# weiguangzhao/PBNet

Measured on AMD Instinct MI355X. Metric: scenes/sec fwd+cluster (ScanNet ~150k pts/scene), higher is better.
Workload: dtype bf16

## Files before the change

include/pbnet_hip.h:

```cpp
#ifndef PBNET_HIP_H
#define PBNET_HIP_H

#include <stddef.h>
#include <stdint.h>

#ifdef __cplusplus
extern "C" {
#endif

typedef void* pbn_stream_t;

enum {
    PBN_OK = 0,
    PBN_ERR_ARG = -1,
    PBN_ERR_WORKSPACE = -2,
    PBN_ERR_HIP = -3,
    PBN_ERR_RANGE = -4,
    PBN_ERR_UNSUPPORTED = -5
};

enum { PBN_F32 = 0, PBN_BF16 = 1, PBN_F16 = 2 };

#define PBN_MAX_SCENES 8

const char* pbn_version(void);
int pbn_last_hip_error(void);

size_t pbn_cluster_workspace_bytes(int n_points, int n_segments, int general_sem);

int pbn_binary_cluster(const float* off_xyz, const float* org_xyz, const int32_t* sem, const int32_t* seg_len,
                       int n_points, int n_segments, float radius, int min_pts, float para_f, int nv_flag,
                       int general_sem , int32_t* cluster_id, int32_t* cluster_num, int32_t* den, float* centers,
                       int32_t* clt_sem, int32_t* n_clusters, int32_t* member_start, int32_t* member_idx,
                       void* workspace, size_t workspace_bytes, pbn_stream_t stream);

int pbn_get_iou(const int32_t* proposals_idx, const int32_t* proposals_offset, const int64_t* instance_labels,
                const int32_t* instance_pointnum, float* proposals_iou, int n_instance, int n_proposal,
                pbn_stream_t stream);

int pbn_cal_iou_and_masklabel(const int32_t* proposals_idx, const int32_t* proposals_offset,
                              const int64_t* instance_labels, const int32_t* instance_pointnum,
                              float* proposals_iou, int n_instance, int n_proposal,
                              const float* mask_scores_sigmoid, float* mask_label, int mode, pbn_stream_t stream);


int pbn_hash_capacity(int n);
size_t pbn_coords_workspace_bytes(int n_max);

int pbn_coords_unique(const int32_t* coords, const int32_t* n_dev, int n_max, uint64_t* table_keys, int32_t* table_vals,
                      int capacity, int32_t* unique_index, int32_t* inverse, int32_t* unique_coords, int32_t* n_unique,
                      void* workspace, size_t workspace_bytes, pbn_stream_t stream);

int pbn_coords_stride(const int32_t* fine_coords, const int32_t* n_fine_dev, int n_fine_max, int stride_out,
                      uint64_t* table_keys, int32_t* table_vals, int capacity, int32_t* coarse_coords,
                      int32_t* parent_row, int32_t* child_k, int32_t* nbr_down, int32_t* n_coarse, void* workspace,
                      size_t workspace_bytes, pbn_stream_t stream);

int pbn_kernel_map(const int32_t* out_coords, const int32_t* n_out_dev, int n_out_max, const int32_t* offsets,
                   int n_offsets, const uint64_t* table_keys, const int32_t* table_vals, int capacity, int32_t* nbr,
                   pbn_stream_t stream);

int pbn_kernel_map_cube(const int32_t* out_coords, const int32_t* n_out_dev, int n_out_max, int kernel_size,
                        int tensor_stride, int x_fastest, const uint64_t* table_keys, const int32_t* table_vals,
                        int capacity, int32_t* nbr, pbn_stream_t stream);

int pbn_up_table(const int32_t* parent_row, const int32_t* child_k, const int32_t* n_fine_dev, int n_fine_max,
                 int32_t* nbr_up, pbn_stream_t stream);

int pbn_spconv_forward(const void* in_feat, int ld_in, int n_in, const int32_t* nbr, int n_offsets, const int32_t* row_perm,
                       const int32_t* n_out_dev, int n_out, const void* w_packed, int vecs_per_offset, int n_steps,
                       int cout_padded, const float* scale, const float* shift, const void* residual, int ld_res,
                       int relu, void* out_feat, int ld_out, int dtype, int rows_per_wave, void* workspace,
                       size_t workspace_bytes, pbn_stream_t stream);

int pbn_spconv_forward_dual(const void* in_feat, int ld_in, int n_in, const int32_t* nbr, int n_offsets,
                            const int32_t* n_out_dev, int n_out, const void* w_packed, int vecs_per_offset, int n_steps,
                            int cout_padded, const float* scale, const float* shift, const void* residual, int ld_res,
                            int relu, void* out_feat, int ld_out, int dtype, int rows_per_wave, void* workspace,
                            size_t workspace_bytes, const void* in2_feat, int ld_in2, int n_in2, int vecs_second,
                            pbn_stream_t stream);

int pbn_spconv_family(int n_out, int n_offsets, int vecs_per_offset, int n_steps, int cout_padded, int dtype, int has_map);

int pbn_gather_rows(const void* in, int ld_in_bytes, const int64_t* idx, int n, int row_bytes, void* out,
                    int ld_out_bytes, pbn_stream_t stream);

size_t pbn_segment_pool_workspace_bytes(int n_seg, int channels);
int pbn_segment_pool(const void* feats, int ld, int channels, int dtype, const int32_t* seg_start, int n_seg,
                     float* out_max, float* out_avg, void* workspace, size_t workspace_bytes, pbn_stream_t stream);

int pbn_local_scene_rows(const int32_t* ent_row_start, const int32_t* ent_member_start, const int32_t* ent_scene,
                         const float* ent_weight, int n_ent, int n_rows, const int32_t* member_idx,
                         const int64_t* ins_ind, const float* xyz, float inv_voxel, const void* point_feat, int ld_feat,
                         int channels, const void* sem_score, int ld_sem, const int64_t* sem_pred, int dtype,
                         int64_t* point_idx, int64_t* row_scene, int32_t* coords, void* feat_out, int ld_out,
                         pbn_stream_t stream);
int pbn_gather_pad_rows(const void* in, int ld_in_bytes, int row_bytes, const int64_t* idx, int n, void* out,
                        int ld_out_bytes, pbn_stream_t stream);

int pbn_pack_weight(const float* src, int n_offsets, int dim_a, int dim_b, int flip, int transpose, int dtype,
                    int vecs_per_offset, int n_steps, int cout_padded, void* out, pbn_stream_t stream);

typedef struct pbn_pack_job {
    const float* src;
    void* out;
    int32_t n_offsets, dim_a, dim_b, flip, transpose, cin, cout, cin_p, cout_p, n_steps;
    int32_t reserved[2];
} pbn_pack_job;
int pbn_pack_weights_batch(const pbn_pack_job* jobs, int n_jobs, int max_vectors, int dtype, pbn_stream_t stream);

int pbn_gather_rulebook_rows(const void* in, int ld_in_bytes, int row_bytes, const int32_t* nbr, int n_offsets, int k0,
                             int kc, int n, void* out, pbn_stream_t stream);

size_t pbn_bn_workspace_bytes(int channels);
int pbn_bn_train_forward(const void* x, int ld_x, int n, int channels, int dtype, const float* weight, const float* bias,
                         float eps, float momentum, float* running_mean, float* running_var, void* y, int ld_y,
                         float* save_mean, float* save_invstd, void* workspace, size_t workspace_bytes, pbn_stream_t stream);
int pbn_bn_train_backward(const void* x, int ld_x, const void* dy, int ld_dy, int n, int channels, int dtype,
                          const float* weight, const float* save_mean, const float* save_invstd, void* dx, int ld_dx,
                          float* dweight, float* dbias, void* workspace, size_t workspace_bytes, pbn_stream_t stream);

int pbn_bn_act_train_forward(const void* x, int ld_x, int n, int channels, int dtype, const float* weight, const float* bias,
                             float eps, float momentum, float* running_mean, float* running_var, const void* residual,
                             int ld_res, int relu, void* y, int ld_y, float* save_mean, float* save_invstd, void* workspace,
                             size_t workspace_bytes, pbn_stream_t stream);
int pbn_bn_act_train_backward(const void* x, int ld_x, const void* dy, int ld_dy, const void* y, int ld_y, int n, int channels,
                              int dtype, const float* weight, const float* save_mean, const float* save_invstd, void* dx,
                              int ld_dx, void* dres, int ld_dres, float* dweight, float* dbias, void* workspace,
                              size_t workspace_bytes, pbn_stream_t stream);

int pbn_rulebook_pair_blocks(int n);
int pbn_rulebook_pair_counts(const int32_t* nbr, int n, int n_offsets, int32_t* table, int32_t* totals, pbn_stream_t stream);
int pbn_rulebook_pair_fill(const int32_t* nbr, int n, int n_offsets, const int32_t* table, const int32_t* seg_start, int seg,
                           int n_segments, int32_t* in_idx, int32_t* out_idx, int64_t* seg_offset, pbn_stream_t stream);

int pbn_rulebook_pair_fill_dev(const int32_t* nbr, int n, int n_offsets, const int32_t* table, const int32_t* totals,
                               int segment, int32_t* seg_begin, int32_t* in_idx, int32_t* out_idx, int64_t* seg_offset,
                               pbn_stream_t stream);

typedef struct {
    const int32_t* nbr;
    int32_t n, n_offsets;
    int32_t* table;
    int32_t* totals;
    int32_t* seg_begin;
    int32_t* in_idx;
    int32_t* out_idx;
    int64_t* seg_offset;
} pbn_pair_job;
int pbn_rulebook_pairs_multi(const pbn_pair_job* jobs, int n_jobs, int segment, pbn_stream_t stream);

size_t pbn_spconv_wgrad_workspace_bytes(int n_offsets, int cin, int cout);
int pbn_spconv_wgrad(const void* x, int ld_x, const void* g, int ld_g, int dtype, const int32_t* in_idx,
                     const int32_t* out_idx, const int32_t* seg_begin, const int32_t* pair_counts, int segment,
                     int n_pairs_total, int n_offsets, int cin, int cout, float* dw, void* workspace, size_t workspace_bytes,
                     pbn_stream_t stream);
int pbn_spconv_wgrad_checked(const void* x, int ld_x, long long n_x_rows, const void* g, int ld_g, long long n_g_rows, int dtype,
                             const int32_t* in_idx, const int32_t* out_idx, const int32_t* seg_begin, const int32_t* pair_counts,
                             int lists_padded, int segment, int n_pairs_total, int n_offsets, int cin, int cout, float* dw,
                             void* workspace, size_t workspace_bytes, pbn_stream_t stream);
typedef struct {
    int32_t form, wa, wb, small_level, strips, co_groups, splits;
    int64_t grid;
} pbn_wgrad_plan;
int pbn_spconv_wgrad_plan(int dtype, int ld_x, int ld_g, int aligned16, int identity, int n_offsets, int n_pairs_total, int cin,
                          int cout, int has_workspace, size_t workspace_bytes, pbn_wgrad_plan* out);

enum {
    PBN_CNT_POINTS = 0, PBN_CNT_CLUSTERS = 1, PBN_CNT_ENTRIES = 2, PBN_CNT_ROWS = 3, PBN_CNT_SCENES = 4,
    PBN_CNT_PROPOSAL_ROWS = 5, PBN_CNT_PROPOSALS = 6, PBN_CNT_OVERFLOW = 7, PBN_CNT_WORDS = 16
};
enum {
    PBN_OVF_POINTS = 1, PBN_OVF_CLUSTERS = 2, PBN_OVF_ENTRIES = 4, PBN_OVF_ROWS = 8, PBN_OVF_SEGMENT = 16,
    PBN_OVF_BATCH = 32, PBN_OVF_LEVEL = 64,
    PBN_OVF_CDIST = 128
};
int pbn_class_gate(const int32_t* table, const float* thr05, int n_classes, int nb, int m_cap, int n_points,
                   int32_t* class_base, int32_t* seg_len, int32_t* counts, pbn_stream_t stream);
size_t pbn_local_plan_workspace_bytes(int c_cap);
int pbn_local_plan(const int32_t* cluster_num, int n_segments, int nb, const int32_t* member_start, const float* centers,
                   const int32_t* n_clusters, const float* thr02, const int32_t* kmax, int c_cap, int e_cap, int r_cap,
                   int32_t* ent_row_start, int32_t* ent_member_start, int32_t* ent_scene, float* ent_weight,
                   int32_t* counts, void* workspace, size_t workspace_bytes, pbn_stream_t stream);
int pbn_proposal_offsets(const int32_t* per_scene, int s_cap, int64_t* proposals_offset, int64_t* alive_ids,
                         int32_t* dense_of, int32_t* counts, pbn_stream_t stream);
int pbn_batch_starts(const int32_t* coords, const int32_t* n_dev, int n_cap, int n_segments, int32_t* seg_start,
                     pbn_stream_t stream);
int pbn_local_scene_rows_dev(const int32_t* ent_row_start, const int32_t* ent_member_start, const int32_t* ent_scene,
                             const float* ent_weight, int n_ent_cap, int n_rows_cap, const int32_t* n_ent_dev,
                             const int32_t* n_rows_dev, const int32_t* member_idx, const int64_t* ins_ind, const float* xyz,
                             float inv_voxel, const void* point_feat, int ld_feat, int channels, const void* sem_score,
                             int ld_sem, const int64_t* sem_pred, int dtype, int64_t* point_idx, int64_t* row_scene,
                             int32_t* coords, void* feat_out, int ld_out, pbn_stream_t stream);
int pbn_gather_pad_rows_dev(const void* in, int ld_in_bytes, int row_bytes, const int64_t* idx, const int64_t* idx2,
                            int n_cap, const int32_t* n_dev, void* out, int ld_out_bytes, pbn_stream_t stream);
int pbn_mlp_rows_dev(const void* in, int ld_in, int in_rows, int channels, const int64_t* idx_a, const int64_t* idx_b, int n_cap,
                     const int32_t* n_dev, const float* w1, const float* scale, const float* shift, const float* slope,
                     int hidden, const float* w2, const float* b2, int n_out, int sigmoid, void* out, int ld_out, int dtype,
                     pbn_stream_t stream);
int pbn_mask_count_dev(const void* mask_score, int ld, float thd, const int64_t* row_scene, int n_cap, const int32_t* n_dev,
                       int n_scenes_cap, int dtype, int32_t* per_scene, int32_t* block_cnt, pbn_stream_t stream);
int pbn_proposal_rows_dev(const void* mask_score, int ld, float thd, const int64_t* row_scene, const int64_t* point_idx,
                          int n_cap, const int32_t* n_dev, const int32_t* dense_of, const int32_t* block_cnt,
                          const float* xyz, float scale, float inv_voxel, const void* point_feat, int ld_feat, int channels,
                          int dtype, int64_t* proposals_idx, void* proposals_ms, int32_t* coords, void* feat_out,
                          pbn_stream_t stream);

int pbn_mlp_rows(const void* in, int ld_in, int channels, const int64_t* idx_a, const int64_t* idx_b, int n,
                 const float* w1, const float* scale, const float* shift, const float* slope, int hidden, const float* w2,
                 const float* b2, int n_out, int sigmoid, void* out, int ld_out, int dtype, pbn_stream_t stream);

int pbn_select_blocks(int n);
int pbn_sem_argmax_table(const void* score, int ld, int n_cls, const int32_t* batch, int nb, int n, int dtype,
                         int64_t* sem_pred, void* sem_prob, int32_t* table, int32_t* block_hist, pbn_stream_t stream);
int pbn_select_points(const int64_t* sem_pred, int n, int n_cls, const int32_t* class_base, const int32_t* block_hist,
                      const float* xyz, const void* offset, int ld_off, int dtype, int64_t* ins_ind, float* ins_orig,
                      float* ins_off, int32_t* ins_sem, pbn_stream_t stream);

int pbn_mask_count(const void* mask_score, int ld, float thd, const int64_t* row_scene, int n, int n_scenes, int dtype,
                   int32_t* per_scene, int32_t* block_cnt, pbn_stream_t stream);
int pbn_proposal_rows(const void* mask_score, int ld, float thd, const int64_t* row_scene, const int64_t* point_idx, int n,
                      const int32_t* dense_of, const int32_t* block_cnt, const float* xyz, float scale, float inv_voxel,
                      const void* point_feat, int ld_feat, int channels, int dtype, int64_t* proposals_idx,
                      void* proposals_ms, int32_t* coords, void* feat_out, pbn_stream_t stream);

int pbn_post_words(int n_fold);
int pbn_proposal_bitmask(const int64_t* proposals_idx, int n_entries, int n_fold, int n_prop, uint32_t* masks,
                         int32_t* counts, pbn_stream_t stream);
int pbn_mask_iou(const uint32_t* masks, const int32_t* rows, int n_rows, int n_fold, const int32_t* counts, float* iou,
                 pbn_stream_t stream);
int pbn_superpoint_refine(const uint32_t* masks, const int32_t* pick, int n_pick, int n_fold, const int64_t* superpoint,
                          int n_sp, int64_t* seg, int32_t* hist, int64_t* sp_label, int64_t* seg_refined,
                          uint32_t* masks_out, int32_t* counts_out, pbn_stream_t stream);
int pbn_bitmask_to_dense(const uint32_t* masks, const int32_t* rows, int n_rows, int n_fold, int32_t* dense,
                         pbn_stream_t stream);

int pbn_post_max_proposals(void);
int pbn_post_select(const float* clt_score, const int32_t* counts, int n_prop, float score_t, int npoint_t, int32_t* rows,
                    int32_t* n_rows, int32_t* status, pbn_stream_t stream);
int pbn_mask_iou_dev(const uint32_t* masks, const int32_t* rows, const int32_t* n_rows, int n_prop, int n_fold,
                     const int32_t* counts, float* iou, pbn_stream_t stream);
int pbn_post_nms(const float* clt_score, const int32_t* rows, const int32_t* n_rows, int n_prop, const float* iou, float nms_t,
                 int32_t* pick, int32_t* pick_rows, int32_t* n_pick, pbn_stream_t stream);
int pbn_superpoint_refine_dev(const uint32_t* masks, const int32_t* pick_rows, const int32_t* n_pick, int n_prop, int n_fold,
                              const int64_t* superpoint, int n_sp_cap, int64_t* seg, int32_t* hist, int64_t* sp_label,
                              int64_t* seg_refined, uint32_t* masks_out, int32_t* counts_out, int32_t* status,
                              pbn_stream_t stream);
int pbn_post_compact(const int32_t* counts2, const int32_t* pick_rows, const int32_t* n_pick, int n_prop, int n_fold,
                     const float* clt_score, const int64_t* proposals_idx, int n_entries, const void* proposals_offset,
                     int offset_i64, const void* pred_sem, int sem_i64, int64_t n_sem, const int64_t* label_table, int n_labels,
                     const uint32_t* masks2, int32_t* keep, float* scores_out, int64_t* semantic_id_out, int32_t* clusters,
                     int32_t* n_keep, int32_t* status, pbn_stream_t stream);

typedef struct pbn_scene_table {
    int32_t n_scenes;
    int32_t point_start[PBN_MAX_SCENES + 1];
    int32_t sp_start[PBN_MAX_SCENES + 1];
} pbn_scene_table;
typedef struct pbn_post_batch_layout {
    int64_t masks, counts, prop_scene, score, rows, pick_rows, n_rows, n_pick, iou, votes, sp_label, seg, seg_refined, counts2,
        renumber, total_bytes;
} pbn_post_batch_layout;
size_t pbn_post_batch_workspace_bytes(int n_prop, int n_points_total, int n_scenes, int n_sp_total, pbn_post_batch_layout* layout);
int pbn_post_batch(const int64_t* proposals_idx, int n_entries, const void* proposals_offset, int offset_i64, int n_prop,
                   const void* clt_score, int score_dtype, const void* pred_sem, int sem_i64, int n_points_total,
                   pbn_scene_table scenes, const int64_t* superpoint, float score_t, int npoint_t, float nms_t,
                   const int64_t* label_table, int n_labels, int32_t* point_instance, float* scores, int64_t* semantic_id,
                   int32_t* npoints, int32_t* scalars, void* workspace, size_t workspace_bytes, pbn_stream_t stream);

typedef struct pbn_tta_table {
    int32_t n_scenes;
    int32_t copies;
    int32_t point_start[PBN_MAX_SCENES + 1];
    int32_t sp_start[PBN_MAX_SCENES + 1];
} pbn_tta_table;
int pbn_post_batch_tta(const int64_t* proposals_idx, int n_entries, const void* proposals_offset, int offset_i64, int n_prop,
                       const void* clt_score, int score_dtype, const void* pred_sem, int sem_i64, int n_points_merged,
                       pbn_tta_table units, const int64_t* superpoint, float score_t, int npoint_t, float nms_t,
                       const int64_t* label_table, int n_labels, int32_t* point_instance, float* scores, int64_t* semantic_id,
                       int32_t* npoints, int32_t* scalars, void* workspace, size_t workspace_bytes, pbn_stream_t stream);

size_t pbn_scene_summary_workspace_bytes(int n_prop, int n_cls);
int pbn_scene_summary_lds_instances(int n_cls);
int pbn_scene_summary(const void* sem_score, int ld, int n_cls, int score_dtype, int n_points_merged, pbn_tta_table units,
                      const int32_t* point_instance, const int32_t* post_scalars, int n_prop, const float* xyz,
                      const int64_t* label_table, int n_labels, int32_t* sem_fold, int64_t* class_vote, int32_t* class_points,
                      float* box, float* centroid, int32_t* status, void* workspace, size_t workspace_bytes, pbn_stream_t stream);

int pbn_instance_overlap(const int32_t* masks, int n_pred, int n_pts, const int32_t* gt_index, int n_gt, int32_t* inter,
                         pbn_stream_t stream);

#define PBN_AP_RECORD_MAGIC 0x41504c47
#define PBN_AP_RECORD_HEADER 8
#define PBN_AP_STATUS_ID_RANGE 4
#define PBN_AP_STATUS_ID_COUNT 8
#define PBN_AP_STATUS_LABEL_RANGE 16
#define PBN_AP_STATUS_INSTANCE_CAP 32
#define PBN_AP_STATUS_SEMANTIC_RANGE 64
int pbn_gt_encode_dev(const void* sem, int sem_i64, const void* ins, int ins_i64, int n_pts, const int32_t* label_table,
                      int n_labels, int32_t* first, int n_inst_cap, int32_t* ids, int32_t* status, pbn_stream_t stream);
int pbn_gt_index_dev(const void* ids, int ids_i64, int n_pts, int32_t* table, int id_cap, int32_t* uid, int32_t* gt_vert,
                     int u_cap, int32_t* n_gt, int32_t* gt_index, int32_t* status, pbn_stream_t stream);
int pbn_instance_overlap_dev(const int32_t* clusters, const int32_t* n_keep, int p_cap, int n_pts, const int32_t* gt_index,
                             const int32_t* n_gt, int u_cap, int32_t* inter, pbn_stream_t stream);
int pbn_ap_record_append(int32_t* state, int32_t* log, int64_t log_words, int scene_tag, const int32_t* n_keep, int p_cap,
                         const int32_t* n_gt, int u_cap, int n_pts, const int32_t* post_status, int32_t* assoc_status,
                         const int32_t* uid, const int32_t* gt_vert, const int64_t* semantic_id, const float* conf,
                         const int32_t* inter, pbn_stream_t stream);

typedef struct pbn_ap_scene_tags {
    int32_t tag[PBN_MAX_SCENES];
} pbn_ap_scene_tags;
size_t pbn_ap_assoc_batch_workspace_bytes(int n_points_total, int n_scenes, int u_cap, int id_cap, int n_inst_cap);
int pbn_ap_assoc_batch_lds_counters(void);
int pbn_ap_assoc_batch(pbn_tta_table units, const int32_t* point_instance, const int32_t* post_scalars, const float* scores,
                       const int64_t* semantic_id, int n_prop, const void* ids, int ids_i64, const void* sem, int sem_i64,
                       const void* ins, int ins_i64, const int32_t* label_table, int n_labels, int u_cap, int id_cap,
                       int n_inst_cap, pbn_ap_scene_tags tags, int32_t* state, int32_t* log, int64_t log_words, void* workspace,
                       size_t workspace_bytes, pbn_stream_t stream);

#define PBN_AP_MAX_CLASSES 32
#define PBN_AP_MAX_OVERLAPS 16
#define PBN_AP_TABLE_SCALARS 16
typedef struct pbn_ap_class_ids {
    int32_t n;
    int32_t id[PBN_AP_MAX_CLASSES];
} pbn_ap_class_ids;
typedef struct pbn_ap_overlaps {
    int32_t n;
    int32_t _pad;
    double th[PBN_AP_MAX_OVERLAPS];
// ... 259 lines not shown
```

pbnet_amd/MinkowskiEngine/nn.py:

```python
import torch
import torch.nn as nn

from .._native import DT as _DT
from ..scratch import StreamScratch
from .core import SparseTensor

_BN_WS = StreamScratch()


def _bn_workspace(device, channels):
    from .. import _native as N
    return _BN_WS.get(device, int(N.lib().pbn_bn_workspace_bytes(int(channels))), min_bytes=1 << 20, zero=True)


def _rows_ok(t):
    es = t.element_size()
    return t.dim() == 2 and t.stride(1) == 1 and (t.stride(0) * es) % 16 == 0 and t.data_ptr() % 16 == 0 \
        and (t.shape[1] * es) % 16 == 0 and t.shape[0] > 0


class _BatchNormTrainFn(torch.autograd.Function):

    @staticmethod
    def forward(ctx, x, weight, bias, running_mean, running_var, eps, momentum):
# ... 62 lines not shown
        dw = torch.empty(c, dtype=torch.float32, device=x.device) if need_w else None
        db = torch.empty(c, dtype=torch.float32, device=x.device) if (weight is not None and ctx.needs_input_grad[2]) else None
        ws = _bn_workspace(x.device, c)
        N.check(N.lib().pbn_bn_act_train_backward(
            N.c_vp(x.data_ptr()), x.stride(0), N.c_vp(dy.data_ptr()), dy.stride(0), None if y is None else N.c_vp(y.data_ptr()),
            0 if y is None else y.stride(0), n, c, _DT[x.dtype], N.ptr(weight), N.ptr(mean), N.ptr(invstd), N.c_vp(dx.data_ptr()), c,
            None if dres is None else N.c_vp(dres.data_ptr()), c, N.ptr(dw), N.ptr(db), N.c_vp(ws.data_ptr()), ws.numel(),
            N.current_stream()), "pbn_bn_act_train_backward")
        if want_res and dres is None:
            dres = dy
        return dx, dw, db, dres, None, None, None, None, None


def bn_act(norm, x, residual=None, relu=True):
    f, bn = x.F, norm.bn
    res = None if residual is None else residual.F
    if norm.NATIVE_TRAIN and norm.FUSE_ACT and bn.training and f.is_cuda and bn.momentum is not None and f.dtype in _DT \
            and _rows_ok(f) and (bn.weight is None or bn.weight.dtype == torch.float32) \
            and (res is None or (res.dtype == f.dtype and _rows_ok(res) and res.shape == f.shape)):
        norm._tick()
        rm, rv = (bn.running_mean, bn.running_var) if bn.track_running_stats else (None, None)
        return x.replace_feature(_BatchNormActTrainFn.apply(f, bn.weight, bn.bias, res, rm, rv, bn.eps, bn.momentum, relu))
    out = norm(x)
    if residual is not None:
        out = out.replace_feature(out.F + residual.F)
    return out.replace_feature(torch.relu(out.F)) if relu else out


def _flush_ticks_hook(module, prefix, keep_vars):
    module.flush_ticks()


def _drop_ticks_hook(module, state_dict, prefix, *unused):
    if prefix + "num_batches_tracked" in state_dict:
        module.__dict__["_pending_ticks"] = 0


class _TickedBatchNorm1d(nn.BatchNorm1d):

    def __init__(self, *a, **k):
        super().__init__(*a, **k)
        self.__dict__["_pending_ticks"] = 0
        self.register_state_dict_pre_hook(_flush_ticks_hook)
        self.register_load_state_dict_pre_hook(_drop_ticks_hook)

    def flush_ticks(self):
        t = self.__dict__.get("_pending_ticks", 0)
        if t:
            self.__dict__["_pending_ticks"] = 0
            buf = self._buffers.get("num_batches_tracked")
            if buf is not None:
                buf.add_(t)

    def __getattr__(self, name):
        if name == "num_batches_tracked":
            self.flush_ticks()
        return super().__getattr__(name)

    def _apply(self, fn, *a, **k):
        self.flush_ticks()
        return super()._apply(fn, *a, **k)

    def buffers(self, *a, **k):
        self.flush_ticks()
        return super().buffers(*a, **k)

    def named_buffers(self, *a, **k):
        self.flush_ticks()
        return super().named_buffers(*a, **k)


class MinkowskiBatchNorm(nn.Module):

    NATIVE_TRAIN = True
    FUSE_ACT = True

    def __init__(self, num_features, eps=1e-5, momentum=0.1, affine=True, track_running_stats=True):
        super().__init__()
        self.bn = _TickedBatchNorm1d(num_features, eps=eps, momentum=momentum, affine=affine,
                                     track_running_stats=track_running_stats)

    def _tick(self):
        bn = self.bn
        if bn.track_running_stats and bn._buffers.get("num_batches_tracked") is not None:
            bn.__dict__["_pending_ticks"] = bn.__dict__.get("_pending_ticks", 0) + 1

    def forward(self, x):
        f, bn = x.F, self.bn
        if self.NATIVE_TRAIN and bn.training and f.is_cuda and bn.momentum is not None and f.dtype in _DT and _rows_ok(f) \
                and (bn.weight is None or bn.weight.dtype == torch.float32):
            self._tick()
            rm, rv = (bn.running_mean, bn.running_var) if bn.track_running_stats else (None, None)
            return x.replace_feature(_BatchNormTrainFn.apply(f, bn.weight, bn.bias, rm, rv, bn.eps, bn.momentum))
        return x.replace_feature(bn(f))


class _Elementwise(nn.Module):
    MODULE = None

    def __init__(self, *args, **kwargs):
        super().__init__()
        self.module = self.MODULE(*args, **kwargs)

    def forward(self, x):
        f = x.F
        if f.dtype != torch.float32 and any(True for _ in self.module.parameters()):
            return x.replace_feature(self.module(f.float()).to(f.dtype))
        return x.replace_feature(self.module(f))


class MinkowskiReLU(_Elementwise):
    MODULE = nn.ReLU


class MinkowskiPReLU(_Elementwise):
    MODULE = nn.PReLU


class MinkowskiSigmoid(_Elementwise):
    MODULE = nn.Sigmoid


class MinkowskiSoftmax(_Elementwise):
    MODULE = nn.Softmax

    def __init__(self, dim=1):
        super().__init__(dim=dim)


def _batch_index(x):
    assert x.tensor_stride >= 1
    b = x.C[:, 0].long()
    return b, int(b.max().item()) + 1 if b.numel() else 0


def segment_pool(feats, batch_sorted, n_batch, want_max=True, want_avg=True, seg_start=None):
    from .. import _native as N
    assert feats.stride(1) == 1
    if seg_start is None:
        seg_start = torch.searchsorted(batch_sorted.to(torch.int32).contiguous(),
                                       torch.arange(n_batch + 1, dtype=torch.int32, device=feats.device)).to(torch.int32)
    c = feats.shape[1]
    mx = torch.empty(n_batch, c, dtype=torch.float32, device=feats.device) if want_max else None
    av = torch.empty(n_batch, c, dtype=torch.float32, device=feats.device) if want_avg else None
    lib = N.lib()
    ws_bytes = int(lib.pbn_segment_pool_workspace_bytes(int(n_batch), c))
    ws = torch.empty(max(ws_bytes, 16), dtype=torch.uint8, device=feats.device)
    rc = lib.pbn_segment_pool(N.c_vp(feats.data_ptr()), feats.stride(0), c, _DT[feats.dtype], N.ptr(seg_start),
                              int(n_batch), N.ptr(mx), N.ptr(av), N.c_vp(ws.data_ptr()), ws_bytes, N.current_stream())
    N.check(rc, "pbn_segment_pool")
    return mx, av


class _SegmentPoolFn(torch.autograd.Function):

    @staticmethod
    def forward(ctx, feats, batch_sorted, n_batch):
        mx, av = segment_pool(feats.detach(), batch_sorted, n_batch)
        b = batch_sorted.long()
        ctx.save_for_backward(feats, b, mx)
        ctx.n_batch = n_batch
        return mx + av

    @staticmethod
    def backward(ctx, g):
        feats, b, mx = ctx.saved_tensors
        g = g.float()
        f = feats.float()
        cnt = torch.bincount(b, minlength=ctx.n_batch).to(torch.float32).clamp_(min=1.0)
        gb = g[b]
        ties = (f == mx[b]).to(torch.float32)
        tie_cnt = torch.zeros(ctx.n_batch, f.shape[1], dtype=torch.float32, device=f.device).index_add_(0, b, ties)
        grad = gb / cnt[b][:, None] + gb * ties / tie_cnt[b].clamp_(min=1.0)
        return grad.to(feats.dtype), None, None


def global_max_plus_avg_pool(x):
    b, nb = _batch_index(x)
    return _PooledTensor(_SegmentPoolFn.apply(x.F, x.C[:, 0].contiguous(), nb).to(x.F.dtype))


class _GlobalPool(nn.Module):
    MODE = "avg"

    def forward(self, x):
        b, nb = _batch_index(x)
        f = x.F.float()
        if self.MODE == "avg":
            s = torch.zeros(nb, f.shape[1], dtype=f.dtype, device=f.device).index_add_(0, b, f)
            cnt = torch.zeros(nb, dtype=f.dtype, device=f.device).index_add_(0, b, torch.ones_like(b, dtype=f.dtype))
            out = s / cnt[:, None]
        else:
            out = torch.full((nb, f.shape[1]), float("-inf"), dtype=f.dtype, device=f.device)
            out = out.scatter_reduce(0, b[:, None].expand_as(f), f, reduce="amax", include_self=True)
        return _PooledTensor(out.to(x.F.dtype))


class _PooledTensor(object):

    def __init__(self, feats):
        self._F = feats

    @property
    def F(self):
        return self._F

    def replace_feature(self, feats):
        return _PooledTensor(feats)

    def __add__(self, other):
        return _PooledTensor(self._F + other._F)


class MinkowskiGlobalAvgPooling(_GlobalPool):
    MODE = "avg"


class MinkowskiGlobalMaxPooling(_GlobalPool):
    MODE = "max"
```

pbnet_amd/_native.py:

```python
import ctypes
import os

import torch

_HERE = os.path.dirname(os.path.abspath(__file__))
LIB_PATH = os.environ.get("PBNET_HIP_LIB") or os.path.join(_HERE, "libpbnet_hip.so")

_lib = None

c_f32p = ctypes.c_void_p
c_i32p = ctypes.c_void_p
c_vp = ctypes.c_void_p
c_int = ctypes.c_int
c_float = ctypes.c_float
c_size = ctypes.c_size_t

c_i64 = ctypes.c_int64
c_i32 = ctypes.c_int32

DT = {torch.float32: 0, torch.bfloat16: 1, torch.float16: 2}


class CoordsLayout(ctypes.Structure):
    _fields_ = [("counts", c_i64), ("unique_index", c_i64), ("inverse", c_i64),
                ("keys", c_i64 * 5), ("vals", c_i64 * 5), ("coords", c_i64 * 5), ("k3", c_i64 * 5),
                ("parent_row", c_i64 * 4), ("child_k", c_i64 * 4), ("nbr_down", c_i64 * 4), ("up", c_i64 * 4),
                ("k5", c_i64), ("workspace", c_i64), ("workspace_bytes", c_i64),
                ("capacity", c_i32 * 5), ("_pad", c_i32)]


class PrepareLayout(ctypes.Structure):
    _fields_ = [("pyramid", CoordsLayout), ("n_unique", c_i64), ("unique_index", c_i64), ("inverse", c_i64),
                ("perm", c_i64), ("inv_perm", c_i64), ("ucoords", c_i64), ("tmp_keys", c_i64), ("tmp_vals", c_i64),
                ("uidx32", c_i64), ("inv32", c_i64), ("sort_keys", c_i64), ("sort_vals", c_i64), ("sort_temp", c_i64),
                ("sort_temp_bytes", c_i64)]


class UnetOp(ctypes.Structure):
    _fields_ = [("map_kind", c_i32), ("level_in", c_i32), ("level_out", c_i32),
                ("in_buf", c_i32), ("in_col", c_i32), ("res_buf", c_i32), ("res_col", c_i32), ("out_buf", c_i32),
                ("out_col", c_i32), ("vpo", c_i32), ("n_steps", c_i32), ("cout_p", c_i32), ("relu", c_i32),
                ("in2_buf", c_i32), ("in2_col", c_i32), ("vpo2", c_i32),
                ("w", ctypes.c_void_p), ("scale", ctypes.c_void_p), ("shift", ctypes.c_void_p)]


class WgradPlan(ctypes.Structure):
    _fields_ = [("form", c_i32), ("wa", c_i32), ("wb", c_i32), ("small_level", c_i32), ("strips", c_i32),
                ("co_groups", c_i32), ("splits", c_i32), ("grid", c_i64)]


class UnetBuf(ctypes.Structure):
    _fields_ = [("level", c_i32), ("width", c_i32)]


class TrainOp(ctypes.Structure):
    _fields_ = [("map_kind", c_i32), ("level_in", c_i32), ("level_out", c_i32),
                ("in_buf", c_i32), ("in_col", c_i32), ("pre_buf", c_i32), ("res_buf", c_i32), ("res_col", c_i32),
                ("out_buf", c_i32), ("out_col", c_i32), ("relu", c_i32), ("cin", c_i32), ("cout", c_i32),
                ("vpo", c_i32), ("n_steps", c_i32), ("cout_p", c_i32), ("vpo_d", c_i32), ("n_steps_d", c_i32),
                ("cout_p_d", c_i32), ("want_dx", c_i32), ("dx_accumulate", c_i32), ("_pad", c_i32),
                ("w", ctypes.c_void_p), ("w_d", ctypes.c_void_p), ("gamma", ctypes.c_void_p), ("beta", ctypes.c_void_p),
                ("running_mean", ctypes.c_void_p), ("running_var", ctypes.c_void_p), ("eps", ctypes.c_float),
                ("momentum", ctypes.c_float), ("stat_off", ctypes.c_int64), ("dw_off", ctypes.c_int64),
                ("dgamma_off", ctypes.c_int64), ("dbeta_off", ctypes.c_int64)]


class PairJob(ctypes.Structure):
    _fields_ = [("nbr", ctypes.c_void_p), ("n", c_i32), ("n_offsets", c_i32), ("table", ctypes.c_void_p),
                ("totals", ctypes.c_void_p), ("seg_begin", ctypes.c_void_p), ("in_idx", ctypes.c_void_p),
                ("out_idx", ctypes.c_void_p), ("seg_offset", ctypes.c_void_p)]


class PairLists(ctypes.Structure):
    _fields_ = [("in_idx", ctypes.c_void_p), ("out_idx", ctypes.c_void_p), ("seg_begin", ctypes.c_void_p),
                ("counts", ctypes.c_void_p), ("segment", c_i32), ("n_pairs_estimate", c_i32)]


MAX_SCENES = 8


class SceneTable(ctypes.Structure):
    _fields_ = [("n_scenes", c_i32), ("point_start", c_i32 * (MAX_SCENES + 1)), ("sp_start", c_i32 * (MAX_SCENES + 1))]


class TtaTable(ctypes.Structure):
    _fields_ = [("n_scenes", c_i32), ("copies", c_i32), ("point_start", c_i32 * (MAX_SCENES + 1)),
                ("sp_start", c_i32 * (MAX_SCENES + 1))]


class SceneTags(ctypes.Structure):
    _fields_ = [("tag", c_i32 * MAX_SCENES)]


AP_MAX_CLASSES, AP_MAX_OVERLAPS, AP_TABLE_SCALARS = 32, 16, 16


class ApClassIds(ctypes.Structure):
    _fields_ = [("n", c_i32), ("id", c_i32 * AP_MAX_CLASSES)]


class ApOverlaps(ctypes.Structure):
    _fields_ = [("n", c_i32), ("_pad", c_i32), ("th", ctypes.c_double * AP_MAX_OVERLAPS)]


class PostBatchLayout(ctypes.Structure):
    _fields_ = [(k, c_i64) for k in ("masks", "counts", "prop_scene", "score", "rows", "pick_rows", "n_rows", "n_pick", "iou",
                                     "votes", "sp_label", "seg", "seg_refined", "counts2", "renumber", "total_bytes")]


SIGNATURES = {
    "pbn_version": (ctypes.c_char_p, []),
    "pbn_last_hip_error": (c_int, []),
    "pbn_cluster_workspace_bytes": (c_size, [c_int, c_int, c_int]),
    "pbn_binary_cluster": (c_int, [c_f32p, c_f32p, c_i32p, c_i32p, c_int, c_int, c_float, c_int, c_float, c_int, c_int,
                                   c_i32p, c_i32p, c_i32p, c_f32p, c_i32p, c_i32p, c_i32p, c_i32p, c_vp, c_size, c_vp]),
    "pbn_get_iou": (c_int, [c_i32p, c_i32p, c_vp, c_i32p, c_f32p, c_int, c_int, c_vp]),
    "pbn_cal_iou_and_masklabel": (c_int, [c_i32p, c_i32p, c_vp, c_i32p, c_f32p, c_int, c_int, c_f32p, c_f32p, c_int,
                                          c_vp]),
    "pbn_hash_capacity": (c_int, [c_int]),
    "pbn_coords_workspace_bytes": (c_size, [c_int]),
    "pbn_coords_unique": (c_int, [c_i32p, c_i32p, c_int, c_vp, c_i32p, c_int, c_i32p, c_i32p, c_i32p, c_i32p, c_vp,
                                  c_size, c_vp]),
    "pbn_coords_stride": (c_int, [c_i32p, c_i32p, c_int, c_int, c_vp, c_i32p, c_int, c_i32p, c_i32p, c_i32p, c_i32p,
                                  c_i32p, c_vp, c_size, c_vp]),
    "pbn_kernel_map": (c_int, [c_i32p, c_i32p, c_int, c_i32p, c_int, c_vp, c_i32p, c_int, c_i32p, c_vp]),
    "pbn_up_table": (c_int, [c_i32p, c_i32p, c_i32p, c_int, c_i32p, c_vp]),
    "pbn_spconv_forward": (c_int, [c_vp, c_int, c_int, c_i32p, c_int, c_i32p, c_i32p, c_int, c_vp, c_int, c_int, c_int,
                                   c_f32p, c_f32p, c_vp, c_int, c_int, c_vp, c_int, c_int, c_int, c_vp, c_size, c_vp]),
    "pbn_spconv_forward_dual": (c_int, [c_vp, c_int, c_int, c_i32p, c_int, c_i32p, c_int, c_vp, c_int, c_int, c_int, c_f32p, c_f32p,
                                        c_vp, c_int, c_int, c_vp, c_int, c_int, c_int, c_vp, c_size, c_vp, c_int, c_int, c_int, c_vp]),
    "pbn_spconv_family": (c_int, [c_int, c_int, c_int, c_int, c_int, c_int, c_int]),
    "pbn_spconv_wgrad_workspace_bytes": (c_size, [c_int, c_int, c_int]),
    "pbn_spconv_wgrad": (c_int, [c_vp, c_int, c_vp, c_int, c_int, c_vp, c_vp, c_i32p, c_i32p, c_int, c_int, c_int, c_int, c_int,
                                 c_f32p, c_vp, c_size, c_vp]),
    "pbn_spconv_wgrad_checked": (c_int, [c_vp, c_int, ctypes.c_longlong, c_vp, c_int, ctypes.c_longlong, c_int, c_vp, c_vp, c_i32p,
                                         c_i32p, c_int, c_int, c_int, c_int, c_int, c_int, c_f32p, c_vp, c_size, c_vp]),
    "pbn_spconv_wgrad_plan": (c_int, [c_int, c_int, c_int, c_int, c_int, c_int, c_int, c_int, c_int, c_int, c_size,
                                      ctypes.POINTER(WgradPlan)]),
    "pbn_gather_rows": (c_int, [c_vp, c_int, c_vp, c_int, c_int, c_vp, c_int, c_vp]),
    "pbn_segment_pool_workspace_bytes": (c_size, [c_int, c_int]),
    "pbn_segment_pool": (c_int, [c_vp, c_int, c_int, c_int, c_i32p, c_int, c_f32p, c_f32p, c_vp, c_size, c_vp]),
    "pbn_local_scene_rows": (c_int, [c_i32p, c_i32p, c_i32p, c_f32p, c_int, c_int, c_i32p, c_vp, c_f32p, c_float, c_vp,
                                     c_int, c_int, c_vp, c_int, c_vp, c_int, c_vp, c_vp, c_i32p, c_vp, c_int, c_vp]),
    "pbn_gather_pad_rows": (c_int, [c_vp, c_int, c_int, c_vp, c_int, c_vp, c_int, c_vp]),
    "pbn_mlp_rows": (c_int, [c_vp, c_int, c_int, c_vp, c_vp, c_int, c_f32p, c_f32p, c_f32p, c_f32p, c_int, c_f32p, c_f32p,
                             c_int, c_int, c_vp, c_int, c_int, c_vp]),
    "pbn_select_blocks": (c_int, [c_int]),
    "pbn_sem_argmax_table": (c_int, [c_vp, c_int, c_int, c_i32p, c_int, c_int, c_int, c_vp, c_vp, c_i32p, c_i32p, c_vp]),
    "pbn_select_points": (c_int, [c_vp, c_int, c_int, c_i32p, c_i32p, c_f32p, c_vp, c_int, c_int, c_vp, c_f32p, c_f32p,
                                  c_i32p, c_vp]),
    "pbn_mask_count": (c_int, [c_vp, c_int, c_float, c_vp, c_int, c_int, c_int, c_i32p, c_i32p, c_vp]),
    "pbn_proposal_rows": (c_int, [c_vp, c_int, c_float, c_vp, c_vp, c_int, c_i32p, c_i32p, c_f32p, c_float, c_float, c_vp,
                                  c_int, c_int, c_int, c_vp, c_vp, c_i32p, c_vp, c_vp]),
    "pbn_post_words": (c_int, [c_int]),
    "pbn_proposal_bitmask": (c_int, [c_vp, c_int, c_int, c_int, c_vp, c_i32p, c_vp]),
    "pbn_mask_iou": (c_int, [c_vp, c_i32p, c_int, c_int, c_i32p, c_f32p, c_vp]),
    "pbn_superpoint_refine": (c_int, [c_vp, c_i32p, c_int, c_int, c_vp, c_int, c_vp, c_i32p, c_vp, c_vp, c_vp, c_i32p,
                                      c_vp]),
    "pbn_bitmask_to_dense": (c_int, [c_vp, c_i32p, c_int, c_int, c_i32p, c_vp]),
    "pbn_post_max_proposals": (c_int, []),
    "pbn_post_select": (c_int, [c_f32p, c_i32p, c_int, c_float, c_int, c_i32p, c_i32p, c_i32p, c_vp]),
    "pbn_mask_iou_dev": (c_int, [c_vp, c_i32p, c_i32p, c_int, c_int, c_i32p, c_f32p, c_vp]),
    "pbn_post_nms": (c_int, [c_f32p, c_i32p, c_i32p, c_int, c_f32p, c_float, c_i32p, c_i32p, c_i32p, c_vp]),
    "pbn_superpoint_refine_dev": (c_int, [c_vp, c_i32p, c_i32p, c_int, c_int, c_vp, c_int, c_vp, c_i32p, c_vp, c_vp, c_vp, c_i32p,
                                          c_i32p, c_vp]),
    "pbn_post_compact": (c_int, [c_i32p, c_i32p, c_i32p, c_int, c_int, c_f32p, c_vp, c_int, c_vp, c_int, c_vp, c_int, c_i64, c_vp,
                                 c_int, c_vp, c_i32p, c_f32p, c_vp, c_i32p, c_i32p, c_i32p, c_vp]),
    "pbn_post_batch_workspace_bytes": (c_size, [c_int, c_int, c_int, c_int, ctypes.POINTER(PostBatchLayout)]),
    "pbn_post_batch": (c_int, [c_vp, c_int, c_vp, c_int, c_int, c_vp, c_int, c_vp, c_int, c_int, SceneTable, c_vp, c_float, c_int,
                               c_float, c_vp, c_int, c_i32p, c_f32p, c_vp, c_i32p, c_i32p, c_vp, c_size, c_vp]),
    "pbn_post_batch_tta": (c_int, [c_vp, c_int, c_vp, c_int, c_int, c_vp, c_int, c_vp, c_int, c_int, TtaTable, c_vp, c_float, c_int,
                                   c_float, c_vp, c_int, c_i32p, c_f32p, c_vp, c_i32p, c_i32p, c_vp, c_size, c_vp]),
    "pbn_scene_summary_workspace_bytes": (c_size, [c_int, c_int]),
    "pbn_scene_summary_lds_instances": (c_int, [c_int]),
    "pbn_scene_summary": (c_int, [c_vp, c_int, c_int, c_int, c_int, TtaTable, c_i32p, c_i32p, c_int, c_f32p, c_vp, c_int, c_i32p,
                                  c_vp, c_i32p, c_f32p, c_f32p, c_i32p, c_vp, c_size, c_vp]),
    "pbn_instance_overlap": (c_int, [c_i32p, c_int, c_int, c_i32p, c_int, c_i32p, c_vp]),
    "pbn_gt_encode_dev": (c_int, [c_vp, c_int, c_vp, c_int, c_int, c_i32p, c_int, c_i32p, c_int, c_i32p, c_i32p, c_vp]),
    "pbn_gt_index_dev": (c_int, [c_vp, c_int, c_int, c_i32p, c_int, c_i32p, c_i32p, c_int, c_i32p, c_i32p, c_i32p, c_vp]),
    "pbn_instance_overlap_dev": (c_int, [c_i32p, c_i32p, c_int, c_int, c_i32p, c_i32p, c_int, c_i32p, c_vp]),
    "pbn_ap_record_append": (c_int, [c_i32p, c_i32p, c_i64, c_int, c_i32p, c_int, c_i32p, c_int, c_int, c_i32p, c_i32p, c_i32p,
                                     c_i32p, c_vp, c_f32p, c_i32p, c_vp]),
    "pbn_ap_assoc_batch_workspace_bytes": (c_size, [c_int, c_int, c_int, c_int, c_int]),
    "pbn_ap_assoc_batch_lds_counters": (c_int, []),
    "pbn_ap_assoc_batch": (c_int, [TtaTable, c_i32p, c_i32p, c_f32p, c_vp, c_int, c_vp, c_int, c_vp, c_int, c_vp, c_int, c_i32p,
                                   c_int, c_int, c_int, c_int, SceneTags, c_i32p, c_i32p, c_i64, c_vp, c_size, c_vp]),
    "pbn_ap_table_workspace_bytes": (c_size, [c_int, c_i64]),
    "pbn_ap_table_lds_entries": (c_int, []),
    "pbn_ap_table_reset": (c_int, [c_vp, c_size, c_int, c_i64, c_vp]),
    "pbn_ap_table_add_log": (c_int, [c_vp, c_size, c_int, c_i64, c_i32p, c_i32p, c_i64, c_int, ApClassIds, ApOverlaps, c_int,
                                     c_vp]),
    "pbn_ap_table_finish": (c_int, [c_vp, c_size, c_int, c_i64, c_int, c_int, c_f32p, c_i32p, c_i32p, c_i32p, c_i32p, c_vp]),
    "pbn_rulebook_pair_blocks": (c_int, [c_int]),
    "pbn_bn_workspace_bytes": (c_size, [c_int]),
    "pbn_bn_train_forward": (c_int, [c_vp, c_int, c_int, c_int, c_int, c_f32p, c_f32p, ctypes.c_float, ctypes.c_float, c_f32p,
                                     c_f32p, c_vp, c_int, c_f32p, c_f32p, c_vp, c_size, c_vp]),
    "pbn_bn_train_backward": (c_int, [c_vp, c_int, c_vp, c_int, c_int, c_int, c_int, c_f32p, c_f32p, c_f32p, c_vp, c_int,
                                      c_f32p, c_f32p, c_vp, c_size, c_vp]),
    "pbn_bn_act_train_forward": (c_int, [c_vp, c_int, c_int, c_int, c_int, c_f32p, c_f32p, ctypes.c_float, ctypes.c_float,
                                         c_f32p, c_f32p, c_vp, c_int, c_int, c_vp, c_int, c_f32p, c_f32p, c_vp, c_size, c_vp]),
    "pbn_bn_act_train_backward": (c_int, [c_vp, c_int, c_vp, c_int, c_vp, c_int, c_int, c_int, c_int, c_f32p, c_f32p, c_f32p,
                                          c_vp, c_int, c_vp, c_int, c_f32p, c_f32p, c_vp, c_size, c_vp]),
    "pbn_rulebook_pair_counts": (c_int, [c_i32p, c_int, c_int, c_i32p, c_i32p, c_vp]),
    "pbn_rulebook_pair_fill_dev": (c_int, [c_i32p, c_int, c_int, c_i32p, c_i32p, c_int, c_i32p, c_vp, c_vp, c_vp, c_vp]),
    "pbn_rulebook_pair_fill": (c_int, [c_i32p, c_int, c_int, c_i32p, c_i32p, c_int, c_int, c_vp, c_vp, c_vp, c_vp]),
    "pbn_gather_rulebook_rows": (c_int, [c_vp, c_int, c_int, c_i32p, c_int, c_int, c_int, c_int, c_vp, c_vp]),
    "pbn_pack_weights_batch": (c_int, [c_vp, c_int, c_int, c_int, c_vp]),
    "pbn_pack_weight": (c_int, [c_f32p, c_int, c_int, c_int, c_int, c_int, c_int, c_int, c_int, c_int, c_vp, c_vp]),
    "pbn_kernel_map_cube": (c_int, [c_i32p, c_i32p, c_int, c_int, c_int, c_int, c_vp, c_i32p, c_int, c_i32p, c_vp]),
    "pbn_coords_arena_bytes": (c_size, [c_int, c_int, ctypes.POINTER(CoordsLayout)]),
    "pbn_coords_build": (c_int, [c_i32p, c_i32p, c_int, c_int, c_int, c_vp, c_size, ctypes.POINTER(CoordsLayout), c_vp]),
    "pbn_coords_prepare_bytes": (c_size, [c_int, c_int, ctypes.POINTER(PrepareLayout)]),
    "pbn_coords_prepare": (c_int, [c_i32p, c_int, c_int, c_int, c_vp, c_size, ctypes.POINTER(PrepareLayout), c_vp]),
    "pbn_coords_prepare_dev": (c_int, [c_i32p, c_i32p, c_int, c_int, c_int, c_vp, c_size, ctypes.POINTER(PrepareLayout), c_vp]),
    "pbn_coords_prepare_hash": (c_int, [c_i32p, c_i32p, c_int, c_int, c_int, c_vp, c_size, ctypes.POINTER(PrepareLayout), c_vp]),
    "pbn_unet_forward_dev": (c_int, [ctypes.POINTER(UnetOp), c_int, ctypes.POINTER(UnetBuf), c_int, ctypes.POINTER(c_i32),
                                     c_i32p, ctypes.POINTER(c_i32), c_vp, c_int, ctypes.POINTER(ctypes.c_void_p), c_vp,
                                     ctypes.POINTER(ctypes.c_void_p), ctypes.POINTER(ctypes.c_void_p), c_vp, c_size, c_int,
                                     c_vp, c_size, c_vp]),
    "pbn_class_gate": (c_int, [c_i32p, c_f32p, c_int, c_int, c_int, c_int, c_i32p, c_i32p, c_i32p, c_vp]),
    "pbn_local_plan_workspace_bytes": (c_size, [c_int]),
    "pbn_local_plan": (c_int, [c_i32p, c_int, c_int, c_i32p, c_f32p, c_i32p, c_f32p, c_i32p, c_int, c_int, c_int, c_i32p,
                               c_i32p, c_i32p, c_f32p, c_i32p, c_vp, c_size, c_vp]),
    "pbn_proposal_offsets": (c_int, [c_i32p, c_int, c_vp, c_vp, c_i32p, c_i32p, c_vp]),
    "pbn_batch_starts": (c_int, [c_i32p, c_i32p, c_int, c_int, c_i32p, c_vp]),
    "pbn_local_scene_rows_dev": (c_int, [c_i32p, c_i32p, c_i32p, c_f32p, c_int, c_int, c_i32p, c_i32p, c_i32p, c_vp, c_f32p,
                                         c_float, c_vp, c_int, c_int, c_vp, c_int, c_vp, c_int, c_vp, c_vp, c_i32p, c_vp,
                                         c_int, c_vp]),
    "pbn_gather_pad_rows_dev": (c_int, [c_vp, c_int, c_int, c_vp, c_vp, c_int, c_i32p, c_vp, c_int, c_vp]),
    "pbn_mlp_rows_dev": (c_int, [c_vp, c_int, c_int, c_int, c_vp, c_vp, c_int, c_i32p, c_f32p, c_f32p, c_f32p, c_f32p, c_int,
                                 c_f32p, c_f32p, c_int, c_int, c_vp, c_int, c_int, c_vp]),
    "pbn_mask_count_dev": (c_int, [c_vp, c_int, c_float, c_vp, c_int, c_i32p, c_int, c_int, c_i32p, c_i32p, c_vp]),
    "pbn_proposal_rows_dev": (c_int, [c_vp, c_int, c_float, c_vp, c_vp, c_int, c_i32p, c_i32p, c_i32p, c_f32p, c_float,
                                      c_float, c_vp, c_int, c_int, c_int, c_vp, c_vp, c_i32p, c_vp, c_vp]),
    "pbn_morton_keys": (c_int, [c_i32p, c_i32p, c_int, c_vp, c_vp]),
    "pbn_unet_arena_bytes": (c_size, [ctypes.POINTER(UnetBuf), c_int, ctypes.POINTER(c_i32), c_int,
                                      ctypes.POINTER(c_i64)]),
    "pbn_unet_forward": (c_int, [ctypes.POINTER(UnetOp), c_int, ctypes.POINTER(UnetBuf), c_int, ctypes.POINTER(c_i32),
                                 c_vp, c_int, ctypes.POINTER(ctypes.c_void_p), c_vp, ctypes.POINTER(ctypes.c_void_p),
                                 ctypes.POINTER(ctypes.c_void_p), c_vp, c_size, c_int, c_vp, c_size, c_vp]),
    "pbn_rulebook_pairs_multi": (c_int, [ctypes.POINTER(PairJob), c_int, c_int, c_vp]),
    "pbn_unet_train_forward": (c_int, [ctypes.POINTER(TrainOp), c_int, ctypes.POINTER(UnetBuf), c_int, ctypes.POINTER(c_i32),
                                       c_vp, c_int, ctypes.POINTER(ctypes.c_void_p), c_vp, ctypes.POINTER(ctypes.c_void_p),
                                       ctypes.POINTER(ctypes.c_void_p), c_vp, c_size, c_vp, c_int, c_vp, c_size, c_vp, c_size,
                                       c_vp]),
    "pbn_unet_train_backward": (c_int, [ctypes.POINTER(TrainOp), c_int, ctypes.POINTER(UnetBuf), c_int, ctypes.POINTER(c_i32),
                                        c_vp, c_int, ctypes.POINTER(ctypes.c_void_p), c_vp, ctypes.POINTER(ctypes.c_void_p),
                                        ctypes.POINTER(ctypes.c_void_p), ctypes.POINTER(PairLists), c_vp, c_vp, c_size, c_vp,
                                        c_vp, c_vp, c_int, c_int, c_vp, c_size, c_vp, c_size, c_vp, c_size, c_vp]),
    "pbn_unet_forward_timed": (c_int, [ctypes.POINTER(UnetOp), c_int, ctypes.POINTER(UnetBuf), c_int,
                                       ctypes.POINTER(c_i32), c_vp, c_int, ctypes.POINTER(ctypes.c_void_p), c_vp,
                                       ctypes.POINTER(ctypes.c_void_p), ctypes.POINTER(ctypes.c_void_p), c_vp, c_size,
                                       c_int, c_vp, c_size, c_vp, ctypes.POINTER(ctypes.c_float)]),
    "pbn_aug_chunks": (c_int, [c_int]),
    "pbn_aug_workspace_bytes": (c_size, [c_int]),
    "pbn_aug_affine": (c_int, [c_f32p, c_i32p, c_int, c_int, c_i32p, c_vp, c_vp, c_i32p, c_vp, c_vp, c_vp, c_vp]),
    "pbn_aug_elastic": (c_int, [c_vp, c_i32p, c_int, c_int, c_i32p, c_int, c_int, c_f32p, c_f32p, c_int, ctypes.c_double, c_vp,
                                c_vp, c_vp]),
    "pbn_aug_sub_min": (c_int, [c_vp, c_i32p, c_int, c_int, c_i32p, c_vp, c_vp]),
    "pbn_aug_crop": (c_int, [c_vp, c_i32p, c_int, c_int, c_i32p, c_vp, c_i32p, c_vp, c_int, c_int, c_i32p, c_i32p, c_vp, c_vp,
                             c_vp, c_vp]),
    "pbn_aug_compact": (c_int, [c_vp, c_f32p, c_f32p, c_vp, c_i32p, c_vp, c_i32p, c_i32p, c_int, c_i32p, c_int, c_i32p, c_vp,
                                c_vp, c_i32p, c_vp, c_vp, c_i32p, c_i32p, c_i32p, c_i32p, c_i32p, c_vp, c_f32p, c_vp, c_i32p,
                                c_i32p, c_int, c_int, c_vp]),
    "pbn_aug_instances": (c_int, [c_vp, c_i32p, c_i32p, c_int, c_i32p, c_i32p, c_int, c_int, c_i32p, c_f32p, c_f32p, c_vp,
                                  c_vp]),
    "pbn_aug_quantize": (c_int, [c_vp, c_i32p, c_int, c_int, ctypes.c_double, c_i32p, c_f32p, c_vp]),
    "pbn_mesh_workspace_bytes": (c_size, [c_int, c_int, c_int]),
    "pbn_mesh_vertex_normals": (c_int, [c_f32p, c_int, c_vp, c_int, c_int, c_f32p, c_i32p, c_vp, c_size, c_vp]),
    "pbn_mesh_segment": (c_int, [c_f32p, c_int, c_vp, c_int, c_int, c_float, c_int, c_vp, c_f32p, c_vp, c_size,
                                 ctypes.POINTER(ctypes.c_float), c_vp]),
    "pbn_mesh_segment_point": (c_int, [c_f32p, c_f32p, c_int, c_vp, c_int, c_int, c_float, c_int, c_vp, c_vp, c_size, c_vp]),
    "pbn_cloud_workspace_bytes": (c_size, [c_int, c_int]),
    "pbn_cloud_max_k": (c_int, []),
    "pbn_cloud_knn": (c_int, [c_f32p, c_int, c_int, c_float, c_i32p, c_f32p, c_i32p, c_vp, c_size, c_vp]),
    "pbn_cloud_knn_timed": (c_int, [c_f32p, c_int, c_int, c_float, c_i32p, c_f32p, c_i32p, c_vp, c_size, c_vp,
                                    ctypes.POINTER(ctypes.c_float)]),
    "pbn_cloud_normals": (c_int, [c_f32p, c_int, c_i32p, c_int, c_f32p, c_f32p, c_vp]),
    "pbn_thin_workspace_bytes": (c_size, [c_int]),
    "pbn_thin_points": (c_int, [c_f32p, c_f32p, c_int, ctypes.c_double, c_f32p, c_f32p, c_i32p, c_i32p, c_i32p, c_i32p, c_vp, c_size,
                                c_vp]),
    "pbn_thin_points_timed": (c_int, [c_f32p, c_f32p, c_int, ctypes.c_double, c_f32p, c_f32p, c_i32p, c_i32p, c_i32p, c_i32p, c_vp,
                                      c_size, c_vp, ctypes.POINTER(ctypes.c_float)]),
    "pbn_cloud_outlier_workspace_bytes": (c_size, [c_int]),
    "pbn_cloud_outlier_mask": (c_int, [c_f32p, c_int, c_int, ctypes.c_double, c_vp, c_vp, c_vp, c_size, c_vp]),
    "pbn_cloud_raw_index_workspace_bytes": (c_size, [c_int]),
    "pbn_cloud_raw_index": (c_int, [c_i32p, c_int, c_vp, c_i32p, c_int, c_int, c_i32p, c_vp, c_size, c_vp]),
    "pbn_cloud_radius_workspace_bytes": (c_size, [c_int]),
    "pbn_cloud_radius_count": (c_int, [c_f32p, c_int, c_float, c_int, c_float, c_i32p, c_i32p, c_vp, c_size, c_vp]),
    "pbn_cloud_radius_count_timed": (c_int, [c_f32p, c_int, c_float, c_int, c_float, c_i32p, c_i32p, c_vp, c_size, c_vp,
                                             ctypes.POINTER(ctypes.c_float)]),
    "pbn_cloud_radius_raw_index_workspace_bytes": (c_size, [c_int, c_int]),
    "pbn_cloud_radius_raw_index": (c_int, [c_f32p, c_int, c_vp, c_float, c_float, c_i32p, c_int, c_i32p, c_i32p, c_vp, c_size,
                                           c_vp]),
    "pbn_cloud_orient_workspace_bytes": (c_size, [c_int, c_int]),
    "pbn_cloud_orient": (c_int, [c_f32p, c_int, c_i32p, c_int, c_f32p, c_vp, c_i32p, c_i32p, c_i32p, c_vp, c_size, c_vp]),
    "pbn_cloud_orient_timed": (c_int, [c_f32p, c_int, c_i32p, c_int, c_f32p, c_vp, c_i32p, c_i32p, c_i32p, c_vp, c_size, c_vp,
                                       ctypes.POINTER(ctypes.c_float)]),
    "pbn_cloud_upright_workspace_bytes": (c_size, [c_int, c_int]),
    "pbn_cloud_upright_max_hyp": (c_int, []),
    "pbn_cloud_upright_chunk": (c_int, []),
    "pbn_cloud_upright_hyp_block": (c_int, []),
    "pbn_cloud_upright": (c_int, [c_f32p, c_int, c_float, c_int, ctypes.c_uint64, ctypes.POINTER(ctypes.c_double),
                                  ctypes.c_double, c_int, c_f32p, c_vp, c_f32p, c_vp, c_f32p, c_vp, c_vp, c_i32p, c_i32p, c_vp,
                                  c_size, c_vp]),
    "pbn_cloud_upright_timed": (c_int, [c_f32p, c_int, c_float, c_int, ctypes.c_uint64, ctypes.POINTER(ctypes.c_double),
                                        ctypes.c_double, c_int, c_f32p, c_vp, c_f32p, c_vp, c_f32p, c_vp, c_vp, c_i32p, c_i32p,
                                        c_vp, c_size, c_vp, ctypes.POINTER(ctypes.c_float)]),
    "pbn_cloud_upright_chunked": (c_int, [c_f32p, c_int, c_float, c_int, ctypes.c_uint64, ctypes.POINTER(ctypes.c_double),
                                          ctypes.c_double, c_int, c_int, c_f32p, c_vp, c_f32p, c_vp, c_f32p, c_vp, c_vp, c_i32p,
                                          c_i32p, c_vp, c_size, c_vp]),
    "pbn_cloud_vote_workspace_bytes": (c_size, [c_int, c_int]),
    "pbn_cloud_vote_labels": (c_int, [c_i32p, c_i32p, c_i32p, c_int, c_int, c_int, c_vp, c_vp, c_i32p, c_i32p, c_i32p, c_vp, c_vp,
                                      c_size, c_vp]),
    "pbn_cloud_vote_labels_timed": (c_int, [c_i32p, c_i32p, c_i32p, c_int, c_int, c_int, c_vp, c_vp, c_i32p, c_i32p, c_i32p, c_vp,
                                            c_vp, c_size, c_vp, ctypes.POINTER(ctypes.c_float)]),
    "pbn_sem_confusion":(c_int, [c_vp, c_int, c_vp, c_int, c_i64, c_int, c_int, c_vp, c_vp, c_vp]),
    "pbn_mask_accuracy": (c_int, [c_vp, c_int, c_vp, c_int, c_i64, c_float, c_vp, c_vp]),
    "pbn_losses_workspace_bytes": (c_size, [c_i64, c_i64, c_i64]),
    "pbn_losses_forward": (c_int, [c_vp, c_int, c_int, c_vp, c_vp, c_int, c_f32p, c_f32p, c_vp, c_i64, c_int, c_vp, c_int, c_vp,
                                   c_vp, c_i64, c_f32p, c_int, c_vp, c_int, c_i64, ctypes.c_double, ctypes.c_double, c_f32p,
                                   c_f32p, c_vp, c_vp, c_vp, c_size, c_vp]),
    "pbn_losses_backward": (c_int, [c_vp, c_int, c_int, c_vp, c_vp, c_int, c_f32p, c_f32p, c_vp, c_i64, c_int, c_vp, c_int, c_vp,
                                    c_vp, c_i64, c_vp, c_int, c_f32p, c_i64, c_vp, c_f32p, c_vp, c_vp, c_vp, c_vp, c_vp]),
    "pbn_optim_chunk": (c_int, []),
    "pbn_optim_adam": (c_int, [c_vp, c_int, c_float, c_float, c_float, c_float, c_float, c_float, c_float, c_float, c_float,
                               c_int, c_vp]),
    "pbn_optim_sgd": (c_int, [c_vp, c_int, c_float, c_float, c_float, c_int, c_vp]),
    "pbn_loss_meter_update": (c_int, [c_f32p, c_vp, c_vp, c_int, c_vp]),
    "pbn_selftest_workspace_bytes": (c_size, [c_int, c_int]),
    "pbn_selftest_sort_tile": (c_int, []),
    "pbn_selftest_fill": (c_int, [c_vp, ctypes.POINTER(c_i64), ctypes.POINTER(c_i64), ctypes.POINTER(ctypes.c_uint8), c_int, c_vp]),
    "pbn_selftest_scan": (c_int, [c_i32p, c_i32p, c_int, c_int, c_i32p, c_i32p, c_vp, c_size, c_vp]),
    "pbn_selftest_sort_u32": (c_int, [c_vp, c_i32p, c_int, c_vp, c_i32p, c_i32p, c_vp, c_size, c_vp]),
}

PBN_OK, PBN_ERR_ARG, PBN_ERR_WORKSPACE, PBN_ERR_HIP, PBN_ERR_RANGE, PBN_ERR_UNSUPPORTED = 0, -1, -2, -3, -4, -5
ERRORS = {-1: "PBN_ERR_ARG", -2: "PBN_ERR_WORKSPACE", -3: "PBN_ERR_HIP", -4: "PBN_ERR_RANGE", -5: "PBN_ERR_UNSUPPORTED"}


class NativeLibraryError(ImportError):
    pass


def lib():
    global _lib
    if _lib is None:
        if not os.path.exists(LIB_PATH):
            raise NativeLibraryError(
                "libpbnet_hip.so not found at %s -- build it with `python -c 'import __graft_entry__ as g; g.build()'` "
                "or `make -C pbnet_amd/csrc`; there is no CPU fallback." % LIB_PATH)
        try:
            handle = ctypes.CDLL(LIB_PATH)
        except OSError as e:
            raise NativeLibraryError("cannot load %s: %s" % (LIB_PATH, e))
        for name, (res, args) in SIGNATURES.items():
            fn = getattr(handle, name)
            fn.restype = res
            fn.argtypes = args
        _lib = handle
    return _lib


def check(rc, what):
    if rc != 0:
        detail = ""
        if rc == -3:
            detail = " (hipError %d)" % lib().pbn_last_hip_error()
        raise RuntimeError("%s failed: %s%s" % (what, ERRORS.get(rc, str(rc)), detail))


def ptr(t):
    if t is None:
# ... 17 lines not shown
```

pbnet_amd/csrc/plan.hip:

```cpp
#include "pbn_common.h"

namespace pbn {
namespace {

constexpr int MAX_K = 6;
constexpr int SEG_CLUSTERS = 2048;

__device__ __forceinline__ int wave_incl_scan_i(int v, int lane) {
#pragma unroll
    for (int o = 1; o < 64; o <<= 1) {
        const int t = __shfl_up(v, o, 64);
        if (lane >= o) v += t;
    }
    return v;
}

__global__ __launch_bounds__(64) void k_class_gate(const int* __restrict__ table, const float* __restrict__ thr05, int n_cls,
                                                  int nb, int m_cap, int n_points, int* __restrict__ class_base,
                                                  int* __restrict__ seg_len, int* __restrict__ counts) {
    const int lane = threadIdx.x;
    int tot = 0;
    if (lane < n_cls)
        for (int b = 0; b < nb; ++b) tot += table[lane * nb + b];
    const bool keep = lane >= 2 && lane < n_cls && !((float)tot < thr05[lane]);
    const int kept = keep ? tot : 0;
    const int incl = wave_incl_scan_i(kept, lane);
    const int m = __shfl(incl, 63, 64);
    int all = tot;
#pragma unroll
    for (int o = 32; o > 0; o >>= 1) all += __shfl_xor(all, o, 64);
    int flags = 0;
    if (all != n_points) flags |= PBN_OVF_BATCH;
    if (m > m_cap) flags |= PBN_OVF_POINTS;
    const bool drop_all = flags != 0;
    if (lane < n_cls) class_base[lane] = (keep && !drop_all) ? incl - kept : -1;
    if (lane >= 2 && lane < n_cls)
        for (int b = 0; b < nb; ++b) seg_len[(lane - 2) * nb + b] = (keep && !drop_all) ? table[lane * nb + b] : 0;
    if (lane == 0) {
        counts[PBN_CNT_POINTS] = drop_all ? 0 : m;
        if (flags) atomicOr(&counts[PBN_CNT_OVERFLOW], flags);
    }
}

__global__ __launch_bounds__(64) void k_plan_scenes(const int* __restrict__ cluster_num, int n_seg, int nb,
                                                   const int* __restrict__ member_start, const float* __restrict__ centers,
                                                   const float* __restrict__ thr02, const int* __restrict__ kmax,
                                                   const int* __restrict__ n_clusters, int c_cap,
                                                   int* __restrict__ scene_n_ent, int* __restrict__ scene_ent,
                                                   float* __restrict__ scene_w, int* __restrict__ counts) {
    __shared__ float s_d2[SEG_CLUSTERS];
    const int lane = threadIdx.x;
    const int C = min(*n_clusters, c_cap);
    const int gid = blockIdx.x;
    if (gid >= C) return;
    int seg = -1, g0 = 0, cb = 0;
    {
        int carry = 0;
        for (int base = 0; base < n_seg && seg < 0; base += 64) {
            const int i = base + lane;
            const int v = i < n_seg ? cluster_num[i] : 0;
            const int incl = wave_incl_scan_i(v, lane);
            const int lo = carry + incl - v, hi = carry + incl;
            const unsigned long long hit = __ballot(i < n_seg && gid >= lo && gid < hi);
            if (hit) {
                const int src = __ffsll((long long)hit) - 1;
                seg = base + src;
                g0 = __shfl(lo, src, 64);
                cb = __shfl(v, src, 64);
            }
            carry += __shfl(incl, 63, 64);
        }
    }
    if (seg < 0) return;
    const int cls = 2 + seg / nb;
    const int para_k = min(min(cb - 1, kmax[cls]), MAX_K);
    const int size = member_start[gid + 1] - member_start[gid];
    const bool big = (float)size > thr02[cls] && para_k > 0;
    int* ent = scene_ent + (size_t)gid * (MAX_K + 1);
    float* wts = scene_w + (size_t)gid * (MAX_K + 1);
    if (lane == 0) { ent[0] = gid; wts[0] = 1.0f; }
    if (!big) {
        if (lane == 0) scene_n_ent[gid] = 1;
        return;
    }
    if (cb > SEG_CLUSTERS) {
        if (lane == 0) { scene_n_ent[gid] = 1; atomicOr(&counts[PBN_CNT_OVERFLOW], PBN_OVF_SEGMENT); }
        return;
    }
    if (cb > 25 && lane == 0) atomicOr(&counts[PBN_CNT_OVERFLOW], PBN_OVF_CDIST);
    const float cx = centers[3 * gid + 0], cy = centers[3 * gid + 1], cz = centers[3 * gid + 2];
    for (int j = lane; j < cb; j += 64) {
        const int o = g0 + j;
        const float dx = __fsub_rn(centers[3 * o + 0], cx), dy = __fsub_rn(centers[3 * o + 1], cy),
                    dz = __fsub_rn(centers[3 * o + 2], cz);
        s_d2[j] = (o == gid) ? __builtin_inff() : __fadd_rn(__fadd_rn(__fmul_rn(dx, dx), __fmul_rn(dy, dy)), __fmul_rn(dz, dz));
    }
    __syncthreads();
    for (int k = 0; k < para_k; ++k) {
        float best = __builtin_inff();
        int bj = 0x7fffffff;
        for (int j = lane; j < cb; j += 64) {
            const float d = s_d2[j];
            if (d < best) { best = d; bj = j; }
        }
#pragma unroll
        for (int o = 32; o > 0; o >>= 1) {
            const float ob = __shfl_xor(best, o, 64);
            const int oj = __shfl_xor(bj, o, 64);
            if (ob < best || (ob == best && oj < bj)) { best = ob; bj = oj; }
        }
        if (lane == 0) {
            ent[1 + k] = g0 + bj;
            wts[1 + k] = (float)(0.5 * (double)((para_k + 1) - k) / (double)(para_k + 1));
            s_d2[bj] = __builtin_inff();
        }
        __syncthreads();
    }
    if (lane == 0) scene_n_ent[gid] = 1 + para_k;
}

constexpr int PACK_TPB = 256;
__device__ __forceinline__ int block_excl_scan256(int v, int* s_w, int& total) {
    const int lane = threadIdx.x & 63, wid = threadIdx.x >> 6;
    const int incl = wave_incl_scan_i(v, lane);
    if (lane == 63) s_w[wid] = incl;
    __syncthreads();
    int off = 0, tot = 0;
#pragma unroll
    for (int w = 0; w < PACK_TPB / 64; ++w) {
        const int t = s_w[w];
        if (w < wid) off += t;
        tot += t;
    }
    total = tot;
    __syncthreads();
    return off + incl - v;
}

__global__ __launch_bounds__(PACK_TPB) void k_plan_pack(const int* __restrict__ scene_n_ent, const int* __restrict__ scene_ent,
                                                       const float* __restrict__ scene_w, const int* __restrict__ member_start,
                                                       const int* __restrict__ n_clusters, int c_cap, int e_cap, int r_cap,
                                                       int* __restrict__ scene_base, int* __restrict__ ent_row_start,
                                                       int* __restrict__ ent_member_start, int* __restrict__ ent_scene,
                                                       float* __restrict__ ent_weight, int* __restrict__ counts) {
    __shared__ int s_w[PACK_TPB / 64];
    __shared__ int s_flag;
    const int C = min(*n_clusters, c_cap);
    if (threadIdx.x == 0) s_flag = (*n_clusters > c_cap) ? PBN_OVF_CLUSTERS : 0;
    int carry = 0;
    for (int base = 0; base < C; base += PACK_TPB) {
        const int c = base + threadIdx.x;
        const int v = c < C ? scene_n_ent[c] : 0;
        int tot;
        const int ex = block_excl_scan256(v, s_w, tot);
        if (c < C) scene_base[c] = carry + ex;
        carry += tot;
    }
    const int n_ent = carry;
    __syncthreads();
    if (n_ent > e_cap) {
        if (threadIdx.x == 0) {
            atomicOr(&counts[PBN_CNT_OVERFLOW], PBN_OVF_ENTRIES | s_flag);
            counts[PBN_CNT_ENTRIES] = 0; counts[PBN_CNT_ROWS] = 0; counts[PBN_CNT_SCENES] = 0;
            counts[PBN_CNT_CLUSTERS] = C;
            ent_row_start[0] = 0;
        }
        return;
    }
    for (int c = threadIdx.x; c < C; c += PACK_TPB) {
        const int b = scene_base[c], ne = scene_n_ent[c];
        for (int j = 0; j < ne; ++j) {
            const int cl = scene_ent[(size_t)c * (MAX_K + 1) + j];
            ent_member_start[b + j] = member_start[cl];
            ent_scene[b + j] = c;
            ent_weight[b + j] = scene_w[(size_t)c * (MAX_K + 1) + j];
            ent_row_start[b + j + 1] = member_start[cl + 1] - member_start[cl];
        }
    }
    __syncthreads();
    carry = 0;
    for (int base = 0; base < n_ent; base += PACK_TPB) {
        const int e = base + threadIdx.x;
        const int v = e < n_ent ? ent_row_start[e + 1] : 0;
        int tot;
        const int ex = block_excl_scan256(v, s_w, tot);
        if (e < n_ent) ent_row_start[e + 1] = carry + ex + v;
        carry += tot;
    }
    if (threadIdx.x == 0) {
        ent_row_start[0] = 0;
        int flags = s_flag;
        const bool ovf = carry > r_cap;
        if (ovf) flags |= PBN_OVF_ROWS;
        counts[PBN_CNT_ENTRIES] = ovf ? 0 : n_ent;
        counts[PBN_CNT_ROWS] = ovf ? 0 : carry;
        counts[PBN_CNT_SCENES] = ovf ? 0 : C;
        counts[PBN_CNT_CLUSTERS] = C;
        if (flags) atomicOr(&counts[PBN_CNT_OVERFLOW], flags);
    }
}

__global__ __launch_bounds__(PACK_TPB) void k_proposal_offsets(const int* __restrict__ per_scene, int s_cap,
                                                              long long* __restrict__ proposals_offset,
                                                              long long* __restrict__ alive_ids, int* __restrict__ dense_of,
                                                              int* __restrict__ counts) {
    __shared__ int s_w[PACK_TPB / 64];
    const int S = min(counts[PBN_CNT_SCENES], s_cap);
    int carry_a = 0, carry_r = 0;
    for (int base = 0; base < S; base += PACK_TPB) {
        const int s = base + threadIdx.x;
        const int rows = s < S ? per_scene[s] : 0;
        const int alive = rows > 0 ? 1 : 0;
        int tot_a, tot_r;
        const int ex_a = block_excl_scan256(alive, s_w, tot_a);
        const int ex_r = block_excl_scan256(rows, s_w, tot_r);
        if (s < S) {
            dense_of[s] = carry_a + ex_a + alive - 1;
            if (alive) {
                alive_ids[carry_a + ex_a] = s;
                proposals_offset[carry_a + ex_a] = carry_r + ex_r;
            }
        }
        carry_a += tot_a;
        carry_r += tot_r;
    }
    if (threadIdx.x == 0) {
        proposals_offset[carry_a] = carry_r;
        counts[PBN_CNT_PROPOSALS] = carry_a;
        counts[PBN_CNT_PROPOSAL_ROWS] = carry_r;
    }
}

__global__ __launch_bounds__(256) void k_batch_starts(const int* __restrict__ coords, const int* __restrict__ n_dev, int n_cap,
                                                     int n_seg, int* __restrict__ seg_start) {
    const int s = blockIdx.x * 256 + threadIdx.x;
    if (s > n_seg) return;
    const int n = n_dev ? min(*n_dev, n_cap) : n_cap;
    int lo = 0, hi = n;
    while (lo < hi) {
        const int mid = (lo + hi) >> 1;
        if (coords[4 * (size_t)mid] < s) lo = mid + 1; else hi = mid;
    }
    seg_start[s] = lo;
}

}
}

using namespace pbn;

extern "C" int pbn_class_gate(const int32_t* table, const float* thr05, int n_classes, int nb, int m_cap, int n_points,
                              int32_t* class_base, int32_t* seg_len, int32_t* counts, pbn_stream_t stream) {
    if (!table || !thr05 || !class_base || !seg_len || !counts || n_classes < 3 || n_classes > 64 || nb < 1 || m_cap < 0)
        return PBN_ERR_ARG;
    hipLaunchKernelGGL(k_class_gate, dim3(1), dim3(64), 0, (hipStream_t)stream, table, thr05, n_classes, nb, m_cap, n_points,
                       class_base, seg_len, counts);
    PBN_LAUNCH_CHECK();
    return PBN_OK;
}

extern "C" size_t pbn_local_plan_workspace_bytes(int c_cap) {
    if (c_cap < 0) return 0;
    const size_t c = (size_t)(c_cap > 0 ? c_cap : 1);
    return align_up(c * 4, 256) * 2 + align_up(c * (MAX_K + 1) * 4, 256) * 2;
}

extern "C" int pbn_local_plan(const int32_t* cluster_num, int n_segments, int nb, const int32_t* member_start,
                              const float* centers, const int32_t* n_clusters, const float* thr02, const int32_t* kmax,
                              int c_cap, int e_cap, int r_cap, int32_t* ent_row_start, int32_t* ent_member_start,
                              int32_t* ent_scene, float* ent_weight, int32_t* counts, void* workspace,
                              size_t workspace_bytes, pbn_stream_t stream_) {
    hipStream_t stream = (hipStream_t)stream_;
    if (!cluster_num || !member_start || !centers || !n_clusters || !thr02 || !kmax || !ent_row_start || !ent_member_start ||
        !ent_scene || !ent_weight || !counts || !workspace || n_segments < 1 || nb < 1 || c_cap < 1 || e_cap < 1 || r_cap < 1)
        return PBN_ERR_ARG;
    if (workspace_bytes < pbn_local_plan_workspace_bytes(c_cap)) return PBN_ERR_WORKSPACE;
    Carver cv(workspace, workspace_bytes);
    int* scene_n_ent = cv.take<int>(c_cap);
    int* scene_base = cv.take<int>(c_cap);
    int* scene_ent = cv.take<int>((size_t)c_cap * (MAX_K + 1));
    float* scene_w = cv.take<float>((size_t)c_cap * (MAX_K + 1));
    { const int frc_ = fill_bytes(scene_n_ent, 0, sizeof(int) * (size_t)c_cap, stream); if (frc_ != PBN_OK) return frc_; }
    hipLaunchKernelGGL(k_plan_scenes, dim3(c_cap), dim3(64), 0, stream, cluster_num, n_segments, nb, member_start, centers,
                       thr02, kmax, n_clusters, c_cap, scene_n_ent, scene_ent, scene_w, counts);
    hipLaunchKernelGGL(k_plan_pack, dim3(1), dim3(PACK_TPB), 0, stream, scene_n_ent, scene_ent, scene_w, member_start,
                       n_clusters, c_cap, e_cap, r_cap, scene_base, ent_row_start, ent_member_start, ent_scene, ent_weight,
                       counts);
    PBN_LAUNCH_CHECK();
    return PBN_OK;
}

extern "C" int pbn_proposal_offsets(const int32_t* per_scene, int s_cap, int64_t* proposals_offset, int64_t* alive_ids,
                                    int32_t* dense_of, int32_t* counts, pbn_stream_t stream) {
    if (!per_scene || !proposals_offset || !alive_ids || !dense_of || !counts || s_cap < 1) return PBN_ERR_ARG;
    hipLaunchKernelGGL(k_proposal_offsets, dim3(1), dim3(PACK_TPB), 0, (hipStream_t)stream, per_scene, s_cap,
                       (long long*)proposals_offset, (long long*)alive_ids, dense_of, counts);
    PBN_LAUNCH_CHECK();
    return PBN_OK;
}

extern "C" int pbn_batch_starts(const int32_t* coords, const int32_t* n_dev, int n_cap, int n_segments, int32_t* seg_start,
                                pbn_stream_t stream) {
    if (!coords || !seg_start || n_cap < 0 || n_segments < 0) return PBN_ERR_ARG;
    hipLaunchKernelGGL(k_batch_starts, dim3(cdiv(n_segments + 1, 256)), dim3(256), 0, (hipStream_t)stream, coords, n_dev, n_cap,
                       n_segments, seg_start);
    PBN_LAUNCH_CHECK();
    return PBN_OK;
}
```

pbnet_amd/csrc/pool.hip:

```cpp
#include <hip/hip_bf16.h>
#include <hip/hip_fp16.h>
#include "pbn_common.h"

namespace pbn {
namespace {

template <typename T> __device__ __forceinline__ float to_f32(T v);
template <> __device__ __forceinline__ float to_f32<float>(float v) { return v; }
template <> __device__ __forceinline__ float to_f32<__hip_bfloat16>(__hip_bfloat16 v) { return __bfloat162float(v); }
template <> __device__ __forceinline__ float to_f32<__half>(__half v) { return __half2float(v); }

template <typename T>
__global__ __launch_bounds__(256) void k_segment_pool(const T* __restrict__ feats, int ld, int channels,
                                                     const int* __restrict__ seg_start, float* __restrict__ out_max,
                                                     float* __restrict__ out_avg) {
    __shared__ float s_max[8][32], s_sum[8][32];
    const int b = blockIdx.x, c = blockIdx.y * 32 + (threadIdx.x & 31), rg = threadIdx.x >> 5;
    const int beg = seg_start[b], end = seg_start[b + 1];
    float mx = -__builtin_inff(), sm = 0.f;
    if (c < channels)
        for (int r = beg + rg; r < end; r += 8) {
            const float v = to_f32<T>(feats[(size_t)r * ld + c]);
            mx = fmaxf(mx, v);
            sm += v;
        }
    s_max[rg][threadIdx.x & 31] = mx;
    s_sum[rg][threadIdx.x & 31] = sm;
    __syncthreads();
    if (rg == 0 && c < channels) {
#pragma unroll
        for (int k = 1; k < 8; ++k) { mx = fmaxf(mx, s_max[k][threadIdx.x]); sm += s_sum[k][threadIdx.x]; }
        if (out_max) out_max[(size_t)b * channels + c] = mx;
        if (out_avg) out_avg[(size_t)b * channels + c] = sm / (float)(end - beg);
    }
}

constexpr int POOL_SPLIT_MAX = 64;

template <typename T> struct PoolVec;
template <> struct PoolVec<float> {
    static constexpr int E = 4;
    static __device__ __forceinline__ void unpack(const uint4& v, float* f) {
        f[0] = __uint_as_float(v.x); f[1] = __uint_as_float(v.y); f[2] = __uint_as_float(v.z); f[3] = __uint_as_float(v.w);
    }
};
template <> struct PoolVec<__hip_bfloat16> {
    static constexpr int E = 8;
    static __device__ __forceinline__ void unpack(const uint4& v, float* f) {
        const unsigned w[4] = {v.x, v.y, v.z, v.w};
#pragma unroll
        for (int i = 0; i < 4; ++i) { f[2 * i] = __uint_as_float(w[i] << 16); f[2 * i + 1] = __uint_as_float(w[i] & 0xffff0000u); }
    }
};
template <> struct PoolVec<__half> {
    static constexpr int E = 8;
    static __device__ __forceinline__ void unpack(const uint4& v, float* f) {
        const unsigned w[4] = {v.x, v.y, v.z, v.w};
#pragma unroll
        for (int i = 0; i < 4; ++i) {
            const float2 t = __half22float2(__builtin_bit_cast(__half2, w[i]));
            f[2 * i] = t.x; f[2 * i + 1] = t.y;
        }
    }
};

template <typename T>
__global__ __launch_bounds__(256) void k_pool_partial(const uint4* __restrict__ feats, int ld_vec, int vpr,
                                                     const int* __restrict__ seg_start, int split,
                                                     float* __restrict__ part_max, float* __restrict__ part_sum) {
    constexpr int E = PoolVec<T>::E;
    extern __shared__ float s_red[];
    const int b = blockIdx.x, z = blockIdx.y;
    const int beg = seg_start[b], end = seg_start[b + 1];
    const long long len = end - beg;
    const int lo = beg + (int)(len * z / split), hi = beg + (int)(len * (z + 1) / split);
    const int rps = 256 / vpr;
    const int q = threadIdx.x % vpr, rl = threadIdx.x / vpr;
    float mx[E], sm[E];
#pragma unroll
    for (int i = 0; i < E; ++i) { mx[i] = -__builtin_inff(); sm[i] = 0.f; }
    if (rl < rps) {
        int r = lo + rl;
        for (; r + 3 * rps < hi; r += 4 * rps) {
            uint4 v[4];
#pragma unroll
            for (int u = 0; u < 4; ++u) v[u] = feats[(size_t)(r + u * rps) * ld_vec + q];
#pragma unroll
            for (int u = 0; u < 4; ++u) {
                float f[E];
                PoolVec<T>::unpack(v[u], f);
#pragma unroll
                for (int i = 0; i < E; ++i) { mx[i] = fmaxf(mx[i], f[i]); sm[i] += f[i]; }
            }
        }
        for (; r < hi; r += rps) {
            float f[E];
            PoolVec<T>::unpack(feats[(size_t)r * ld_vec + q], f);
#pragma unroll
            for (int i = 0; i < E; ++i) { mx[i] = fmaxf(mx[i], f[i]); sm[i] += f[i]; }
        }
    }
    const int C = vpr * E;
    float* s_mx = s_red;
    float* s_sm = s_red + rps * C;
    if (rl < rps) {
#pragma unroll
        for (int i = 0; i < E; ++i) { s_mx[rl * C + q * E + i] = mx[i]; s_sm[rl * C + q * E + i] = sm[i]; }
    }
    __syncthreads();
    for (int c = threadIdx.x; c < C; c += 256) {
        float m = -__builtin_inff(), t = 0.f;
        for (int k = 0; k < rps; ++k) { m = fmaxf(m, s_mx[k * C + c]); t += s_sm[k * C + c]; }
        part_max[((size_t)b * split + z) * C + c] = m;
        part_sum[((size_t)b * split + z) * C + c] = t;
    }
}

__global__ __launch_bounds__(256) void k_pool_final(const float* __restrict__ part_max, const float* __restrict__ part_sum,
                                                   const int* __restrict__ seg_start, int n_seg, int C, int split,
                                                   float* __restrict__ out_max, float* __restrict__ out_avg) {
    const int e = blockIdx.x * 256 + threadIdx.x;
    if (e >= n_seg * C) return;
    const int b = e / C, c = e - b * C;
    float m = -__builtin_inff(), t = 0.f;
    for (int z = 0; z < split; ++z) {
        m = fmaxf(m, part_max[((size_t)b * split + z) * C + c]);
        t += part_sum[((size_t)b * split + z) * C + c];
    }
    if (out_max) out_max[e] = m;
    if (out_avg) out_avg[e] = t / (float)(seg_start[b + 1] - seg_start[b]);
}

int pool_split(int n_seg) {
    int s = 1024 / (n_seg > 0 ? n_seg : 1);
    return s < 1 ? 1 : (s > POOL_SPLIT_MAX ? POOL_SPLIT_MAX : s);
}

}
}

using namespace pbn;

extern "C" size_t pbn_segment_pool_workspace_bytes(int n_seg, int channels) {
    if (n_seg <= 0 || channels <= 0) return 0;
    return (size_t)2 * n_seg * pool_split(n_seg) * channels * sizeof(float);
}

extern "C" int pbn_segment_pool(const void* feats, int ld, int channels, int dtype, const int32_t* seg_start, int n_seg,
                                float* out_max, float* out_avg, void* workspace, size_t workspace_bytes,
                                pbn_stream_t stream_) {
    hipStream_t stream = (hipStream_t)stream_;
    if (n_seg < 0 || channels <= 0 || ld < channels) return PBN_ERR_ARG;
    if (n_seg == 0) return PBN_OK;
    if (!feats || !seg_start || (!out_max && !out_avg)) return PBN_ERR_ARG;
    const int esz = dtype == PBN_F32 ? 4 : 2;
    const int split = pool_split(n_seg);
    if (workspace && workspace_bytes >= pbn_segment_pool_workspace_bytes(n_seg, channels) && split > 1 &&
        (channels * esz) % 16 == 0 && (ld * esz) % 16 == 0 && ((uintptr_t)feats & 15) == 0 &&
        ((uintptr_t)workspace & 15) == 0 && channels * esz / 16 <= 256) {
        const int vpr = channels * esz / 16, rps = 256 / vpr;
        float* pm = reinterpret_cast<float*>(workspace);
        float* ps = pm + (size_t)n_seg * split * channels;
        const size_t lds = (size_t)2 * rps * channels * sizeof(float);
        const dim3 grid(n_seg, split);
        if (dtype == PBN_F32)
            hipLaunchKernelGGL(k_pool_partial<float>, grid, dim3(256), lds, stream, (const uint4*)feats, ld * esz / 16, vpr,
                               seg_start, split, pm, ps);
        else if (dtype == PBN_BF16)
            hipLaunchKernelGGL(k_pool_partial<__hip_bfloat16>, grid, dim3(256), lds, stream, (const uint4*)feats,
                               ld * esz / 16, vpr, seg_start, split, pm, ps);
        else if (dtype == PBN_F16)
            hipLaunchKernelGGL(k_pool_partial<__half>, grid, dim3(256), lds, stream, (const uint4*)feats, ld * esz / 16,
                               vpr, seg_start, split, pm, ps);
        else
            return PBN_ERR_ARG;
        hipLaunchKernelGGL(k_pool_final, dim3(cdiv((long long)n_seg * channels, 256)), dim3(256), 0, stream, pm, ps, seg_start,
                           n_seg, channels, split, out_max, out_avg);
        PBN_LAUNCH_CHECK();
        return PBN_OK;
    }
    const dim3 grid(n_seg, cdiv(channels, 32));
    switch (dtype) {
        case PBN_F32:
            hipLaunchKernelGGL(k_segment_pool<float>, grid, dim3(256), 0, stream, (const float*)feats, ld, channels,
                               seg_start, out_max, out_avg);
            break;
        case PBN_BF16:
            hipLaunchKernelGGL(k_segment_pool<__hip_bfloat16>, grid, dim3(256), 0, stream, (const __hip_bfloat16*)feats,
                               ld, channels, seg_start, out_max, out_avg);
            break;
        case PBN_F16:
            hipLaunchKernelGGL(k_segment_pool<__half>, grid, dim3(256), 0, stream, (const __half*)feats, ld, channels,
                               seg_start, out_max, out_avg);
            break;
        default: return PBN_ERR_ARG;
    }
    PBN_LAUNCH_CHECK();
    return PBN_OK;
}
```

pbnet_amd/csrc/stages.hip:

```cpp
#include <hip/hip_bf16.h>
#include <hip/hip_fp16.h>
#include "pbn_common.h"

namespace pbn {
namespace {

constexpr int TPB = 256;

__device__ __forceinline__ int upper_entry(const int* __restrict__ start, int n, int r) {
    int lo = 0, hi = n;
    while (hi - lo > 1) {
        const int mid = (lo + hi) >> 1;
        if (start[mid] <= r) lo = mid; else hi = mid;
    }
    return lo;
}

template <int ESZ>
__global__ __launch_bounds__(TPB) void k_local_scene_rows(
    const int* __restrict__ ent_row_start, const int* __restrict__ ent_member_start, const int* __restrict__ ent_scene,
    const float* __restrict__ ent_weight, int n_ent_cap, int n_rows_cap, const int* __restrict__ n_ent_dev,
    const int* __restrict__ n_rows_dev, const int* __restrict__ member_idx,
    const long long* __restrict__ ins_ind, const float* __restrict__ xyz, float inv_voxel,
    const unsigned char* __restrict__ point_feat, int ld_feat, int channels, const unsigned char* __restrict__ sem_score,
    int ld_sem, const long long* __restrict__ sem_pred, int dtype, long long* __restrict__ point_idx,
    long long* __restrict__ row_scene, int* __restrict__ coords, unsigned* __restrict__ feat_out, int words_per_row) {
    const int n_ent = n_ent_dev ? min(*n_ent_dev, n_ent_cap) : n_ent_cap;
    const int n_rows = n_rows_dev ? min(*n_rows_dev, n_rows_cap) : n_rows_cap;
    const long long e = (long long)blockIdx.x * TPB + threadIdx.x;
    if (e >= (long long)n_rows * words_per_row) return;
    const int r = (int)(e / words_per_row), w = (int)(e - (long long)r * words_per_row);
    const int ent = upper_entry(ent_row_start, n_ent, r);
    const int local = member_idx[ent_member_start[ent] + (r - ent_row_start[ent])];
    const long long p = ins_ind[local];
    if (w == 0) {
        point_idx[r] = p;
        row_scene[r] = ent_scene[ent];
        const float x = xyz[3 * p + 0] * inv_voxel, y = xyz[3 * p + 1] * inv_voxel, z = xyz[3 * p + 2] * inv_voxel;
        reinterpret_cast<int4*>(coords)[r] = make_int4(ent_scene[ent], (int)floorf(x), (int)floorf(y), (int)floorf(z));
    }
    constexpr int EPW = 4 / ESZ;
    unsigned out = 0;
#pragma unroll
    for (int k = 0; k < EPW; ++k) {
        const int c = w * EPW + k;
        unsigned bits = 0;
        if (c < channels) {
            if (ESZ == 4) bits = *reinterpret_cast<const unsigned*>(point_feat + ((size_t)p * ld_feat + c) * 4);
            else bits = *reinterpret_cast<const unsigned short*>(point_feat + ((size_t)p * ld_feat + c) * 2);
        } else if (c == channels) {
            const size_t o = (size_t)p * ld_sem + (sem_pred ? (size_t)sem_pred[p] : 0);
            if (ESZ == 4) bits = *reinterpret_cast<const unsigned*>(sem_score + o * 4);
            else bits = *reinterpret_cast<const unsigned short*>(sem_score + o * 2);
        } else if (c == channels + 1) {
            const float wt = ent_weight[ent];
            if (ESZ == 4) bits = __float_as_uint(wt);
            else if (dtype == PBN_BF16) bits = __builtin_bit_cast(unsigned short, __float2bfloat16(wt));
            else bits = __builtin_bit_cast(unsigned short, __float2half(wt));
        }
        out |= bits << (8 * ESZ * k);
    }
    feat_out[e] = out;
}

__global__ __launch_bounds__(TPB) void k_gather_pad_rows(const unsigned* __restrict__ in, int ld_in_w, int row_w,
                                                        const long long* __restrict__ idx,
                                                        const long long* __restrict__ idx2, int n_cap,
                                                        const int* __restrict__ n_dev, unsigned* __restrict__ out,
                                                        int ld_out_w) {
    const int n = n_dev ? min(*n_dev, n_cap) : n_cap;
    const long long e = (long long)blockIdx.x * TPB + threadIdx.x;
    if (e >= (long long)n * ld_out_w) return;
    const int i = (int)(e / ld_out_w), w = (int)(e - (long long)i * ld_out_w);
    unsigned v = 0;
    if (w < row_w) {
        long long r = idx ? idx[i] : i;
        if (idx2) r = idx2[r];
        v = in[(size_t)r * ld_in_w + w];
    }
    out[e] = v;
}


template <typename T> struct RowIO;
template <> struct RowIO<float> {
    static constexpr int E = 4;
    static __device__ __forceinline__ void unpack(const uint4& v, float* f) {
        f[0] = __uint_as_float(v.x); f[1] = __uint_as_float(v.y); f[2] = __uint_as_float(v.z); f[3] = __uint_as_float(v.w);
    }
    static __device__ __forceinline__ void store(float* p, float v) { *p = v; }
};
template <> struct RowIO<__hip_bfloat16> {
    static constexpr int E = 8;
    static __device__ __forceinline__ void unpack(const uint4& v, float* f) {
        const unsigned w[4] = {v.x, v.y, v.z, v.w};
#pragma unroll
        for (int i = 0; i < 4; ++i) { f[2 * i] = __uint_as_float(w[i] << 16); f[2 * i + 1] = __uint_as_float(w[i] & 0xffff0000u); }
    }
    static __device__ __forceinline__ void store(__hip_bfloat16* p, float v) { *p = __float2bfloat16(v); }
};
template <> struct RowIO<__half> {
    static constexpr int E = 8;
    static __device__ __forceinline__ void unpack(const uint4& v, float* f) {
        const unsigned w[4] = {v.x, v.y, v.z, v.w};
#pragma unroll
        for (int i = 0; i < 4; ++i) {
            const float2 t = __half22float2(__builtin_bit_cast(__half2, w[i]));
            f[2 * i] = t.x; f[2 * i + 1] = t.y;
        }
    }
    static __device__ __forceinline__ void store(__half* p, float v) { *p = __float2half(v); }
};

template <typename T, int C, int H>
__global__ __launch_bounds__(TPB) void k_mlp_rows(const T* __restrict__ in, int ld_in, const long long* __restrict__ idx_a,
                                                 const long long* __restrict__ idx_b, int n_cap,
                                                 const int* __restrict__ n_dev, long long in_rows,
                                                 const float* __restrict__ w1, const float* __restrict__ scale,
                                                 const float* __restrict__ shift, const float* __restrict__ slope,
                                                 const float* __restrict__ w2, const float* __restrict__ b2, int n_out,
                                                 int sigmoid, T* __restrict__ out, int ld_out) {
    constexpr int E = RowIO<T>::E;
    const int n = n_dev ? min(*n_dev, n_cap) : n_cap;
    const int i = blockIdx.x * TPB + threadIdx.x;
    if (i >= n) return;
    long long row = idx_a ? idx_a[i] : i;
    if (idx_b && row >= 0) row = idx_b[row];
    float x[C];
    const bool inside = row >= 0 && (in_rows < 0 || row < in_rows);
    const uint4* src = reinterpret_cast<const uint4*>(in + (size_t)(inside ? row : 0) * ld_in);
#pragma unroll
    for (int v = 0; v < C / E; ++v) {
        RowIO<T>::unpack(inside ? src[v] : make_uint4(0u, 0u, 0u, 0u), x + v * E);
    }
    float h[H];
#pragma unroll
    for (int k = 0; k < H; ++k) {
        float a = 0.f;
#pragma unroll
        for (int c = 0; c < C; ++c) a = fmaf(w1[k * C + c], x[c], a);
        a = fmaf(a, scale[k], shift[k]);
        h[k] = a >= 0.f ? a : a * slope[k];
    }
    for (int o = 0; o < n_out; ++o) {
        float a = b2 ? b2[o] : 0.f;
#pragma unroll
        for (int k = 0; k < H; ++k) a = fmaf(w2[o * H + k], h[k], a);
        if (sigmoid) a = 1.0f / (1.0f + expf(-a));
        RowIO<T>::store(out + (size_t)i * ld_out + o, a);
    }
}

typedef float mlp_f32x4 __attribute__((ext_vector_type(4)));
template <typename T, int H, int U>
__global__ __launch_bounds__(TPB) void k_mlp_rows_mfma(const T* __restrict__ in, int ld_in, const long long* __restrict__ idx_a,
                                                      const long long* __restrict__ idx_b, int n_cap,
                                                      const int* __restrict__ n_dev, long long in_rows,
                                                      const float* __restrict__ w1, const float* __restrict__ scale,
                                                      const float* __restrict__ shift, const float* __restrict__ slope,
                                                      const float* __restrict__ w2, const float* __restrict__ b2, int n_out,
                                                      int sigmoid, T* __restrict__ out, int ld_out) {
    constexpr int C = 32, HT = H / 16;
    const int n = n_dev ? min(*n_dev, n_cap) : n_cap;
    const int lane = threadIdx.x & 63, kq = lane >> 4, r = lane & 15;
    const int wave = (int)((blockIdx.x * TPB + threadIdx.x) >> 6), n_waves = (int)((gridDim.x * TPB) >> 6);
    float a1[HT][8];
#pragma unroll
    for (int t = 0; t < HT; ++t)
#pragma unroll
        for (int kb = 0; kb < 8; ++kb) a1[t][kb] = w1[(16 * t + r) * C + 8 * kq + kb];
    float sc[HT][4], sh[HT][4], sl[HT][4];
#pragma unroll
    for (int t = 0; t < HT; ++t)
#pragma unroll
        for (int i = 0; i < 4; ++i) {
            const int hh = 16 * t + 4 * kq + i;
            sc[t][i] = scale[hh]; sh[t][i] = shift[hh]; sl[t][i] = slope[hh];
        }
    float a2[U][HT][4];
    float bias[U][4];
#pragma unroll
    for (int u = 0; u < U; ++u) {
        const int o = 16 * u + r;
#pragma unroll
        for (int t = 0; t < HT; ++t)
#pragma unroll
            for (int i = 0; i < 4; ++i) a2[u][t][i] = o < n_out ? w2[o * H + 16 * t + 4 * kq + i] : 0.0f;
#pragma unroll
        for (int i = 0; i < 4; ++i) {
            const int oo = 16 * u + 4 * kq + i;
            bias[u][i] = (b2 && oo < n_out) ? b2[oo] : 0.0f;
        }
    }
    for (int blk = wave; blk * 16 < n; blk += n_waves) {
        const int i_row = blk * 16 + r;
        long long row = -1;
        if (i_row < n) {
            row = idx_a ? idx_a[i_row] : i_row;
            if (idx_b && row >= 0) row = idx_b[row];
        }
        const bool inside = row >= 0 && (in_rows < 0 || row < in_rows);
        float x[8];
        {
            const unsigned char* src = reinterpret_cast<const unsigned char*>(in + (size_t)(inside ? row : 0) * ld_in) + (size_t)kq * 8 * sizeof(T);
            if constexpr (sizeof(T) == 4) {
                const uint4 v0 = inside ? reinterpret_cast<const uint4*>(src)[0] : make_uint4(0u, 0u, 0u, 0u);
                const uint4 v1 = inside ? reinterpret_cast<const uint4*>(src)[1] : make_uint4(0u, 0u, 0u, 0u);
                RowIO<T>::unpack(v0, x);
                RowIO<T>::unpack(v1, x + 4);
            } else {
                RowIO<T>::unpack(inside ? reinterpret_cast<const uint4*>(src)[0] : make_uint4(0u, 0u, 0u, 0u), x);
            }
        }
        mlp_f32x4 d1[HT];
#pragma unroll
        for (int t = 0; t < HT; ++t) {
            d1[t] = mlp_f32x4{0.f, 0.f, 0.f, 0.f};
#pragma unroll
            for (int kb = 0; kb < 8; ++kb) d1[t] = __builtin_amdgcn_mfma_f32_16x16x4f32(a1[t][kb], x[kb], d1[t], 0, 0, 0);
#pragma unroll
            for (int i = 0; i < 4; ++i) {
                const float v = fmaf(d1[t][i], sc[t][i], sh[t][i]);
                d1[t][i] = v >= 0.f ? v : v * sl[t][i];
            }
        }
#pragma unroll
        for (int u = 0; u < U; ++u) {
            mlp_f32x4 d2 = mlp_f32x4{bias[u][0], bias[u][1], bias[u][2], bias[u][3]};
#pragma unroll
            for (int t = 0; t < HT; ++t)
#pragma unroll
                for (int i = 0; i < 4; ++i) d2 = __builtin_amdgcn_mfma_f32_16x16x4f32(a2[u][t][i], d1[t][i], d2, 0, 0, 0);
            if (i_row < n) {
// ... 215 lines not shown
        prop_ms[pos] = score[(size_t)i * ld];
        if (coords) {
            const float x = (xyz[3 * p + 0] * scale) * inv_voxel, y = (xyz[3 * p + 1] * scale) * inv_voxel,
                        z = (xyz[3 * p + 2] * scale) * inv_voxel;
            reinterpret_cast<int4*>(coords)[pos] = make_int4(dense, (int)floorf(x), (int)floorf(y), (int)floorf(z));
        }
        if (feat)
            for (int v = 0; v < vpr; ++v) feat[(size_t)pos * vpr + v] = point_feat[(size_t)p * ld_feat_vec + v];
        ++pos;
    }
}


__global__ __launch_bounds__(TPB) void k_gather_rulebook_rows(const unsigned* __restrict__ in, int ld_in_w, int row_w,
                                                             const int* __restrict__ nbr, int K, int k0, int kc, int n,
                                                             unsigned* __restrict__ out) {
    const long long e = (long long)blockIdx.x * TPB + threadIdx.x;
    const long long per_row = (long long)kc * row_w;
    if (e >= (long long)n * per_row) return;
    const int v = (int)(e / per_row);
    const int r = (int)(e - (long long)v * per_row);
    const int j = r / row_w, w = r - j * row_w;
    const int src = nbr[(size_t)v * K + k0 + j];
    out[e] = src >= 0 ? in[(size_t)src * ld_in_w + w] : 0u;
}


template <typename T>
__device__ __forceinline__ void pack_weight_element(const float* __restrict__ src, int K, int A, int B, int flip, int transpose,
                                                    int cin, int cout, int cin_p, int cout_p, long long e, T* __restrict__ out) {
    constexpr int E = 16 / (int)sizeof(T);
    const int ntt = cout_p / 16;
    const int j = (int)(e % E);
    const int lane = (int)((e / E) % 64);
    const int tt = (int)((e / (E * 64)) % ntt);
    const int st = (int)(e / ((long long)E * 64 * ntt));
    const int g = lane >> 4, c = lane & 15;
    const int r = st * 4 * E + g * E + j;
    const int k = r / cin_p, ci = r - k * cin_p;
    const int co = tt * 16 + c;
    float v = 0.f;
    if (k < K && ci < cin && co < cout) {
        const int ks = flip ? K - 1 - k : k;
        v = transpose ? src[((size_t)ks * A + co) * B + ci] : src[((size_t)ks * A + ci) * B + co];
    }
    RowIO<T>::store(out + e, v);
}

template <typename T>
__global__ __launch_bounds__(TPB) void k_pack_weight(const float* __restrict__ src, int K, int A, int B, int flip,
                                                    int transpose, int cin, int cout, int cin_p, int cout_p, int n_steps,
                                                    T* __restrict__ out) {
    constexpr int E = 16 / (int)sizeof(T);
    const long long e = (long long)blockIdx.x * TPB + threadIdx.x;
    const long long total = (long long)n_steps * (cout_p / 16) * 64 * E;
    if (e >= total) return;
    pack_weight_element<T>(src, K, A, B, flip, transpose, cin, cout, cin_p, cout_p, e, out);
}

template <typename T>
__global__ __launch_bounds__(TPB) void k_pack_weights_batch(const pbn_pack_job* __restrict__ jobs) {
    constexpr int E = 16 / (int)sizeof(T);
    const pbn_pack_job jb = jobs[blockIdx.y];
    const long long total = (long long)jb.n_steps * (jb.cout_p / 16) * 64 * E;
    for (long long e = (long long)blockIdx.x * TPB + threadIdx.x; e < total; e += (long long)gridDim.x * TPB)
        pack_weight_element<T>(jb.src, jb.n_offsets, jb.dim_a, jb.dim_b, jb.flip, jb.transpose, jb.cin, jb.cout, jb.cin_p,
                               jb.cout_p, e, (T*)jb.out);
}

}
}

using namespace pbn;

static int local_scene_rows_impl(const int32_t* ent_row_start, const int32_t* ent_member_start,
                                    const int32_t* ent_scene, const float* ent_weight, int n_ent, int n_rows,
                                    const int32_t* n_ent_dev, const int32_t* n_rows_dev,
                                    const int32_t* member_idx, const int64_t* ins_ind, const float* xyz, float inv_voxel,
                                    const void* point_feat, int ld_feat, int channels, const void* sem_score, int ld_sem,
                                    const int64_t* sem_pred, int dtype, int64_t* point_idx, int64_t* row_scene,
                                    int32_t* coords, void* feat_out, int ld_out, pbn_stream_t stream_) {
    hipStream_t stream = (hipStream_t)stream_;
    if (n_ent < 0 || n_rows < 0 || channels < 0 || ld_out < channels + 2 || ld_feat < channels) return PBN_ERR_ARG;
    if (n_rows == 0) return PBN_OK;
    if (n_ent == 0 || !ent_row_start || !ent_member_start || !ent_scene || !ent_weight || !member_idx || !ins_ind || !xyz ||
        !point_feat || !sem_score || !point_idx || !row_scene || !coords || !feat_out)
        return PBN_ERR_ARG;
    const int esz = dtype == PBN_F32 ? 4 : 2;
    if ((ld_out * esz) % 4 || ((uintptr_t)feat_out & 3) || ((uintptr_t)coords & 15)) return PBN_ERR_ARG;
    const int wpr = ld_out * esz / 4;
    const long long total = (long long)n_rows * wpr;
    const dim3 grid(cdiv(total, TPB));
#define PBN_ARGS                                                                                                        \
    ent_row_start, ent_member_start, ent_scene, ent_weight, n_ent, n_rows, n_ent_dev, n_rows_dev, member_idx,            \
        (const long long*)ins_ind, xyz,                                                                                  \
        inv_voxel, (const unsigned char*)point_feat, ld_feat, channels, (const unsigned char*)sem_score, ld_sem,         \
        (const long long*)sem_pred, dtype, (long long*)point_idx, (long long*)row_scene, coords, (unsigned*)feat_out, wpr
    if (esz == 4) hipLaunchKernelGGL(k_local_scene_rows<4>, grid, dim3(TPB), 0, stream, PBN_ARGS);
    else hipLaunchKernelGGL(k_local_scene_rows<2>, grid, dim3(TPB), 0, stream, PBN_ARGS);
#undef PBN_ARGS
    PBN_LAUNCH_CHECK();
    return PBN_OK;
}

extern "C" int pbn_local_scene_rows(const int32_t* ent_row_start, const int32_t* ent_member_start,
                                    const int32_t* ent_scene, const float* ent_weight, int n_ent, int n_rows,
                                    const int32_t* member_idx, const int64_t* ins_ind, const float* xyz, float inv_voxel,
                                    const void* point_feat, int ld_feat, int channels, const void* sem_score, int ld_sem,
                                    const int64_t* sem_pred, int dtype, int64_t* point_idx, int64_t* row_scene,
                                    int32_t* coords, void* feat_out, int ld_out, pbn_stream_t stream) {
    return local_scene_rows_impl(ent_row_start, ent_member_start, ent_scene, ent_weight, n_ent, n_rows, nullptr, nullptr,
                                 member_idx, ins_ind, xyz, inv_voxel, point_feat, ld_feat, channels, sem_score, ld_sem,
                                 sem_pred, dtype, point_idx, row_scene, coords, feat_out, ld_out, stream);
}

extern "C" int pbn_local_scene_rows_dev(const int32_t* ent_row_start, const int32_t* ent_member_start,
                                        const int32_t* ent_scene, const float* ent_weight, int n_ent_cap, int n_rows_cap,
                                        const int32_t* n_ent_dev, const int32_t* n_rows_dev, const int32_t* member_idx,
                                        const int64_t* ins_ind, const float* xyz, float inv_voxel, const void* point_feat,
                                        int ld_feat, int channels, const void* sem_score, int ld_sem,
                                        const int64_t* sem_pred, int dtype, int64_t* point_idx, int64_t* row_scene,
                                        int32_t* coords, void* feat_out, int ld_out, pbn_stream_t stream) {
    if (!n_ent_dev || !n_rows_dev) return PBN_ERR_ARG;
    return local_scene_rows_impl(ent_row_start, ent_member_start, ent_scene, ent_weight, n_ent_cap, n_rows_cap, n_ent_dev,
                                 n_rows_dev, member_idx, ins_ind, xyz, inv_voxel, point_feat, ld_feat, channels, sem_score,
                                 ld_sem, sem_pred, dtype, point_idx, row_scene, coords, feat_out, ld_out, stream);
}

static int gather_pad_rows_impl(const void* in, int ld_in_bytes, int row_bytes, const int64_t* idx, const int64_t* idx2,
                                int n, const int32_t* n_dev, void* out, int ld_out_bytes, pbn_stream_t stream_) {
    hipStream_t stream = (hipStream_t)stream_;
    if (n < 0 || row_bytes <= 0 || (row_bytes & 3) || (ld_in_bytes & 3) || (ld_out_bytes & 3) || ld_out_bytes < row_bytes ||
        ld_in_bytes < row_bytes)
        return PBN_ERR_ARG;
    if (n == 0) return PBN_OK;
    if (!in || !out || (((uintptr_t)in | (uintptr_t)out) & 3)) return PBN_ERR_ARG;
    const long long total = (long long)n * (ld_out_bytes / 4);
    hipLaunchKernelGGL(k_gather_pad_rows, dim3(cdiv(total, TPB)), dim3(TPB), 0, stream, (const unsigned*)in, ld_in_bytes / 4,
                       row_bytes / 4, (const long long*)idx, (const long long*)idx2, n, n_dev, (unsigned*)out,
                       ld_out_bytes / 4);
    PBN_LAUNCH_CHECK();
    return PBN_OK;
}

extern "C" int pbn_gather_pad_rows(const void* in, int ld_in_bytes, int row_bytes, const int64_t* idx, int n, void* out,
                                   int ld_out_bytes, pbn_stream_t stream) {
    return gather_pad_rows_impl(in, ld_in_bytes, row_bytes, idx, nullptr, n, nullptr, out, ld_out_bytes, stream);
}

extern "C" int pbn_gather_pad_rows_dev(const void* in, int ld_in_bytes, int row_bytes, const int64_t* idx,
                                       const int64_t* idx2, int n_cap, const int32_t* n_dev, void* out, int ld_out_bytes,
                                       pbn_stream_t stream) {
    return gather_pad_rows_impl(in, ld_in_bytes, row_bytes, idx, idx2, n_cap, n_dev, out, ld_out_bytes, stream);
}

static int mlp_rows_impl(const void* in, int ld_in, long long in_rows, int channels, const int64_t* idx_a, const int64_t* idx_b, int n,
                            const int32_t* n_dev, const float* w1, const float* scale, const float* shift, const float* slope, int hidden,
                            const float* w2, const float* b2, int n_out, int sigmoid, void* out, int ld_out, int dtype,
                            pbn_stream_t stream_) {
    hipStream_t stream = (hipStream_t)stream_;
    if (n < 0 || n_out < 1 || ld_out < n_out || ld_in < channels) return PBN_ERR_ARG;
    if (channels != 32 || (hidden != 16 && hidden != 32)) return PBN_ERR_UNSUPPORTED;
    if (n == 0) return PBN_OK;
    if (!in || !w1 || !scale || !shift || !slope || !w2 || !out) return PBN_ERR_ARG;
    const int esz = dtype == PBN_F32 ? 4 : 2;
    if ((ld_in * esz) % 16 || ((uintptr_t)in & 15)) return PBN_ERR_ARG;
    static const int form_env = getenv("PBN_MLP_FORM") ? atoi(getenv("PBN_MLP_FORM")) : 1;
    if (form_env != 0 && n_out <= 32) {
        const long long blocks16 = cdiv(n, 16);
        static const int bpw_env = getenv("PBN_MLP_BLOCKS") ? atoi(getenv("PBN_MLP_BLOCKS")) : 4;
        long long wgs = cdiv(blocks16, (TPB / 64) * (bpw_env > 0 ? bpw_env : 1));
        if (wgs > 8192) wgs = 8192;
        if (wgs < 1) wgs = 1;
        const dim3 g((unsigned)wgs);
#define PBN_MLPM(TT, HH, UU)                                                                                            \
        hipLaunchKernelGGL((k_mlp_rows_mfma<TT, HH, UU>), g, dim3(TPB), 0, stream, (const TT*)in, ld_in,                 \
                           (const long long*)idx_a, (const long long*)idx_b, n, n_dev, in_rows, w1, scale, shift, slope, w2, b2, \
                           n_out, sigmoid, (TT*)out, ld_out)
#define PBN_MLPM_T(TT)                                                                                                  \
        { if (hidden == 16) { if (n_out <= 16) PBN_MLPM(TT, 16, 1); else PBN_MLPM(TT, 16, 2); }                          \
          else { if (n_out <= 16) PBN_MLPM(TT, 32, 1); else PBN_MLPM(TT, 32, 2); } }
        if (dtype == PBN_F32) PBN_MLPM_T(float)
        else if (dtype == PBN_BF16) PBN_MLPM_T(__hip_bfloat16)
        else if (dtype == PBN_F16) PBN_MLPM_T(__half)
        else return PBN_ERR_ARG;
#undef PBN_MLPM_T
#undef PBN_MLPM
        PBN_LAUNCH_CHECK();
        return PBN_OK;
    }
    const dim3 grid(cdiv(n, TPB));
#define PBN_MLP(TT, HH)                                                                                                 \
    hipLaunchKernelGGL((k_mlp_rows<TT, 32, HH>), grid, dim3(TPB), 0, stream, (const TT*)in, ld_in,                        \
                       (const long long*)idx_a, (const long long*)idx_b, n, n_dev, in_rows, w1, scale, shift, slope, w2, b2, \
                       n_out,                                                                                            \
                       sigmoid, (TT*)out, ld_out)
    if (dtype == PBN_F32) { if (hidden == 16) PBN_MLP(float, 16); else PBN_MLP(float, 32); }
    else if (dtype == PBN_BF16) { if (hidden == 16) PBN_MLP(__hip_bfloat16, 16); else PBN_MLP(__hip_bfloat16, 32); }
    else if (dtype == PBN_F16) { if (hidden == 16) PBN_MLP(__half, 16); else PBN_MLP(__half, 32); }
    else return PBN_ERR_ARG;
#undef PBN_MLP
    PBN_LAUNCH_CHECK();
    return PBN_OK;
}

extern "C" int pbn_mlp_rows(const void* in, int ld_in, int channels, const int64_t* idx_a, const int64_t* idx_b, int n,
                            const float* w1, const float* scale, const float* shift, const float* slope, int hidden,
                            const float* w2, const float* b2, int n_out, int sigmoid, void* out, int ld_out, int dtype,
                            pbn_stream_t stream) {
    return mlp_rows_impl(in, ld_in, -1, channels, idx_a, idx_b, n, nullptr, w1, scale, shift, slope, hidden, w2, b2, n_out,
                         sigmoid, out, ld_out, dtype, stream);
}

extern "C" int pbn_mlp_rows_dev(const void* in, int ld_in, int in_rows, int channels, const int64_t* idx_a, const int64_t* idx_b,
                                int n_cap, const int32_t* n_dev, const float* w1, const float* scale, const float* shift,
                                const float* slope, int hidden, const float* w2, const float* b2, int n_out, int sigmoid,
                                void* out, int ld_out, int dtype, pbn_stream_t stream) {
    if (in_rows < 0) return PBN_ERR_ARG;
    return mlp_rows_impl(in, ld_in, in_rows, channels, idx_a, idx_b, n_cap, n_dev, w1, scale, shift, slope, hidden, w2, b2, n_out,
                         sigmoid, out, ld_out, dtype, stream);
}

extern "C" int pbn_select_blocks(int n) { return n > 0 ? cdiv(n, SEL_BLOCK) : 0; }

extern "C" int pbn_sem_argmax_table(const void* score, int ld, int n_cls, const int32_t* batch, int nb, int n, int dtype,
                                    int64_t* sem_pred, void* sem_prob, int32_t* table, int32_t* block_hist,
                                    pbn_stream_t stream_) {
    hipStream_t stream = (hipStream_t)stream_;
    if (n < 0 || n_cls < 1 || n_cls > SEL_MAX_CLASSES || nb < 1 || nb > PBN_MAX_SCENES || ld < n_cls || !table) return PBN_ERR_ARG;
    { const int frc_ = fill_bytes(table, 0, sizeof(int) * (size_t)n_cls * nb, stream); if (frc_ != PBN_OK) return frc_; }
    if (n == 0) return PBN_OK;
    if (!score || !sem_pred || !block_hist) return PBN_ERR_ARG;
    const dim3 grid(cdiv(n, SEL_BLOCK));
    if (dtype == PBN_F32)
        hipLaunchKernelGGL(k_sem_argmax_table<float>, grid, dim3(TPB), 0, stream, (const float*)score, ld, n_cls, batch, nb,
                           n, (long long*)sem_pred, (float*)sem_prob, table, block_hist);
    else if (dtype == PBN_BF16)
        hipLaunchKernelGGL(k_sem_argmax_table<__hip_bfloat16>, grid, dim3(TPB), 0, stream, (const __hip_bfloat16*)score, ld,
                           n_cls, batch, nb, n, (long long*)sem_pred, (__hip_bfloat16*)sem_prob, table, block_hist);
    else if (dtype == PBN_F16)
        hipLaunchKernelGGL(k_sem_argmax_table<__half>, grid, dim3(TPB), 0, stream, (const __half*)score, ld, n_cls, batch,
                           nb, n, (long long*)sem_pred, (__half*)sem_prob, table, block_hist);
    else
        return PBN_ERR_ARG;
    PBN_LAUNCH_CHECK();
    return PBN_OK;
}

extern "C" int pbn_select_points(const int64_t* sem_pred, int n, int n_cls, const int32_t* class_base,
                                 const int32_t* block_hist, const float* xyz, const void* offset, int ld_off, int dtype,
                                 int64_t* ins_ind, float* ins_orig, float* ins_off, int32_t* ins_sem,
                                 pbn_stream_t stream_) {
    hipStream_t stream = (hipStream_t)stream_;
    if (n < 0 || n_cls < 1 || n_cls > SEL_MAX_CLASSES || ld_off < 3) return PBN_ERR_ARG;
    if (n == 0) return PBN_OK;
    if (!sem_pred || !class_base || !block_hist || !xyz || !offset || !ins_ind || !ins_orig || !ins_off || !ins_sem)
        return PBN_ERR_ARG;
    const dim3 grid(cdiv(n, SEL_BLOCK));
    if (dtype == PBN_F32)
        hipLaunchKernelGGL(k_select_points<float>, grid, dim3(TPB), 0, stream, (const long long*)sem_pred, n, n_cls,
                           class_base, block_hist, xyz, (const float*)offset, ld_off, (long long*)ins_ind, ins_orig, ins_off,
                           ins_sem);
    else if (dtype == PBN_BF16)
        hipLaunchKernelGGL(k_select_points<__hip_bfloat16>, grid, dim3(TPB), 0, stream, (const long long*)sem_pred, n, n_cls,
                           class_base, block_hist, xyz, (const __hip_bfloat16*)offset, ld_off, (long long*)ins_ind, ins_orig,
                           ins_off, ins_sem);
    else if (dtype == PBN_F16)
        hipLaunchKernelGGL(k_select_points<__half>, grid, dim3(TPB), 0, stream, (const long long*)sem_pred, n, n_cls,
                           class_base, block_hist, xyz, (const __half*)offset, ld_off, (long long*)ins_ind, ins_orig, ins_off,
                           ins_sem);
    else
        return PBN_ERR_ARG;
    PBN_LAUNCH_CHECK();
    return PBN_OK;
}

static int mask_count_impl(const void* mask_score, int ld, float thd, const int64_t* row_scene, int n,
                           const int32_t* n_dev, int n_scenes, int dtype, int32_t* per_scene, int32_t* block_cnt,
                           pbn_stream_t stream_) {
    hipStream_t stream = (hipStream_t)stream_;
    if (n < 0 || n_scenes < 0 || ld < 1) return PBN_ERR_ARG;
    if (n_scenes > 0) {
        if (!per_scene) return PBN_ERR_ARG;
        { const int frc_ = fill_bytes(per_scene, 0, sizeof(int) * (size_t)n_scenes, stream); if (frc_ != PBN_OK) return frc_; }
    }
    if (n == 0) return PBN_OK;
    if (!mask_score || !row_scene || !block_cnt) return PBN_ERR_ARG;
    const dim3 grid(cdiv(n, SEL_BLOCK));
    if (dtype == PBN_F32)
        hipLaunchKernelGGL(k_mask_count<float>, grid, dim3(TPB), 0, stream, (const float*)mask_score, ld, thd,
                           (const long long*)row_scene, n, n_dev, n_scenes, per_scene, block_cnt);
    else if (dtype == PBN_BF16)
        hipLaunchKernelGGL(k_mask_count<__hip_bfloat16>, grid, dim3(TPB), 0, stream, (const __hip_bfloat16*)mask_score, ld,
                           thd, (const long long*)row_scene, n, n_dev, n_scenes, per_scene, block_cnt);
    else if (dtype == PBN_F16)
        hipLaunchKernelGGL(k_mask_count<__half>, grid, dim3(TPB), 0, stream, (const __half*)mask_score, ld, thd,
                           (const long long*)row_scene, n, n_dev, n_scenes, per_scene, block_cnt);
    else
        return PBN_ERR_ARG;
    PBN_LAUNCH_CHECK();
    return PBN_OK;
}

extern "C" int pbn_mask_count(const void* mask_score, int ld, float thd, const int64_t* row_scene, int n, int n_scenes,
                              int dtype, int32_t* per_scene, int32_t* block_cnt, pbn_stream_t stream) {
    return mask_count_impl(mask_score, ld, thd, row_scene, n, nullptr, n_scenes, dtype, per_scene, block_cnt, stream);
// ... 376 lines not shown
```

pbnet_amd/network/PBNet.py:

```python
import os
import threading
from types import SimpleNamespace

import numpy as np
import torch
import torch.nn as nn

from .. import MinkowskiEngine as ME
from .. import pbnet_ops
from .. import stage_ops
from ..prof import section, mark
from ..stage_ops import CNT
from .Mink import Mink_unet as unet3d

COUNT_MEAN = [-1., -1., 3917., 12056., 2303., 8331., 3948., 3166., 5629., 11719., 1003., 3317., 4912., 10221., 3889.,
              4136., 2120., 945., 3967., 2589.]
LOCAL_VOXEL = 0.02
HEAD_CLUSTERS = 256
MASK_THD = 0.45
TRAIN_FUSED_GLUE = os.environ.get("PBNET_TRAIN_FUSED_GLUE", "1") == "1"
DEVICE_FRONT = os.environ.get("PBNET_DEVICE_FRONT", "1") == "1"
FRONT_CLUSTER_CAP = 1024
FRONT_MAX_POINTS = int(os.environ.get("PBNET_DEVICE_FRONT_MAX_POINTS", "2000000"))


def _pack_entries(plan, dev):
    n_ent = len(plan.ent_np)
    row_start = np.zeros(n_ent + 1, dtype=np.int32)
    np.cumsum(plan.sizes[plan.ent_np], out=row_start[1:])
    ent_scene = np.repeat(np.arange(len(plan.scene_len), dtype=np.int32), plan.scene_len)
    packed = torch.from_numpy(np.concatenate([row_start, plan.member_start[:-1][plan.ent_np].astype(np.int32), ent_scene,
                                              np.asarray(plan.ent_weight, dtype=np.float32).view(np.int32)])).to(dev)
    return packed, n_ent, int(row_start[-1])


def _mlp(cin, mid, cout, sigmoid=False):
    layers = [ME.MinkowskiLinear(cin, mid, bias=False), ME.MinkowskiBatchNorm(mid), ME.MinkowskiPReLU(),
              ME.MinkowskiLinear(mid, cout, bias=True)]
    if sigmoid:
        layers.append(ME.MinkowskiSigmoid())
    return nn.Sequential(*layers)


class PBNet(nn.Module):
    def __init__(self, cfg):
        super().__init__()
        self.batch_size = cfg.batch_size
        self.cluster_batch = cfg.batch_size * 1
        self.sem_num = cfg.sem_num
        self.voxel_size = cfg.voxel_size
        self.scale_size = cfg.scale_size
        self.cluster_epoch = cfg.cluster_epoch
        self.radius = cfg.radius
        self.min_pts = cfg.min_pts
        self.method = getattr(cfg, "method", "PBNet")
        self.count_mean = torch.tensor(COUNT_MEAN)
        self.K_max = torch.ones(20, dtype=torch.float32) * 6
        self.MEUnet = unet3d(in_channels=6, out_channels=32, arch="MinkUNet34C")
        self.D_Unet = unet3d(in_channels=34, out_channels=32, arch="MinkUNet14A")
        self.score_Unet = unet3d(in_channels=32, out_channels=32, arch="MinkUNet34C")
        self.linear_sem = _mlp(32, 16, self.sem_num)
        self.linear_offset = _mlp(32, 16, 3)
        self.linear_binary = _mlp(32, 16, 1, sigmoid=True)
        self.global_max_pool = ME.MinkowskiGlobalMaxPooling()
        self.global_avg_pool = ME.MinkowskiGlobalAvgPooling()
        self.linear_IOU_feat = _mlp(32, 32, 32)
        self.linear_IOU = _mlp(32, 16, 1, sigmoid=True)
        self.soft_max = ME.MinkowskiSoftmax()
        self.weight_initialization()
        self.fix_module = []

    @property
    def _tls(self):
        t = self.__dict__.get("_tls_obj")
        if t is None:
            t = self.__dict__["_tls_obj"] = threading.local()
        return t

    def __getstate__(self):
        d = self.__dict__.copy()
        d.pop("_tls_obj", None)
        return d

    @property
    def _last_sizes(self):
        return self._tls.__dict__.setdefault("last_sizes", {})

    @_last_sizes.setter
    def _last_sizes(self, v):
        self._tls.last_sizes = v

    def weight_initialization(self):
        for m in self.modules():
            if isinstance(m, ME.MinkowskiConvolution):
                ME.utils.kaiming_normal_(m.kernel, mode="fan_out", nonlinearity="relu")
            if isinstance(m, ME.MinkowskiBatchNorm):
                nn.init.constant_(m.bn.weight, 1)
                nn.init.constant_(m.bn.bias, 0)

    def forward(self, feat_voxel, xyz_voxel, xyz_original, v2p_v1, ins_label, epoch, task="train", teacher=None, n_batch=None):
        dev = torch.device("cuda", torch.cuda.current_device())
        if feat_voxel.shape[0] == 0 or xyz_original.shape[0] == 0:
            raise ValueError("PBNet.forward: empty scene (0 voxels / 0 points)")
        fused = not torch.is_grad_enabled()
        nb = self.batch_size if task == "train" else (3 if n_batch is None else int(n_batch))
        stage1 = self.backbone_stage(feat_voxel.to(dev), xyz_voxel.to(dev), v2p_v1.to(dev), fused)
        if teacher is not None:
            stage1["sem_pred_score_p"] = teacher["sem_score"].to(dev, stage1["sem_pred_score_p"].dtype)
            stage1["offset_pred_p"] = teacher["offset"].to(dev, stage1["offset_pred_p"].dtype)
            if not fused:
                stage1["sem_pred_score_sfp"] = torch.softmax(stage1["sem_pred_score_p"].float(), 1).to(stage1["point_feat_p"].dtype)
                stage1["sem_pred_p"] = stage1["sem_pred_score_p"].max(1)[1]
        if fused:
            stage1["sem_pred_p"], stage1["sem_prob_p"], stage1["table"], stage1["block_hist"] = \
                stage_ops.sem_argmax_table(stage1["sem_pred_score_p"], stage1["batch_head_p"], nb)
        elif TRAIN_FUSED_GLUE and stage1["sem_pred_score_p"].is_cuda and epoch > self.cluster_epoch:
            with torch.no_grad():
                sc = stage1["sem_pred_score_p"].detach()
                stage1["sem_pred_p"], _, stage1["table"], stage1["block_hist"] = stage_ops.sem_argmax_table(
                    sc if sc.stride(1) == 1 else sc.contiguous(), stage1["batch_head_p"].to(torch.int32).contiguous(), nb)
        ret = {"sem_pred_p": stage1["sem_pred_p"], "sem_pred_score_p": stage1["sem_pred_score_p"],
               "offset_pred_p": stage1["offset_pred_p"]}
        if epoch > self.cluster_epoch:
            ret.update(self.cluster_stage(stage1, xyz_original.to(dev), None if ins_label is None else ins_label.to(dev),
                                          task, nb))
        return ret

    def backbone_stage(self, feat_voxel, xyz_voxel, v2p_v1, fused=False):
        with section("a3_coords"):
            inputs_v1 = ME.SparseTensor(feat_voxel, xyz_voxel)
        with section("a4_unet"):
            point_feat = self.MEUnet(inputs_v1)
        if fused:
            self._last_sizes = {"lv1": list(inputs_v1.coordinate_manager.row_counts())}
        with section("a5_heads_gather"):
            v2p = v2p_v1.long()
            if fused:
                f, row_index = point_feat.rows()
                if row_index is not None:
                    v2p = row_index[v2p]
                return {
                    "point_feat_p": f[v2p],
                    "sem_pred_score_p": stage_ops.mlp_rows(self.linear_sem, f, v2p),
                    "offset_pred_p": stage_ops.mlp_rows(self.linear_offset, f, v2p),
                    "batch_head_p": xyz_voxel[:, 0].to(torch.int32)[v2p_v1.long()],
                }
            sem_pred_score = self.linear_sem(point_feat)
            sem_pred_score_sf = self.soft_max(sem_pred_score)
            offsets_pred = self.linear_offset(point_feat)
            out = {
                "point_feat_p": point_feat.F[v2p],
                "sem_pred_score_p": sem_pred_score.F[v2p],
                "sem_pred_score_sfp": sem_pred_score_sf.F[v2p],
                "offset_pred_p": offsets_pred.F[v2p],
                "batch_head_p": xyz_voxel[:, 0][v2p],
            }
            out["sem_pred_p"] = out["sem_pred_score_p"].max(1)[1]
            return out

    def cluster_stage(self, s1, xyz_original, ins_label, task, n_batch=None):
        dev = xyz_original.device
        xyz_original = xyz_original.float()
        fused = "table" in s1
        infer = not torch.is_grad_enabled()
        train_glue = fused and not infer
        sem_pred_p, point_feat_p = s1["sem_pred_p"], s1["point_feat_p"]
        sem_sfp = s1["sem_prob_p"].view(-1, 1) if (fused and infer) else s1["sem_pred_score_sfp"]
        nb = n_batch if n_batch is not None else (self.batch_size if task == "train" else 3)
        self.cluster_batch = nb

        front = None
        if (DEVICE_FRONT and fused and infer and task == "test" and ins_label is None and xyz_original.is_contiguous()
                and xyz_original.shape[0] <= FRONT_MAX_POINTS):
            front = self._device_front(s1, xyz_original, nb)
            if isinstance(front, str):
                return self._empty_stage(dev, task)
        if front is not None:
            ins_ind, res, packed, n_ent, n_rows, n_clt, m = front
            n_scenes, scene_gt, plan = n_clt, None, None
            self._last_sizes["points"] = int(m)
        else:
            front = self._host_front(s1, xyz_original, ins_label, task, nb, fused, train_glue)
            if front is None:
                return self._empty_stage(dev, task)
            ins_ind, res, plan, n_clt = front
            n_scenes, scene_gt = len(plan.scene_len), plan.scene_gt

        with section("a17_gather"):
            if plan is not None and not (infer or train_glue):
                rows = self._rows_torch(plan, res, ins_ind, xyz_original, point_feat_p, sem_sfp, sem_pred_p)
            else:
                if plan is not None:
                    packed, n_ent, n_rows = _pack_entries(plan, dev)
                rows = self._rows_fused(packed, n_ent, n_rows, res, ins_ind, xyz_original, point_feat_p, sem_sfp,
                                        None if (fused and infer) else sem_pred_p)
                if train_glue:
                    rows = self._rows_train_glue(rows, point_feat_p, sem_sfp, sem_pred_p)
                elif fused:
                    self._last_sizes.update(clusters=int(n_clt), entries=int(n_ent), rows=int(n_rows))
            point_idx, row_scene, coords, feat = rows
        mark("a17:rows queued")

        out = {}
        with section("a18_mask_coords"):
            inputs_v2 = ME.SparseTensor(feat, coords)
        with section("a18_mask_unet"):
            if infer:
                f2, row_index = self.D_Unet(inputs_v2).rows()
                if fused:
                    self._last_sizes["lv2"] = list(inputs_v2.coordinate_manager.row_counts())
                mask_score = stage_ops.mlp_rows(self.linear_binary, f2, inputs_v2.inverse_mapping, row_index)
            else:
                mask_score = self.linear_binary(self.D_Unet(inputs_v2)).F[inputs_v2.inverse_mapping]
        if task != "test":
            gt_rows = torch.tensor(scene_gt, dtype=torch.long).to(dev)[row_scene]
            lab = ins_label[point_idx]
            gt_mask = (lab == gt_rows).long()
            gt_mask[lab == -100] = -1
            out["mask_scores"] = (mask_score, gt_mask.detach())
        mark("a18:mask unet queued")
        coords3 = feat3 = None
        with section("a19_proposals"):
            if infer:
                out["proposals"], coords3, feat3 = self._proposals_fused(row_scene, point_idx, mask_score, n_scenes,
                                                                         xyz_original, point_feat_p)
            elif train_glue:
                with torch.no_grad():
                    out["proposals"], coords3, _ = self._proposals_fused(row_scene, point_idx, mask_score.detach(), n_scenes,
                                                                         xyz_original, point_feat_p.detach())
                feat3 = point_feat_p[out["proposals"][0][:, 1]]
            else:
                out["proposals"] = self.get_proposal(row_scene, point_idx, mask_score, n_scenes=n_scenes)
        mark("a19:proposals queued")
        out["clt_scores"] = self._score_branch(out["proposals"], coords3, feat3, xyz_original, point_feat_p, fused, infer)
        mark("a20:score branch queued")
        return out

    def _score_branch(self, proposals, coords3, feat3, xyz_original, point_feat_p, fused, infer):
        proposals_idx, proposals_offset, _, _ = proposals
        if proposals_offset.shape[0] <= 1:
            return torch.zeros(0, dtype=torch.float32, device=xyz_original.device)
        if coords3 is None:
            pidx = proposals_idx[:, 1]
            c3 = torch.floor(xyz_original[pidx] * self.scale_size / self.voxel_size).to(torch.int32)
            coords3 = torch.cat([proposals_idx[:, 0:1].to(torch.int32), c3], 1)
            feat3 = point_feat_p[pidx]
        with section("a20_score_coords"):
            inputs_v3 = ME.SparseTensor(feat3, coords3)
        with section("a20_score_unet"):
            if infer:
                iou_feat_f = stage_ops.mlp_rows(self.linear_IOU_feat, *self.score_Unet(inputs_v3).rows())
                if fused:
                    self._last_sizes["lv3"] = list(inputs_v3.coordinate_manager.row_counts())
            else:
                iou_feat = self.linear_IOU_feat(self.score_Unet(inputs_v3))
        with section("a20_pool_head"):
            if not infer:
                from ..MinkowskiEngine.nn import global_max_plus_avg_pool
                global_feat = global_max_plus_avg_pool(iou_feat) if iou_feat.F.is_cuda else \
                    self.global_max_pool(iou_feat) + self.global_avg_pool(iou_feat)
                return self.linear_IOU(global_feat).F.view(-1)
            from ..MinkowskiEngine.nn import segment_pool
            n_prop = int(proposals_offset.shape[0]) - 1
            mx, av = segment_pool(iou_feat_f, inputs_v3.C[:, 0], n_prop)
            return stage_ops.mlp_rows(self.linear_IOU, (mx + av).to(iou_feat_f.dtype)).view(-1)

    def _rows_fused(self, packed, n_ent, n_rows, res, ins_ind, xyz_original, point_feat_p, sem_sfp, sem_pred_p):
        with torch.no_grad():
            return stage_ops.local_scene_rows(packed, n_ent, n_rows, res.member_idx, ins_ind, xyz_original, LOCAL_VOXEL,
                                              point_feat_p.detach(), sem_sfp.detach(), sem_pred_p)

    def _rows_train_glue(self, rows, point_feat_p, sem_sfp, sem_pred_p):
        point_idx, row_scene, coords, feat = rows
        row_sem_sf = sem_sfp[point_idx, sem_pred_p[point_idx]]
        feat = torch.cat([point_feat_p[point_idx], row_sem_sf.view(-1, 1).to(point_feat_p.dtype), feat[:, -1:]], 1)
        return point_idx, row_scene, coords, feat

    def _rows_torch(self, plan, res, ins_ind, xyz_original, point_feat_p, sem_sfp, sem_pred_p):
        dev = xyz_original.device
        ent_cluster_t = torch.from_numpy(plan.ent_np)
        ent_rows = torch.from_numpy(plan.sizes.astype(np.int64))[ent_cluster_t]
        member_start = torch.from_numpy(plan.member_start)
        ent_scene = torch.repeat_interleave(torch.arange(len(plan.scene_len)), torch.tensor(plan.scene_len))
        d = lambda t: t.to(dev)
        row_ent = torch.repeat_interleave(torch.arange(len(plan.ent_np), device=dev), d(ent_rows))
        ent_first = d(torch.cumsum(ent_rows, 0) - ent_rows)
        pos_in_ent = torch.arange(row_ent.shape[0], device=dev) - ent_first[row_ent]
        member_pos = d(member_start[:-1][ent_cluster_t])[row_ent] + pos_in_ent
        local_idx = res.member_idx[member_pos].long()
        point_idx = ins_ind[local_idx]
        row_scene = d(ent_scene)[row_ent]
        row_weight = d(torch.tensor(plan.ent_weight, dtype=torch.float32))[row_ent]
        row_sem_sf = sem_sfp[point_idx, sem_pred_p[point_idx]]
        feat = torch.cat([point_feat_p[point_idx], row_sem_sf.view(-1, 1).to(point_feat_p.dtype),
                          row_weight.view(-1, 1).to(point_feat_p.dtype)], 1)
        coords = torch.cat([row_scene.view(-1, 1).to(torch.int32),
                            torch.floor(xyz_original[point_idx] / LOCAL_VOXEL).to(torch.int32)], 1)
        return point_idx, row_scene, coords, feat

    def _host_select(self, s1, xyz_original, nb, fused):
        dev = xyz_original.device
        n_cls = int(self.sem_num)
        sem_pred_p, offset_pred_p = s1["sem_pred_p"], s1["offset_pred_p"]
        if fused:
            table = s1["table"]
        else:
            batch_head_p = s1["batch_head_p"].long()
            table = torch.bincount(sem_pred_p * nb + batch_head_p, minlength=n_cls * nb)[:n_cls * nb].view(n_cls, nb)
        mark("a6:before table sync")
        tab = table.cpu().numpy()
        mark("a6:table on host")
        assert int(tab.sum()) == sem_pred_p.shape[0], "batch index outside [0, cluster_batch)"
        per_class = tab.sum(1).tolist()
        thr05, _ = self._class_thresholds()
        classes = [c for c in range(2, n_cls) if not (float(per_class[c]) < thr05[c])]
        if not classes:
            return None
        m = sum(per_class[c] for c in classes)
        seg_len_h = tab[classes].reshape(-1).astype(np.int32)
        if fused:
            class_base = np.full(n_cls, -1, dtype=np.int32)
            run = 0
            for c in classes:
                class_base[c] = run
                run += per_class[c]
            up = torch.from_numpy(np.concatenate([class_base, seg_len_h])).to(dev)
            with torch.no_grad():
                selected = stage_ops.select_points(sem_pred_p, up[:n_cls], s1["block_hist"], xyz_original,
                                                   offset_pred_p.detach(), m)
            return (classes, m) + selected + (up[n_cls:],)
        keep = torch.zeros(n_cls, dtype=torch.bool)
        keep[classes] = True
        key = torch.where(keep.to(dev)[sem_pred_p], sem_pred_p, torch.full_like(sem_pred_p, n_cls))
        order = torch.sort(key, stable=True)[1]
        ins_ind = order[:m]
        ins_orig = xyz_original[ins_ind]
        ins_offseted = ins_orig + offset_pred_p[ins_ind].float()
        return classes, m, ins_ind, ins_orig, ins_offseted, sem_pred_p[ins_ind].to(torch.int32), torch.from_numpy(seg_len_h).to(dev)

    def _host_front(self, s1, xyz_original, ins_label, task, nb, fused, train_glue):
        with section("a6_select"):
            sel = self._host_select(s1, xyz_original, nb, fused)
        if sel is None:
            return None
        classes, m, ins_ind, ins_orig, ins_offseted, ins_sem, seg_len = sel
        if fused and not train_glue:
            self._last_sizes["points"] = int(m)
        mark("a7:select queued")
        with section("a7_16_grouping"):
            res = pbnet_ops.cluster_device(ins_offseted, ins_orig, ins_sem, seg_len, self.radius, self.min_pts,
                                          need_den=False)
            mark("a7:grouping queued")
            n_seg = int(res.cluster_num.shape[0])
            hc = min(HEAD_CLUSTERS, int(res.member_start.shape[0]) - 1)
            head = torch.cat([res.n_clusters, res.cluster_num, res.member_start[:hc + 1],
                              res.centers[:3 * hc].view(torch.int32)]).cpu().numpy()
            mark("a7:grouping done")
            n_clt = int(head[0])
        if n_clt < 0:
            raise RuntimeError("grouping rejected its input (class id outside [2,19])")
        if n_clt == 0:
            return None
        with section("a17_plan"):
            cluster_num = head[1:1 + n_seg].reshape(len(classes), nb).tolist()
            if n_clt <= hc:
                member_start = head[1 + n_seg:1 + n_seg + n_clt + 1]
                centers = torch.from_numpy(head[2 + n_seg + hc:2 + n_seg + hc + 3 * n_clt].view(np.float32).copy()).view(n_clt, 3)
            else:
                packed = torch.cat([res.centers[:3 * n_clt], res.member_start[:n_clt + 1].view(torch.float32)]).cpu()
                centers = packed[:3 * n_clt].view(n_clt, 3)
                member_start = packed[3 * n_clt:].view(torch.int32).numpy()
            mark("a17:centres on host")
            labels_h = None
            if task != "test":
                labels_h = ins_label[ins_ind[res.member_idx[:int(member_start[-1])].long()]].cpu()
            plan = self._host_plan(classes, nb, cluster_num, centers, member_start, labels_h)
            if plan is None:
                return None
        mark("a17:plan done")
        return ins_ind, res, plan, n_clt

    def _host_plan(self, classes, nb, cluster_num, centers, member_start, labels_h):
        sizes = (member_start[1:] - member_start[:-1])
        sizes_l = sizes.tolist()
        _, thr02 = self._class_thresholds()
        ent_cluster, ent_weight, scene_len, scene_gt = [], [], [], []
        k_max = self._k_max_list()
        g = 0
        for ci, cls in enumerate(classes):
            for b in range(nb):
                c_b = cluster_num[ci][b]
                if c_b == 0:
                    continue
                para_k = min(c_b - 1, k_max[cls])
                if para_k > 0:
                    peak_v = [0.5 * ((para_k + 1) - p_i) / (para_k + 1) for p_i in range(para_k + 1)]
                    ctr = centers[g:g + c_b]
                    knn_idx = torch.cdist(ctr, ctr).topk(k=c_b, dim=1, largest=False)[1].tolist()
                big = thr02[cls]
                for c_i in range(c_b):
                    gid = g + c_i
                    gt = None
                    if labels_h is not None:
                        gt = int(torch.mode(labels_h[int(member_start[gid]):int(member_start[gid + 1])])[0])
                        if gt == -100:
                            continue
                    ents, wts = [gid], [1.0]
                    if float(sizes_l[gid]) > big and para_k > 0:
                        row = knn_idx[c_i]
                        for k_i in range(para_k):
                            ents.append(g + row[k_i + 1])
                            wts.append(peak_v[k_i])
                    ent_cluster += ents
                    ent_weight += wts
                    scene_len.append(len(ents))
                    scene_gt.append(gt)
                g += c_b
        if not scene_len:
            return None
        return SimpleNamespace(ent_np=np.asarray(ent_cluster, dtype=np.int64), ent_weight=ent_weight, scene_len=scene_len,
                               scene_gt=scene_gt, sizes=sizes, member_start=member_start)

    def _front_consts(self, dev):
        consts = self.__dict__.setdefault("_front_consts_cache", {})
        c = consts.get(dev)
        if c is None:
            thr05, thr02 = self._class_thresholds()
            f32 = dict(dtype=torch.float32, device=dev)
            c = consts[dev] = (torch.tensor(thr05, **f32), torch.tensor(thr02, **f32),
                               torch.tensor(self._k_max_list(), dtype=torch.int32, device=dev))
        return c

    def _front_launches(self, table, sem_pred, block_hist, xyz, offset, nb, m_cap, c_cap, e_cap, r_cap, counts):
        thr05, thr02, kmax = self._front_consts(xyz.device)
        with section("a6_select"):
            class_base, seg_len = stage_ops.class_gate(table, thr05, nb, m_cap, int(xyz.shape[0]), counts)
            ins_ind, ins_orig, ins_off, ins_sem = stage_ops.select_points(sem_pred, class_base, block_hist, xyz, offset.detach(),
                                                                          m_cap)
        mark("a7:select queued")
        with section("a7_16_grouping"):
            res = pbnet_ops.cluster_device(ins_off, ins_orig, ins_sem, seg_len, self.radius, self.min_pts, capacity=True,
                                          need_den=False)
            ent = stage_ops.local_plan(res, nb, thr02, kmax, c_cap, e_cap, r_cap, counts)
            mark("a7:grouping queued")
        return ins_ind, res, ent

    def _device_front(self, s1, xyz_original, nb):
        n_pts = int(xyz_original.shape[0])
        c_cap = min(FRONT_CLUSTER_CAP, n_pts)
        counts = torch.zeros(CNT.WORDS, dtype=torch.int32, device=xyz_original.device)
        ins_ind, res, ent = self._front_launches(s1["table"], s1["sem_pred_p"], s1["block_hist"], xyz_original,
                                                 s1["offset_pred_p"], nb, n_pts, c_cap, 7 * c_cap, 2 ** 31 - 1, counts)
        h = torch.cat([counts, res.n_clusters]).cpu().tolist()
        mark("a7:grouping done")
        if h[CNT.WORDS] < 0:
            raise RuntimeError("grouping rejected its input (class id outside [2,19])")
        if h[CNT.OVERFLOW] & 32:
            raise AssertionError("batch index outside [0, cluster_batch)")
        if h[CNT.OVERFLOW]:
            return None
        m, n_clt, n_ent, n_rows = h[CNT.POINTS], h[CNT.CLUSTERS], h[CNT.ENTRIES], h[CNT.ROWS]
        if m == 0 or n_clt == 0 or n_ent == 0:
            return "empty"
        return ins_ind, res, ent.compact(n_ent), n_ent, n_rows, n_clt, m

    def _class_thresholds(self):
        hit = getattr(self, "_thr_cache", None)
        if hit is None:
            hit = ((self.count_mean * 0.05).tolist(), (self.count_mean * 0.2).tolist())
            self._thr_cache = hit
        return hit

    def _k_max_list(self):
        hit = getattr(self, "_kmax_cache", None)
        if hit is None:
            hit = [int(v) for v in self.K_max.tolist()]
            self._kmax_cache = hit
        return hit

    def _empty_stage(self, dev, task):
        z = torch.zeros(0, dtype=torch.int64, device=dev)
        out = {"proposals": (torch.zeros(0, 2, dtype=torch.int64, device=dev), torch.zeros(1, dtype=torch.int64, device=dev),
                             z, torch.zeros(0, device=dev)),
               "clt_scores": torch.zeros(0, device=dev)}
        if task != "test":
            out["mask_scores"] = (torch.zeros(0, 1, device=dev), z)
        return out

    def _proposals_fused(self, row_scene, point_idx, mask_score, n_scenes, xyz_original, point_feat_p,
                         mask_score_thd=MASK_THD):
        dev = row_scene.device
        per_scene_d, block_cnt = stage_ops.mask_count(mask_score, mask_score_thd, row_scene, n_scenes)
        mark("a19:before count sync")
        per_scene = per_scene_d.cpu().numpy().astype(np.int64)
        mark("a19:counts on host")
        total = int(per_scene.sum())
        alive = per_scene > 0
        n_alive = int(alive.sum())
        proposals_offset = np.zeros(n_alive + 1, dtype=np.int64)
        np.cumsum(per_scene[alive], out=proposals_offset[1:])
        dense_of = (np.cumsum(alive) - 1).astype(np.int32)
        up64 = torch.from_numpy(np.concatenate([proposals_offset, np.nonzero(alive)[0].astype(np.int64)])).to(dev)
        dense_of = torch.from_numpy(dense_of).to(dev)
        prop_idx, prop_ms, coords3, feat3 = stage_ops.proposal_rows(
            mask_score, mask_score_thd, row_scene, point_idx, dense_of, block_cnt, total, xyz_original,
            self.scale_size, self.voxel_size, point_feat_p)
        return (prop_idx, up64[:n_alive + 1], up64[n_alive + 1:], prop_ms), coords3, feat3

    def get_proposal(self, row_scene, point_idx, mask_score, mask_score_thd=MASK_THD, n_scenes=None):
        assert row_scene.shape[0] == mask_score.shape[0]
        dev = row_scene.device
        if n_scenes is None:
            n_scenes = int(row_scene.max().item()) + 1 if row_scene.numel() else 0
        keep = mask_score.view(-1).float() > mask_score_thd
        per_scene = torch.bincount(row_scene[keep], minlength=n_scenes).cpu()
        total = int(per_scene.sum())
        valid = torch.nonzero_static(keep, size=total).view(-1)
        proposals_ms = mask_score[valid].view(-1)
        alive = per_scene > 0
        cluster_id_v = torch.nonzero(alive).view(-1)
        proposals_offset = torch.zeros(int(alive.sum()) + 1, dtype=torch.int64)
        proposals_offset[1:] = torch.cumsum(per_scene[alive], 0)
        dense_of = torch.cumsum(alive.to(torch.int64), 0) - 1
        dense = dense_of.to(dev)[row_scene[valid]]
        proposals_idx = torch.stack([dense, point_idx[valid]], 1).to(torch.int64)
        return proposals_idx.detach(), proposals_offset.to(dev), cluster_id_v.to(dev), proposals_ms


def model_losses(ret, sem_label, ins_label, instance_info, instance_pointnum, xyz_original, epoch, cfg, get_iou=None):
    sem_pred_score_p, offset_pred_p = ret["sem_pred_score_p"].float(), ret["offset_pred_p"].float()
    semantic_loss = nn.CrossEntropyLoss(ignore_index=-100)(sem_pred_score_p, sem_label)
    gt_offsets = instance_info[:, 0:3] - xyz_original
    pt_dist = torch.sum(torch.abs(offset_pred_p - gt_offsets), dim=-1)
    valid = (ins_label != -100).float()
    offset_norm_loss = torch.sum(pt_dist * valid) / (torch.sum(valid) + 1e-6)
    gt_dir = gt_offsets / (torch.norm(gt_offsets, p=2, dim=1).unsqueeze(-1) + 1e-8)
    pt_dir = offset_pred_p / (torch.norm(offset_pred_p, p=2, dim=1).unsqueeze(-1) + 1e-8)
    offset_dir_loss = torch.sum(-(gt_dir * pt_dir).sum(-1) * valid) / (torch.sum(valid) + 1e-6)
    loss = semantic_loss + offset_norm_loss + offset_dir_loss
    parts = {"semantic_loss": semantic_loss, "offset_norm_loss": offset_norm_loss, "offset_dir_loss": offset_dir_loss}
    weight = gt_mask = None
    if epoch > cfg.cluster_epoch:
        pred_mask, gt_mask = ret["mask_scores"]
        pred_mask = pred_mask.float()
        weight = (gt_mask != -1).float()
        gt_mask[gt_mask == -1] = 0
        mask_loss = nn.BCELoss(reduction="none", weight=weight)(pred_mask.view(-1), gt_mask.float()).mean()
        dice_loss = diceLoss(pred_mask.view(-1), gt_mask.view(-1))
        proposals_idx, proposals_offset, _, _ = ret["proposals"]
        if get_iou is None:
            from .. import pbnet_ops as ops
            get_iou = ops.get_iou
        ious = get_iou(proposals_idx[:, 1].contiguous(), proposals_offset, ins_label, instance_pointnum)
        gt_ious, _ = ious.max(1)
        gt_scores = get_segmented_scores(gt_ious, cfg.fg_thresh, cfg.bg_thresh)
        score_loss = nn.BCELoss()(ret["clt_scores"].float().view(-1), gt_scores).mean()
        loss = loss + mask_loss + dice_loss + score_loss
        parts.update(mask_loss=mask_loss, dice_loss=dice_loss, score_loss=score_loss)
    parts["loss"] = loss
    return loss, parts, valid, weight, gt_mask


def model_fn(batch, model, epoch, cfg, task="train"):
    xyz_original = batch["xyz_original"].cuda()
    ins_label = batch["ins"].cuda()
    ret = model(batch["feat_voxel"], batch["xyz_voxel"], xyz_original, batch["v2p_index"], ins_label, epoch, task)
    sem_label = batch["sem"].cuda()
    instance_info = batch["inst_info"].cuda()
    instance_pointnum = batch["instance_pointnum"].cuda()
    offset_pred_p, sem_pred_p = ret["offset_pred_p"].float(), ret["sem_pred_p"]
    if getattr(cfg, "native_losses", False):
        from ..losses import model_losses_native as losses_fn
    else:
        losses_fn = model_losses
    loss, parts, valid, weight, gt_mask = losses_fn(ret, sem_label, ins_label, instance_info, instance_pointnum,
                                                    xyz_original.float(), epoch, cfg)
    with torch.no_grad():
        pred = {"sem": sem_pred_p, "offseted_xyz": xyz_original + offset_pred_p}
        names = ["loss", "semantic_loss", "offset_norm_loss", "offset_dir_loss"] + (["mask_loss"] if epoch > cfg.cluster_epoch else [])
        host = torch.stack([parts[k].detach().float().reshape(()) for k in names])
        host = host.unbind(0) if getattr(cfg, "device_meters", False) else host.tolist()
        visual_dict = dict(zip(names[:4], host[:4]))
        meter_dict = {k: (v, valid.sum()) for k, v in visual_dict.items()}
        if epoch > cfg.cluster_epoch:
            visual_dict["mask_loss"] = host[4]
            meter_dict["mask_loss"] = (visual_dict["mask_loss"], weight.sum())
            pred["mask_scores"] = ret["mask_scores"]
            pred["proposals"] = ret["proposals"]
            pred["clt_scores"] = ret["clt_scores"]
    return loss, pred, visual_dict, meter_dict


def model_fn_eval(batch, model, epoch, cfg, task="test", teacher=None, n_batch=None):
    ret = model(batch["feat_voxel"], batch["xyz_voxel"], batch["xyz_original"], batch["v2p_index"], None, epoch, task,
                teacher=teacher, n_batch=n_batch)
    pred = {"sem": ret["sem_pred_p"]}
    if epoch > cfg.cluster_epoch:
        pred["proposals"] = ret["proposals"]
        pred["clt_scores"] = ret["clt_scores"]
    return pred


def get_segmented_scores(scores, fg_thresh=1.0, bg_thresh=0.0):
    fg_mask = scores > fg_thresh
    bg_mask = scores < bg_thresh
    interval_mask = (fg_mask == 0) & (bg_mask == 0)
    out = (fg_mask > 0).float()
    k = 1 / (fg_thresh - bg_thresh)
    b = bg_thresh / (bg_thresh - fg_thresh)
    out[interval_mask] = scores[interval_mask] * k + b
    return out


def diceLoss(mask_pred, mask_gt, ep=1e-8):
    inter = 2 * (mask_gt * mask_pred).sum() + 1
    union = (mask_gt ** 2.0).sum() + (mask_pred ** 2.0).sum() + 1 + ep
    return 1 - inter / union
```

pbnet_amd/pbnet_ops.py:

```python
import torch
from torch.autograd import Function

from . import _native as N

PARA_F = 0.05
NV_FLAG = True


class ClusterResult(object):
    __slots__ = ("cluster_id", "cluster_num", "den", "centers", "clt_sem", "n_clusters", "member_start",
                 "member_idx")

    def __init__(self, **kw):
        for k, v in kw.items():
            setattr(self, k, v)


def cluster_device(off_xyz, org_xyz, sem, seg_len, radius, min_pts, para_f=PARA_F, nv_flag=NV_FLAG,
                   general_sem=False, want_members=True, capacity=False, need_den=True):
    N.require_cuda(off_xyz, org_xyz, sem, seg_len)
    off_xyz = off_xyz.to(torch.float32).contiguous()
    org_xyz = org_xyz.to(torch.float32).contiguous()
    sem = sem.to(torch.int32).contiguous()
    seg_len = seg_len.to(torch.int32).contiguous()
    n = int(off_xyz.shape[0])
    b = int(seg_len.shape[0])
    dev = off_xyz.device
    i32 = dict(dtype=torch.int32, device=dev)
    cluster_id = torch.empty(n, **i32)
    cluster_num = torch.empty(b, **i32)
    den = torch.empty(n, **i32)
    centers = torch.empty(3 * max(n, 1), dtype=torch.float32, device=dev)
    clt_sem = torch.empty(max(n, 1), **i32)
    n_clusters = torch.empty(1, **i32)
    member_start = torch.empty(n + 1, **i32) if want_members else None
    member_idx = torch.empty(max(n, 1), **i32) if want_members else None
    lib = N.lib()
    ws_bytes = lib.pbn_cluster_workspace_bytes(n, b, int(bool(general_sem)))
    ws = torch.empty(max(ws_bytes, 1), dtype=torch.uint8, device=dev)
    rc = lib.pbn_binary_cluster(N.ptr(off_xyz), N.ptr(org_xyz), N.ptr(sem), N.ptr(seg_len), n, b, float(radius),
                                int(min_pts), float(para_f), int(bool(nv_flag)), int(bool(general_sem)) | (2 if capacity else 0) | (0 if need_den else 4),
                                N.ptr(cluster_id), N.ptr(cluster_num), N.ptr(den), N.ptr(centers), N.ptr(clt_sem),
                                N.ptr(n_clusters), N.ptr(member_start), N.ptr(member_idx), N.ptr(ws), ws_bytes,
                                N.current_stream())
    N.check(rc, "pbn_binary_cluster")
    return ClusterResult(cluster_id=cluster_id, cluster_num=cluster_num, den=den, centers=centers, clt_sem=clt_sem,
                         n_clusters=n_clusters, member_start=member_start, member_idx=member_idx)


class Cluster(Function):

    @staticmethod
    def forward(ctx, ins_offseted, ins_orig, sem, ins_bp, radius, min_pts, batch_size):
        out_dev = ins_offseted.device
        dev = out_dev if out_dev.type == "cuda" else torch.device("cuda", torch.cuda.current_device())
        sem_d = sem.to(dev)
        uniform = True
        if sem_d.numel() > 0:
            uniform = bool((sem_d == sem_d[0]).all().item())
        res = cluster_device(ins_offseted.to(dev), ins_orig.to(dev), sem_d, ins_bp.to(dev)[:batch_size], radius,
                             min_pts, general_sem=not uniform, want_members=False)
        c = int(res.n_clusters.item())
        if c < 0:
            raise RuntimeError("pbnet_ops.cluster: invalid input (segment lengths do not sum to the number of points, "
                               "or a class id outside [2,19])")
        center = res.centers[:3 * c]
        return (res.cluster_id.to(out_dev), res.cluster_num.to(out_dev), (res.den + 1).to(out_dev),
                center.to(out_dev))

    @staticmethod
    def backward(ctx, a=None, b=None, c=None, d=None):
        return None, None, None, None, None, None, None


cluster = Cluster.apply


def get_iou_device(proposals_idx, proposals_offset, instance_labels, instance_pointnum):
    N.require_cuda(proposals_idx, proposals_offset, instance_labels, instance_pointnum)
    n_inst = int(instance_pointnum.size(0))
    n_prop = int(proposals_offset.size(0)) - 1
    idx = proposals_idx.to(torch.int32).contiguous()
    off = proposals_offset.to(torch.int32).contiguous()
    lab = instance_labels.to(torch.int64).contiguous()
    pnum = instance_pointnum.to(torch.int32).contiguous()
    iou = torch.zeros(max(n_prop, 0), n_inst, dtype=torch.float32, device=idx.device)
    rc = N.lib().pbn_get_iou(N.ptr(idx), N.ptr(off), N.ptr(lab), N.ptr(pnum), N.ptr(iou), n_inst, n_prop,
                             N.current_stream())
    N.check(rc, "pbn_get_iou")
    return iou


class GetIoU(Function):

    @staticmethod
    def forward(ctx, proposals_idx, proposals_offset, instance_labels, instance_pointnum):
        assert proposals_idx.is_contiguous() and proposals_idx.is_cuda
        assert proposals_offset.is_contiguous() and proposals_offset.is_cuda
        assert instance_labels.is_contiguous() and instance_labels.is_cuda
        assert instance_pointnum.is_contiguous() and instance_pointnum.is_cuda
        return get_iou_device(proposals_idx, proposals_offset, instance_labels, instance_pointnum)

    @staticmethod
    def backward(ctx, a=None):
        return None, None, None, None


get_iou = GetIoU.apply


class CalIoUAndMasklabel(Function):

    @staticmethod
    def forward(ctx, proposals_idx, proposals_offset, instance_labels, instance_pointnum, mask_scores_sigmoid, mode):
        N.require_cuda(proposals_idx, proposals_offset, instance_labels, instance_pointnum, mask_scores_sigmoid)
        n_inst = int(instance_pointnum.size(0))
        n_prop = int(proposals_offset.size(0)) - 1
        idx = proposals_idx.to(torch.int32).contiguous()
        off = proposals_offset.to(torch.int32).contiguous()
        lab = instance_labels.to(torch.int64).contiguous()
        pnum = instance_pointnum.to(torch.int32).contiguous()
        ms = mask_scores_sigmoid.to(torch.float32).contiguous()
        iou = torch.zeros(n_prop, n_inst, dtype=torch.float32, device=idx.device)
        mask_label = torch.full(ms.shape, -1.0, dtype=torch.float32, device=idx.device)
        rc = N.lib().pbn_cal_iou_and_masklabel(N.ptr(idx), N.ptr(off), N.ptr(lab), N.ptr(pnum), N.ptr(iou), n_inst,
                                               n_prop, N.ptr(ms), N.ptr(mask_label), int(mode), N.current_stream())
        N.check(rc, "pbn_cal_iou_and_masklabel")
        return iou, mask_label

    @staticmethod
    def backward(ctx, a=None, b=None):
        return None, None, None, None, None, None


cal_iou_and_masklabel = CalIoUAndMasklabel.apply


def get_normal_line(xyz, face):
    raise NotImplementedError("cal_normal_line is offline preprocessing outside the MI355X hot path (SURVEY.md 2 #7)")
```

pbnet_amd/stage_ops.py:

```python
from types import SimpleNamespace

import numpy as np
import torch

from . import _native as N

_DT = N.DT
CNT = SimpleNamespace(POINTS=0, CLUSTERS=1, ENTRIES=2, ROWS=3, SCENES=4, PROPOSAL_ROWS=5, PROPOSALS=6, OVERFLOW=7, WORDS=16)
OVF_NAMES = {1: "selected points", 2: "clusters", 4: "local-scene entries", 8: "local-scene rows",
             16: "clusters of one (class, batch) segment", 32: "batch index outside [0, cluster_batch)", 64: "rows of a level",
             128: "a segment of more than 25 clusters (torch.cdist ranks through its matrix-multiply path: host plan)"}


def reciprocal_f32(x):
    return float(np.float32(1.0) / np.float32(x))


class EntryTable(object):

    def __init__(self, buf, n):
        assert buf.dtype == torch.int32 and buf.numel() == 4 * n + 1 and buf.is_contiguous()
        self.buf, self.n = buf, int(n)

    row_start = property(lambda self: self.buf[:self.n + 1])
    member_start = property(lambda self: self.buf[self.n + 1:2 * self.n + 1])
    scene = property(lambda self: self.buf[2 * self.n + 1:3 * self.n + 1])
    weight = property(lambda self: self.buf[3 * self.n + 1:].view(torch.float32))

    def pointers(self):
        base, n = self.buf.data_ptr(), self.n
        return tuple(N.c_vp(base + 4 * (k * n + 1)) if k else N.c_vp(base) for k in range(4))

    def compact(self, n_ent):
        return torch.cat([self.buf[:n_ent + 1]] + [self.buf[k * self.n + 1:k * self.n + 1 + n_ent] for k in (1, 2, 3)])


def local_scene_rows(packed, n_ent, n_rows, member_idx, ins_ind, xyz, voxel, point_feat, sem_score, sem_pred, ld_out=None,
                     n_ent_dev=None, n_rows_dev=None):
    ent = packed if isinstance(packed, EntryTable) else EntryTable(packed, n_ent)
    N.require_cuda(ent.buf, member_idx, ins_ind, xyz, point_feat, sem_score)
    dev = point_feat.device
    c = int(point_feat.shape[1])
    ld_out = c + 2 if ld_out is None else int(ld_out)
    assert ent.n == n_ent and (n_ent_dev is None) == (n_rows_dev is None)
    assert point_feat.stride(1) == 1 and sem_score.stride(1) == 1 and sem_score.dtype == point_feat.dtype
    assert xyz.dtype == torch.float32 and xyz.is_contiguous() and ins_ind.dtype == torch.int64
    assert member_idx.dtype == torch.int32 and (sem_pred is None or sem_pred.dtype == torch.int64)
    point_idx = torch.empty(n_rows, dtype=torch.int64, device=dev)
    row_scene = torch.empty(n_rows, dtype=torch.int64, device=dev)
    coords = torch.empty(n_rows, 4, dtype=torch.int32, device=dev)
    feat = torch.empty(n_rows, ld_out, dtype=point_feat.dtype, device=dev)
    vp = N.c_vp
    head = ent.pointers() + (int(n_ent), int(n_rows))
    rest = (N.ptr(member_idx), N.ptr(ins_ind), N.ptr(xyz), reciprocal_f32(voxel),
            vp(point_feat.data_ptr()), point_feat.stride(0), c, vp(sem_score.data_ptr()), sem_score.stride(0),
            N.ptr(sem_pred), _DT[point_feat.dtype], N.ptr(point_idx), N.ptr(row_scene), N.ptr(coords),
            vp(feat.data_ptr()), ld_out, N.current_stream())
    if n_ent_dev is None:
        rc = N.lib().pbn_local_scene_rows(*(head + rest))
    else:
        rc = N.lib().pbn_local_scene_rows_dev(*(head + (N.ptr(n_ent_dev), N.ptr(n_rows_dev)) + rest))
    N.check(rc, "pbn_local_scene_rows")
    return point_idx, row_scene, coords, feat


def gather_pad_rows(feats, width, idx=None, idx2=None, n=None, n_dev=None):
    N.require_cuda(feats, idx, idx2)
    es = feats.element_size()
    if n is None:
        n = int(idx.shape[0]) if idx is not None else int(feats.shape[0])
    assert feats.stride(1) == 1 and feats.shape[1] <= width and (idx2 is None or n_dev is not None)
    out = torch.empty(n, width, dtype=feats.dtype, device=feats.device)
    vp = N.c_vp
    src = (vp(feats.data_ptr()), feats.stride(0) * es, int(feats.shape[1]) * es, N.ptr(idx))
    dst = (vp(out.data_ptr()), width * es, N.current_stream())
    if n_dev is None:
        rc = N.lib().pbn_gather_pad_rows(*(src + (int(n),) + dst))
    else:
        rc = N.lib().pbn_gather_pad_rows_dev(*(src + (N.ptr(idx2), int(n), N.ptr(n_dev)) + dst))
    N.check(rc, "pbn_gather_pad_rows")
    return out


class _HeadParams(object):

    def __init__(self):
        self.key = None

    def get(self, head):
        lin1, bn, act, lin2 = head[0].linear, head[1].bn, head[2].module, head[3].linear
        tensors = [lin1.weight, bn.weight, bn.bias, bn.running_mean, bn.running_var, act.weight, lin2.weight, lin2.bias]
        key = tuple((t.data_ptr(), t._version) for t in tensors if t is not None)
        if key != self.key:
            with torch.no_grad():
                f = lambda t: t.detach().float().contiguous()
                scale = f(bn.weight) / torch.sqrt(f(bn.running_var) + bn.eps)
                shift = f(bn.bias) - f(bn.running_mean) * scale
                hidden = lin1.weight.shape[0]
                self.w1 = f(lin1.weight)
                self.scale, self.shift = scale.contiguous(), shift.contiguous()
                self.slope = f(act.weight).expand(hidden).contiguous()
                self.w2 = f(lin2.weight)
                self.b2 = f(lin2.bias) if lin2.bias is not None else None
                self.hidden, self.n_out, self.channels = int(hidden), int(lin2.weight.shape[0]), int(lin1.weight.shape[1])
                self.sigmoid = len(head) > 4
                assert lin1.bias is None
            self.key = key
        return self


_HEADS = {}


def mlp_rows(head, feats, idx_a=None, idx_b=None, n=None, n_dev=None, in_rows=None):
    hp = _HEADS.setdefault(id(head), _HeadParams()).get(head)
    N.require_cuda(feats)
    assert feats.stride(1) == 1 and feats.shape[1] == hp.channels
    if n is None:
        n = int(idx_a.shape[0]) if idx_a is not None else int(feats.shape[0])
    out = torch.empty(n, hp.n_out, dtype=feats.dtype, device=feats.device)
    vp = N.c_vp
    rest = (N.ptr(hp.w1), N.ptr(hp.scale), N.ptr(hp.shift), N.ptr(hp.slope), hp.hidden, N.ptr(hp.w2), N.ptr(hp.b2), hp.n_out,
            int(hp.sigmoid), vp(out.data_ptr()), hp.n_out, _DT[feats.dtype], N.current_stream())
    if n_dev is None:
        rc = N.lib().pbn_mlp_rows(vp(feats.data_ptr()), feats.stride(0), hp.channels, N.ptr(idx_a), N.ptr(idx_b), int(n), *rest)
    else:
        rc = N.lib().pbn_mlp_rows_dev(vp(feats.data_ptr()), feats.stride(0), int(feats.shape[0] if in_rows is None else in_rows),
                                      hp.channels, N.ptr(idx_a), N.ptr(idx_b), int(n), N.ptr(n_dev), *rest)
    N.check(rc, "pbn_mlp_rows")
    return out


def sem_argmax_table(score, batch, nb):
    N.require_cuda(score)
    n, s = int(score.shape[0]), int(score.shape[1])
    dev = score.device
    assert score.stride(1) == 1 and (batch is None or (batch.dtype == torch.int32 and batch.is_contiguous()))
    lib = N.lib()
    sem_pred = torch.empty(n, dtype=torch.int64, device=dev)
    sem_prob = torch.empty(n, dtype=score.dtype, device=dev)
    table = torch.empty(s, nb, dtype=torch.int32, device=dev)
    block_hist = torch.empty(max(lib.pbn_select_blocks(n), 1), s, dtype=torch.int32, device=dev)
    rc = lib.pbn_sem_argmax_table(N.c_vp(score.data_ptr()), score.stride(0), s, N.ptr(batch), int(nb), n, _DT[score.dtype],
                                  N.ptr(sem_pred), N.c_vp(sem_prob.data_ptr()), N.ptr(table), N.ptr(block_hist),
                                  N.current_stream())
    N.check(rc, "pbn_sem_argmax_table")
    return sem_pred, sem_prob, table, block_hist


def select_points(sem_pred, class_base, block_hist, xyz, offset, m):
    N.require_cuda(sem_pred, class_base, block_hist, xyz, offset)
    dev = xyz.device
    n, s = int(sem_pred.shape[0]), int(class_base.shape[0])
    assert xyz.dtype == torch.float32 and xyz.is_contiguous() and offset.stride(1) == 1 and class_base.dtype == torch.int32
    ins_ind = torch.empty(m, dtype=torch.int64, device=dev)
    ins_orig = torch.empty(m, 3, dtype=torch.float32, device=dev)
    ins_off = torch.empty(m, 3, dtype=torch.float32, device=dev)
    ins_sem = torch.empty(m, dtype=torch.int32, device=dev)
    rc = N.lib().pbn_select_points(N.ptr(sem_pred), n, s, N.ptr(class_base), N.ptr(block_hist), N.ptr(xyz),
                                   N.c_vp(offset.data_ptr()), offset.stride(0), _DT[offset.dtype], N.ptr(ins_ind),
                                   N.ptr(ins_orig), N.ptr(ins_off), N.ptr(ins_sem), N.current_stream())
    N.check(rc, "pbn_select_points")
    return ins_ind, ins_orig, ins_off, ins_sem


def class_gate(table, thr05, nb, m_cap, n_points, counts):
    N.require_cuda(table, thr05, counts)
    s = int(table.shape[0])
    assert table.dtype == torch.int32 and thr05.dtype == torch.float32 and thr05.shape[0] == s and counts.numel() == CNT.WORDS
    class_base = torch.empty(s, dtype=torch.int32, device=table.device)
    seg_len = torch.empty((s - 2) * nb, dtype=torch.int32, device=table.device)
    rc = N.lib().pbn_class_gate(N.ptr(table), N.ptr(thr05), s, int(nb), int(m_cap), int(n_points), N.ptr(class_base),
                                N.ptr(seg_len), N.ptr(counts), N.current_stream())
    N.check(rc, "pbn_class_gate")
    return class_base, seg_len


def local_plan(res, nb, thr02, kmax, c_cap, e_cap, r_cap, counts):
    N.require_cuda(res.cluster_num, thr02, kmax, counts)
    assert thr02.dtype == torch.float32 and kmax.dtype == torch.int32 and counts.dtype == torch.int32
    dev, lib = counts.device, N.lib()
    ent = EntryTable(torch.empty(4 * e_cap + 1, dtype=torch.int32, device=dev), e_cap)
    ws_bytes = int(lib.pbn_local_plan_workspace_bytes(int(c_cap)))
    ws = torch.empty(ws_bytes, dtype=torch.uint8, device=dev)
    rc = lib.pbn_local_plan(N.ptr(res.cluster_num), int(res.cluster_num.shape[0]), int(nb), N.ptr(res.member_start),
                            N.ptr(res.centers), N.ptr(res.n_clusters), N.ptr(thr02), N.ptr(kmax), int(c_cap), int(e_cap),
                            int(r_cap), *(ent.pointers() + (N.ptr(counts), N.ptr(ws), ws_bytes, N.current_stream())))
    N.check(rc, "pbn_local_plan")
    return ent


def mask_count(mask_score, thd, row_scene, n_scenes, n_dev=None):
    N.require_cuda(mask_score, row_scene)
    n = int(row_scene.shape[0])
    dev = mask_score.device
    lib = N.lib()
    ms = mask_score.view(n, -1) if n else mask_score.view(0, 1)
    assert ms.stride(1) == 1 and row_scene.dtype == torch.int64
    per_scene = torch.empty(max(n_scenes, 1), dtype=torch.int32, device=dev)
    block_cnt = torch.empty(max(lib.pbn_select_blocks(n), 1), dtype=torch.int32, device=dev)
    src = (N.c_vp(ms.data_ptr()), ms.stride(0), float(thd), N.ptr(row_scene), n)
    rest = (int(n_scenes), _DT[ms.dtype], N.ptr(per_scene), N.ptr(block_cnt), N.current_stream())
    rc = lib.pbn_mask_count(*(src + rest)) if n_dev is None else lib.pbn_mask_count_dev(*(src + (N.ptr(n_dev),) + rest))
    N.check(rc, "pbn_mask_count")
    return per_scene[:n_scenes], block_cnt


def proposal_offsets(per_scene, counts):
    N.require_cuda(per_scene, counts)
    s_cap, dev = int(per_scene.shape[0]), per_scene.device
    assert per_scene.dtype == torch.int32 and counts.numel() == CNT.WORDS
    proposals_offset = torch.zeros(s_cap + 1, dtype=torch.int64, device=dev)
    alive_ids = torch.zeros(s_cap, dtype=torch.int64, device=dev)
    dense_of = torch.empty(s_cap, dtype=torch.int32, device=dev)
    rc = N.lib().pbn_proposal_offsets(N.ptr(per_scene), s_cap, N.ptr(proposals_offset), N.ptr(alive_ids), N.ptr(dense_of),
                                      N.ptr(counts), N.current_stream())
    N.check(rc, "pbn_proposal_offsets")
    return proposals_offset, alive_ids, dense_of


def proposal_rows(mask_score, thd, row_scene, point_idx, dense_of, block_cnt, total, xyz=None, scale=1.0, voxel=1.0,
                  point_feat=None, n_dev=None):
    n = int(row_scene.shape[0])
    dev = mask_score.device
    ms = mask_score.view(n, -1) if n else mask_score.view(0, 1)
    prop_idx = torch.empty(total, 2, dtype=torch.int64, device=dev)
    prop_ms = torch.empty(total, dtype=ms.dtype, device=dev)
    coords = torch.empty(total, 4, dtype=torch.int32, device=dev) if xyz is not None else None
    feat = None
    c = ld_feat = 0
    if point_feat is not None:
        assert point_feat.stride(1) == 1 and point_feat.dtype == ms.dtype
        c, ld_feat = int(point_feat.shape[1]), point_feat.stride(0)
        feat = torch.empty(total, c, dtype=point_feat.dtype, device=dev)
    if total == 0:
        return prop_idx, prop_ms, coords, feat
    vp = N.c_vp
    src = (vp(ms.data_ptr()), ms.stride(0), float(thd), N.ptr(row_scene), N.ptr(point_idx), n)
    rest = (N.ptr(dense_of), N.ptr(block_cnt), N.ptr(xyz), float(np.float32(scale)), reciprocal_f32(voxel),
            None if point_feat is None else vp(point_feat.data_ptr()), ld_feat, c, _DT[ms.dtype], N.ptr(prop_idx),
            vp(prop_ms.data_ptr()), N.ptr(coords), None if feat is None else vp(feat.data_ptr()), N.current_stream())
    lib = N.lib()
    rc = lib.pbn_proposal_rows(*(src + rest)) if n_dev is None else lib.pbn_proposal_rows_dev(*(src + (N.ptr(n_dev),) + rest))
    N.check(rc, "pbn_proposal_rows")
    return prop_idx, prop_ms, coords, feat


def batch_starts(coords, n_cap, n_dev, n_segments):
    N.require_cuda(coords)
    assert coords.dtype == torch.int32 and coords.shape[1] == 4
    seg_start = torch.empty(n_segments + 1, dtype=torch.int32, device=coords.device)
    rc = N.lib().pbn_batch_starts(N.ptr(coords), N.ptr(n_dev), int(n_cap), int(n_segments), N.ptr(seg_start),
                                  N.current_stream())
    N.check(rc, "pbn_batch_starts")
    return seg_start
```

Before: 362.8.

## Fuse pooling sum, point-row gather, counter clearing and host uploads into fewer launches

Adds a segment-pool-sum entry that computes segment starts on device by binary search and writes max plus average straight into the output dtype. It also adds a fused point-rows gather kernel and a class-gate variant that clears the counter block itself, which removes a separate zeros fill. Counts and n_clusters now share one buffer so a single device-to-host copy replaces a concat plus copy, and the proposal metadata is packed into one host-to-device upload. The entry-table compact step is dropped and the final pooling reduction is unrolled; the aim is fewer small launches and transfers, at the cost of more API surface and relaxed asserts.

```diff
diff --git a/include/pbnet_hip.h b/include/pbnet_hip.h
--- a/include/pbnet_hip.h
+++ b/include/pbnet_hip.h
@@ -88,6 +88,9 @@
 size_t pbn_segment_pool_workspace_bytes(int n_seg, int channels);
 int pbn_segment_pool(const void* feats, int ld, int channels, int dtype, const int32_t* seg_start, int n_seg,
                      float* out_max, float* out_avg, void* workspace, size_t workspace_bytes, pbn_stream_t stream);
+size_t pbn_segment_pool_sum_workspace_bytes(int n_seg, int channels);
+int pbn_segment_pool_sum(const void* feats, int ld, int channels, int dtype, const int32_t* seg_ids, int ld_ids, int n_rows,
+                         int n_seg, void* out_sum, void* workspace, size_t workspace_bytes, pbn_stream_t stream);
 
 int pbn_local_scene_rows(const int32_t* ent_row_start, const int32_t* ent_member_start, const int32_t* ent_scene,
                          const float* ent_weight, int n_ent, int n_rows, const int32_t* member_idx,
@@ -97,6 +100,9 @@
                          pbn_stream_t stream);
 int pbn_gather_pad_rows(const void* in, int ld_in_bytes, int row_bytes, const int64_t* idx, int n, void* out,
                         int ld_out_bytes, pbn_stream_t stream);
+int pbn_point_rows(const void* v2p, int v2p_is_i64, const int64_t* row_index, const void* coords, int coords_is_i64,
+                   int ld_coords, int n_voxels, int n_rows, int n, const void* feats, int ld_feat_bytes, int row_bytes,
+                   int64_t* idx, int32_t* batch, void* out, pbn_stream_t stream);
 
 int pbn_pack_weight(const float* src, int n_offsets, int dim_a, int dim_b, int flip, int transpose, int dtype,
                     int vecs_per_offset, int n_steps, int cout_padded, void* out, pbn_stream_t stream);
@@ -177,6 +183,8 @@
 };
 int pbn_class_gate(const int32_t* table, const float* thr05, int n_classes, int nb, int m_cap, int n_points,
                    int32_t* class_base, int32_t* seg_len, int32_t* counts, pbn_stream_t stream);
+int pbn_class_gate_first(const int32_t* table, const float* thr05, int n_classes, int nb, int m_cap, int n_points,
+                         int32_t* class_base, int32_t* seg_len, int32_t* counts, pbn_stream_t stream);
 size_t pbn_local_plan_workspace_bytes(int c_cap);
 int pbn_local_plan(const int32_t* cluster_num, int n_segments, int nb, const int32_t* member_start, const float* centers,
                    const int32_t* n_clusters, const float* thr02, const int32_t* kmax, int c_cap, int e_cap, int r_cap,
diff --git a/pbnet_amd/MinkowskiEngine/nn.py b/pbnet_amd/MinkowskiEngine/nn.py
--- a/pbnet_amd/MinkowskiEngine/nn.py
+++ b/pbnet_amd/MinkowskiEngine/nn.py
@@ -238,6 +238,22 @@
     return mx, av
 
 
+def segment_pool_sum(feats, coords, n_batch):
+    from .. import _native as N
+    N.require_cuda(feats, coords)
+    assert feats.stride(1) == 1 and coords.dtype == torch.int32 and coords.dim() == 2 and coords.shape[0] == feats.shape[0]
+    c = int(feats.shape[1])
+    out = torch.empty(n_batch, c, dtype=feats.dtype, device=feats.device)
+    lib = N.lib()
+    ws_bytes = int(lib.pbn_segment_pool_sum_workspace_bytes(int(n_batch), c))
+    ws = torch.empty(max(ws_bytes, 16), dtype=torch.uint8, device=feats.device)
+    rc = lib.pbn_segment_pool_sum(N.c_vp(feats.data_ptr()), feats.stride(0), c, _DT[feats.dtype], N.c_vp(coords.data_ptr()),
+                                  coords.stride(0), int(coords.shape[0]), int(n_batch), N.c_vp(out.data_ptr()),
+                                  N.c_vp(ws.data_ptr()), ws_bytes, N.current_stream())
+    N.check(rc, "pbn_segment_pool_sum")
+    return out
+
+
 class _SegmentPoolFn(torch.autograd.Function):
 
     @staticmethod
diff --git a/pbnet_amd/_native.py b/pbnet_amd/_native.py
--- a/pbnet_amd/_native.py
+++ b/pbnet_amd/_native.py
@@ -140,6 +140,10 @@
     "pbn_gather_rows": (c_int, [c_vp, c_int, c_vp, c_int, c_int, c_vp, c_int, c_vp]),
     "pbn_segment_pool_workspace_bytes": (c_size, [c_int, c_int]),
     "pbn_segment_pool": (c_int, [c_vp, c_int, c_int, c_int, c_i32p, c_int, c_f32p, c_f32p, c_vp, c_size, c_vp]),
+    "pbn_segment_pool_sum_workspace_bytes": (c_size, [c_int, c_int]),
+    "pbn_segment_pool_sum": (c_int, [c_vp, c_int, c_int, c_int, c_i32p, c_int, c_int, c_int, c_vp, c_vp, c_size, c_vp]),
+    "pbn_point_rows": (c_int, [c_vp, c_int, c_vp, c_vp, c_int, c_int, c_int, c_int, c_int, c_vp, c_int, c_int, c_vp, c_i32p,
+                               c_vp, c_vp]),
     "pbn_local_scene_rows": (c_int, [c_i32p, c_i32p, c_i32p, c_f32p, c_int, c_int, c_i32p, c_vp, c_f32p, c_float, c_vp,
                                      c_int, c_int, c_vp, c_int, c_vp, c_int, c_vp, c_vp, c_i32p, c_vp, c_int, c_vp]),
     "pbn_gather_pad_rows": (c_int, [c_vp, c_int, c_int, c_vp, c_int, c_vp, c_int, c_vp]),
@@ -219,6 +223,7 @@
                                      ctypes.POINTER(ctypes.c_void_p), ctypes.POINTER(ctypes.c_void_p), c_vp, c_size, c_int,
                                      c_vp, c_size, c_vp]),
     "pbn_class_gate": (c_int, [c_i32p, c_f32p, c_int, c_int, c_int, c_int, c_i32p, c_i32p, c_i32p, c_vp]),
+    "pbn_class_gate_first": (c_int, [c_i32p, c_f32p, c_int, c_int, c_int, c_int, c_i32p, c_i32p, c_i32p, c_vp]),
     "pbn_local_plan_workspace_bytes": (c_size, [c_int]),
     "pbn_local_plan": (c_int, [c_i32p, c_int, c_int, c_i32p, c_f32p, c_i32p, c_f32p, c_i32p, c_int, c_int, c_int, c_i32p,
                                c_i32p, c_i32p, c_f32p, c_i32p, c_vp, c_size, c_vp]),
diff --git a/pbnet_amd/csrc/plan.hip b/pbnet_amd/csrc/plan.hip
--- a/pbnet_amd/csrc/plan.hip
+++ b/pbnet_amd/csrc/plan.hip
@@ -15,6 +15,7 @@
     return v;
 }
 
+template <bool CLEAR>
 __global__ __launch_bounds__(64) void k_class_gate(const int* __restrict__ table, const float* __restrict__ thr05, int n_cls,
                                                   int nb, int m_cap, int n_points, int* __restrict__ class_base,
                                                   int* __restrict__ seg_len, int* __restrict__ counts) {
@@ -36,7 +37,10 @@
     if (lane < n_cls) class_base[lane] = (keep && !drop_all) ? incl - kept : -1;
     if (lane >= 2 && lane < n_cls)
         for (int b = 0; b < nb; ++b) seg_len[(lane - 2) * nb + b] = (keep && !drop_all) ? table[lane * nb + b] : 0;
-    if (lane == 0) {
+    if (CLEAR) {
+        if (lane < PBN_CNT_WORDS)
+            counts[lane] = lane == PBN_CNT_POINTS ? (drop_all ? 0 : m) : (lane == PBN_CNT_OVERFLOW ? flags : 0);
+    } else if (lane == 0) {
         counts[PBN_CNT_POINTS] = drop_all ? 0 : m;
         if (flags) atomicOr(&counts[PBN_CNT_OVERFLOW], flags);
     }
@@ -249,14 +253,28 @@
 
 using namespace pbn;
 
+static int class_gate_impl(const int32_t* table, const float* thr05, int n_classes, int nb, int m_cap, int n_points,
+                           int32_t* class_base, int32_t* seg_len, int32_t* counts, bool clear, pbn_stream_t stream) {
+    if (!table || !thr05 || !class_base || !seg_len || !counts || n_classes < 3 || n_classes > 64 || nb < 1 || m_cap < 0)
+        return PBN_ERR_ARG;
+    if (clear)
+        hipLaunchKernelGGL(k_class_gate<true>, dim3(1), dim3(64), 0, (hipStream_t)stream, table, thr05, n_classes, nb, m_cap,
+                           n_points, class_base, seg_len, counts);
+    else
+        hipLaunchKernelGGL(k_class_gate<false>, dim3(1), dim3(64), 0, (hipStream_t)stream, table, thr05, n_classes, nb, m_cap,
+                           n_points, class_base, seg_len, counts);
+    PBN_LAUNCH_CHECK();
+    return PBN_OK;
+}
+
 extern "C" int pbn_class_gate(const int32_t* table, const float* thr05, int n_classes, int nb, int m_cap, int n_points,
                               int32_t* class_base, int32_t* seg_len, int32_t* counts, pbn_stream_t stream) {
-    if (!table || !thr05 || !class_base || !seg_len || !counts || n_classes < 3 || n_classes > 64 || nb < 1 || m_cap < 0)
-        return PBN_ERR_ARG;
-    hipLaunchKernelGGL(k_class_gate, dim3(1), dim3(64), 0, (hipStream_t)stream, table, thr05, n_classes, nb, m_cap, n_points,
-                       class_base, seg_len, counts);
-    PBN_LAUNCH_CHECK();
-    return PBN_OK;
+    return class_gate_impl(table, thr05, n_classes, nb, m_cap, n_points, class_base, seg_len, counts, false, stream);
+}
+
+extern "C" int pbn_class_gate_first(const int32_t* table, const float* thr05, int n_classes, int nb, int m_cap, int n_points,
+                                    int32_t* class_base, int32_t* seg_len, int32_t* counts, pbn_stream_t stream) {
+    return class_gate_impl(table, thr05, n_classes, nb, m_cap, n_points, class_base, seg_len, counts, true, stream);
 }
 
 extern "C" size_t pbn_local_plan_workspace_bytes(int c_cap) {
diff --git a/pbnet_amd/csrc/pool.hip b/pbnet_amd/csrc/pool.hip
--- a/pbnet_amd/csrc/pool.hip
+++ b/pbnet_amd/csrc/pool.hip
@@ -10,10 +10,17 @@
 template <> __device__ __forceinline__ float to_f32<__hip_bfloat16>(__hip_bfloat16 v) { return __bfloat162float(v); }
 template <> __device__ __forceinline__ float to_f32<__half>(__half v) { return __half2float(v); }
 
+__device__ __forceinline__ void store_sum(void* out, size_t e, int dtype, float mx, float av) {
+    const float s = __fadd_rn(mx, av);
+    if (dtype == PBN_F32) reinterpret_cast<float*>(out)[e] = s;
+    else if (dtype == PBN_BF16) reinterpret_cast<__hip_bfloat16*>(out)[e] = __float2bfloat16(s);
+    else reinterpret_cast<__half*>(out)[e] = __float2half(s);
+}
+
 template <typename T>
 __global__ __launch_bounds__(256) void k_segment_pool(const T* __restrict__ feats, int ld, int channels,
                                                      const int* __restrict__ seg_start, float* __restrict__ out_max,
-                                                     float* __restrict__ out_avg) {
+                                                     float* __restrict__ out_avg, void* __restrict__ out_sum, int dtype) {
     __shared__ float s_max[8][32], s_sum[8][32];
     const int b = blockIdx.x, c = blockIdx.y * 32 + (threadIdx.x & 31), rg = threadIdx.x >> 5;
     const int beg = seg_start[b], end = seg_start[b + 1];
@@ -30,8 +37,10 @@
     if (rg == 0 && c < channels) {
 #pragma unroll
         for (int k = 1; k < 8; ++k) { mx = fmaxf(mx, s_max[k][threadIdx.x]); sm += s_sum[k][threadIdx.x]; }
+        const float av = sm / (float)(end - beg);
         if (out_max) out_max[(size_t)b * channels + c] = mx;
-        if (out_avg) out_avg[(size_t)b * channels + c] = sm / (float)(end - beg);
+        if (out_avg) out_avg[(size_t)b * channels + c] = av;
+        if (out_sum) store_sum(out_sum, (size_t)b * channels + c, dtype, mx, av);
     }
 }
 
@@ -118,17 +127,42 @@
 
 __global__ __launch_bounds__(256) void k_pool_final(const float* __restrict__ part_max, const float* __restrict__ part_sum,
                                                    const int* __restrict__ seg_start, int n_seg, int C, int split,
-                                                   float* __restrict__ out_max, float* __restrict__ out_avg) {
+                                                   float* __restrict__ out_max, float* __restrict__ out_avg,
+                                                   void* __restrict__ out_sum, int dtype) {
     const int e = blockIdx.x * 256 + threadIdx.x;
     if (e >= n_seg * C) return;
     const int b = e / C, c = e - b * C;
     float m = -__builtin_inff(), t = 0.f;
-    for (int z = 0; z < split; ++z) {
-        m = fmaxf(m, part_max[((size_t)b * split + z) * C + c]);
-        t += part_sum[((size_t)b * split + z) * C + c];
-    }
+    const float* pm = part_max + (size_t)b * split * C + c;
+    const float* ps = part_sum + (size_t)b * split * C + c;
+    int z = 0;
+    for (; z + 8 <= split; z += 8) {
+        float vm[8], vs[8];
+#pragma unroll
+        for (int u = 0; u < 8; ++u) { vm[u] = pm[(size_t)(z + u) * C]; vs[u] = ps[(size_t)(z + u) * C]; }
+#pragma unroll
+        for (int u = 0; u < 8; ++u) { m = fmaxf(m, vm[u]); t += vs[u]; }
+    }
+    for (; z < split; ++z) {
+        m = fmaxf(m, pm[(size_t)z * C]);
+        t += ps[(size_t)z * C];
+    }
+    const float av = t / (float)(seg_start[b + 1] - seg_start[b]);
     if (out_max) out_max[e] = m;
-    if (out_avg) out_avg[e] = t / (float)(seg_start[b + 1] - seg_start[b]);
+    if (out_avg) out_avg[e] = av;
+    if (out_sum) store_sum(out_sum, (size_t)e, dtype, m, av);
+}
+
+__global__ __launch_bounds__(256) void k_segment_starts(const int* __restrict__ ids, int ld, int n, int n_seg,
+                                                       int* __restrict__ seg_start) {
+    const int s = blockIdx.x * 256 + threadIdx.x;
+    if (s > n_seg) return;
+    int lo = 0, hi = n;
+    while (lo < hi) {
+        const int mid = (lo + hi) >> 1;
+        if (ids[(size_t)mid * ld] < s) lo = mid + 1; else hi = mid;
+    }
+    seg_start[s] = lo;
 }
 
 int pool_split(int n_seg) {
@@ -146,13 +180,13 @@
     return (size_t)2 * n_seg * pool_split(n_seg) * channels * sizeof(float);
 }
 
-extern "C" int pbn_segment_pool(const void* feats, int ld, int channels, int dtype, const int32_t* seg_start, int n_seg,
-                                float* out_max, float* out_avg, void* workspace, size_t workspace_bytes,
-                                pbn_stream_t stream_) {
-    hipStream_t stream = (hipStream_t)stream_;
+static int segment_pool_impl(const void* feats, int ld, int channels, int dtype, const int32_t* seg_start, int n_seg,
+                             float* out_max, float* out_avg, void* out_sum, void* workspace, size_t workspace_bytes,
+                             hipStream_t stream) {
     if (n_seg < 0 || channels <= 0 || ld < channels) return PBN_ERR_ARG;
     if (n_seg == 0) return PBN_OK;
-    if (!feats || !seg_start || (!out_max && !out_avg)) return PBN_ERR_ARG;
+    if (!feats || !seg_start || (!out_max && !out_avg && !out_sum)) return PBN_ERR_ARG;
+    if (dtype != PBN_F32 && dtype != PBN_BF16 && dtype != PBN_F16) return PBN_ERR_ARG;
     const int esz = dtype == PBN_F32 ? 4 : 2;
     const int split = pool_split(n_seg);
     if (workspace && workspace_bytes >= pbn_segment_pool_workspace_bytes(n_seg, channels) && split > 1 &&
@@ -175,7 +209,7 @@
         else
             return PBN_ERR_ARG;
         hipLaunchKernelGGL(k_pool_final, dim3(cdiv((long long)n_seg * channels, 256)), dim3(256), 0, stream, pm, ps, seg_start,
-                           n_seg, channels, split, out_max, out_avg);
+                           n_seg, channels, split, out_max, out_avg, out_sum, dtype);
         PBN_LAUNCH_CHECK();
         return PBN_OK;
     }
@@ -183,18 +217,48 @@
     switch (dtype) {
         case PBN_F32:
             hipLaunchKernelGGL(k_segment_pool<float>, grid, dim3(256), 0, stream, (const float*)feats, ld, channels,
-                               seg_start, out_max, out_avg);
+                               seg_start, out_max, out_avg, out_sum, dtype);
             break;
         case PBN_BF16:
             hipLaunchKernelGGL(k_segment_pool<__hip_bfloat16>, grid, dim3(256), 0, stream, (const __hip_bfloat16*)feats,
-                               ld, channels, seg_start, out_max, out_avg);
+                               ld, channels, seg_start, out_max, out_avg, out_sum, dtype);
             break;
         case PBN_F16:
             hipLaunchKernelGGL(k_segment_pool<__half>, grid, dim3(256), 0, stream, (const __half*)feats, ld, channels,
-                               seg_start, out_max, out_avg);
+                               seg_start, out_max, out_avg, out_sum, dtype);
             break;
         default: return PBN_ERR_ARG;
     }
     PBN_LAUNCH_CHECK();
     return PBN_OK;
 }
+
+extern "C" int pbn_segment_pool(const void* feats, int ld, int channels, int dtype, const int32_t* seg_start, int n_seg,
+                                float* out_max, float* out_avg, void* workspace, size_t workspace_bytes,
+                                pbn_stream_t stream) {
+    return segment_pool_impl(feats, ld, channels, dtype, seg_start, n_seg, out_max, out_avg, nullptr, workspace, workspace_bytes,
+                             (hipStream_t)stream);
+}
+
+static size_t pool_sum_starts_bytes(int n_seg) { return align_up(sizeof(int) * ((size_t)n_seg + 1), 256); }
+
+extern "C" size_t pbn_segment_pool_sum_workspace_bytes(int n_seg, int channels) {
+    if (n_seg <= 0 || channels <= 0) return 0;
+    return pool_sum_starts_bytes(n_seg) + pbn_segment_pool_workspace_bytes(n_seg, channels);
+}
+
+extern "C" int pbn_segment_pool_sum(const void* feats, int ld, int channels, int dtype, const int32_t* seg_ids, int ld_ids,
+                                    int n_rows, int n_seg, void* out_sum, void* workspace, size_t workspace_bytes,
+                                    pbn_stream_t stream_) {
+    hipStream_t stream = (hipStream_t)stream_;
+    if (n_seg < 0 || n_rows < 0 || ld_ids < 1 || channels <= 0) return PBN_ERR_ARG;
+    if (n_seg == 0) return PBN_OK;
+    if (!out_sum || !workspace || (n_rows > 0 && !seg_ids) || ((uintptr_t)workspace & 15)) return PBN_ERR_ARG;
+    if (workspace_bytes < pbn_segment_pool_sum_workspace_bytes(n_seg, channels)) return PBN_ERR_WORKSPACE;
+    int* seg_start = reinterpret_cast<int*>(workspace);
+    hipLaunchKernelGGL(k_segment_starts, dim3(cdiv(n_seg + 1, 256)), dim3(256), 0, stream, seg_ids, ld_ids, n_rows, n_seg,
+                       seg_start);
+    const size_t head = pool_sum_starts_bytes(n_seg);
+    return segment_pool_impl(feats, ld, channels, dtype, seg_start, n_seg, nullptr, nullptr, out_sum,
+                             reinterpret_cast<unsigned char*>(workspace) + head, workspace_bytes - head, stream);
+}
diff --git a/pbnet_amd/csrc/stages.hip b/pbnet_amd/csrc/stages.hip
--- a/pbnet_amd/csrc/stages.hip
+++ b/pbnet_amd/csrc/stages.hip
@@ -79,6 +79,27 @@
         v = in[(size_t)r * ld_in_w + w];
     }
     out[e] = v;
+}
+
+template <typename IV, typename IC>
+__global__ __launch_bounds__(TPB) void k_point_rows(const IV* __restrict__ v2p, const long long* __restrict__ row_index,
+                                                   const IC* __restrict__ coords, int ld_coords, int n_voxels, int n_rows,
+                                                   int n, const uint4* __restrict__ feats, int ld_vec, int vpr,
+                                                   long long* __restrict__ idx, int* __restrict__ batch,
+                                                   uint4* __restrict__ out) {
+    const long long e = (long long)blockIdx.x * TPB + threadIdx.x;
+    if (e >= (long long)n * vpr) return;
+    const int i = (int)(e / vpr), q = (int)(e - (long long)i * vpr);
+    const long long v = (long long)v2p[i];
+    const bool ok_v = v >= 0 && v < n_voxels;
+    long long r = -1;
+    if (ok_v) r = row_index ? row_index[v] : v;
+    const bool ok = ok_v && r >= 0 && r < n_rows;
+    if (q == 0) {
+        idx[i] = ok ? r : -1;
+        batch[i] = ok ? (int)coords[(size_t)v * ld_coords] : -1;
+    }
+    out[e] = ok ? feats[(size_t)r * ld_vec + q] : make_uint4(0u, 0u, 0u, 0u);
 }
 
 
@@ -600,6 +621,28 @@
                                        const int64_t* idx2, int n_cap, const int32_t* n_dev, void* out, int ld_out_bytes,
                                        pbn_stream_t stream) {
     return gather_pad_rows_impl(in, ld_in_bytes, row_bytes, idx, idx2, n_cap, n_dev, out, ld_out_bytes, stream);
+}
+
+extern "C" int pbn_point_rows(const void* v2p, int v2p_is_i64, const int64_t* row_index, const void* coords, int coords_is_i64,
+                              int ld_coords, int n_voxels, int n_rows, int n, const void* feats, int ld_feat_bytes, int row_bytes,
+                              int64_t* idx, int32_t* batch, void* out, pbn_stream_t stream_) {
+    hipStream_t stream = (hipStream_t)stream_;
+    if (n < 0 || n_voxels < 0 || n_rows < 0 || ld_coords < 1 || row_bytes <= 0 || (row_bytes & 15) || (ld_feat_bytes & 15) ||
+        ld_feat_bytes < row_bytes)
+        return PBN_ERR_ARG;
+    if (n == 0) return PBN_OK;
+    if (!v2p || !coords || !feats || !idx || !batch || !out || (((uintptr_t)feats | (uintptr_t)out) & 15)) return PBN_ERR_ARG;
+    const int vpr = row_bytes / 16;
+    const dim3 grid(cdiv((long long)n * vpr, TPB));
+#define PBN_POINT_ROWS(IV, IC)                                                                                          \
+    hipLaunchKernelGGL((k_point_rows<IV, IC>), grid, dim3(TPB), 0, stream, (const IV*)v2p, (const long long*)row_index,  \
+                       (const IC*)coords, ld_coords, n_voxels, n_rows, n, (const uint4*)feats, ld_feat_bytes / 16, vpr,  \
+                       (long long*)idx, batch, (uint4*)out)
+    if (v2p_is_i64) { if (coords_is_i64) PBN_POINT_ROWS(long long, long long); else PBN_POINT_ROWS(long long, int); }
+    else { if (coords_is_i64) PBN_POINT_ROWS(int, long long); else PBN_POINT_ROWS(int, int); }
+#undef PBN_POINT_ROWS
+    PBN_LAUNCH_CHECK();
+    return PBN_OK;
 }
 
 static int mlp_rows_impl(const void* in, int ld_in, long long in_rows, int channels, const int64_t* idx_a, const int64_t* idx_b, int n,
diff --git a/pbnet_amd/network/PBNet.py b/pbnet_amd/network/PBNet.py
--- a/pbnet_amd/network/PBNet.py
+++ b/pbnet_amd/network/PBNet.py
@@ -134,17 +134,16 @@
         if fused:
             self._last_sizes = {"lv1": list(inputs_v1.coordinate_manager.row_counts())}
         with section("a5_heads_gather"):
-            v2p = v2p_v1.long()
             if fused:
                 f, row_index = point_feat.rows()
-                if row_index is not None:
-                    v2p = row_index[v2p]
+                v2p, batch_head_p, point_feat_p = stage_ops.point_rows(f, row_index, v2p_v1, xyz_voxel)
                 return {
-                    "point_feat_p": f[v2p],
+                    "point_feat_p": point_feat_p,
                     "sem_pred_score_p": stage_ops.mlp_rows(self.linear_sem, f, v2p),
                     "offset_pred_p": stage_ops.mlp_rows(self.linear_offset, f, v2p),
-                    "batch_head_p": xyz_voxel[:, 0].to(torch.int32)[v2p_v1.long()],
+                    "batch_head_p": batch_head_p,
                 }
+            v2p = v2p_v1.long()
             sem_pred_score = self.linear_sem(point_feat)
             sem_pred_score_sf = self.soft_max(sem_pred_score)
             offsets_pred = self.linear_offset(point_feat)
@@ -260,10 +259,9 @@
                 global_feat = global_max_plus_avg_pool(iou_feat) if iou_feat.F.is_cuda else \
                     self.global_max_pool(iou_feat) + self.global_avg_pool(iou_feat)
                 return self.linear_IOU(global_feat).F.view(-1)
-            from ..MinkowskiEngine.nn import segment_pool
+            from ..MinkowskiEngine.nn import segment_pool_sum
             n_prop = int(proposals_offset.shape[0]) - 1
-            mx, av = segment_pool(iou_feat_f, inputs_v3.C[:, 0], n_prop)
-            return stage_ops.mlp_rows(self.linear_IOU, (mx + av).to(iou_feat_f.dtype)).view(-1)
+            return stage_ops.mlp_rows(self.linear_IOU, segment_pool_sum(iou_feat_f, inputs_v3.C, n_prop)).view(-1)
 
     def _rows_fused(self, packed, n_ent, n_rows, res, ins_ind, xyz_original, point_feat_p, sem_sfp, sem_pred_p):
         with torch.no_grad():
@@ -431,16 +429,19 @@
                                torch.tensor(self._k_max_list(), dtype=torch.int32, device=dev))
         return c
 
-    def _front_launches(self, table, sem_pred, block_hist, xyz, offset, nb, m_cap, c_cap, e_cap, r_cap, counts):
+    def _front_launches(self, table, sem_pred, block_hist, xyz, offset, nb, m_cap, c_cap, e_cap, r_cap, counts, block=None):
         thr05, thr02, kmax = self._front_consts(xyz.device)
+        n_clusters = None
+        if block is not None:
+            counts, n_clusters = block[:CNT.WORDS], block[CNT.WORDS:]
         with section("a6_select"):
-            class_base, seg_len = stage_ops.class_gate(table, thr05, nb, m_cap, int(xyz.shape[0]), counts)
+            class_base, seg_len = stage_ops.class_gate(table, thr05, nb, m_cap, int(xyz.shape[0]), counts, first=block is not None)
             ins_ind, ins_orig, ins_off, ins_sem = stage_ops.select_points(sem_pred, class_base, block_hist, xyz, offset.detach(),
                                                                           m_cap)
         mark("a7:select queued")
         with section("a7_16_grouping"):
             res = pbnet_ops.cluster_device(ins_off, ins_orig, ins_sem, seg_len, self.radius, self.min_pts, capacity=True,
-                                          need_den=False)
+                                          need_den=False, n_clusters=n_clusters)
             ent = stage_ops.local_plan(res, nb, thr02, kmax, c_cap, e_cap, r_cap, counts)
             mark("a7:grouping queued")
         return ins_ind, res, ent
@@ -448,10 +449,10 @@
     def _device_front(self, s1, xyz_original, nb):
         n_pts = int(xyz_original.shape[0])
         c_cap = min(FRONT_CLUSTER_CAP, n_pts)
-        counts = torch.zeros(CNT.WORDS, dtype=torch.int32, device=xyz_original.device)
+        block = torch.empty(CNT.WORDS + 1, dtype=torch.int32, device=xyz_original.device)
         ins_ind, res, ent = self._front_launches(s1["table"], s1["sem_pred_p"], s1["block_hist"], xyz_original,
-                                                 s1["offset_pred_p"], nb, n_pts, c_cap, 7 * c_cap, 2 ** 31 - 1, counts)
-        h = torch.cat([counts, res.n_clusters]).cpu().tolist()
+                                                 s1["offset_pred_p"], nb, n_pts, c_cap, 7 * c_cap, 2 ** 31 - 1, None, block=block)
+        h = block.cpu().tolist()
         mark("a7:grouping done")
         if h[CNT.WORDS] < 0:
             raise RuntimeError("grouping rejected its input (class id outside [2,19])")
@@ -462,7 +463,7 @@
         m, n_clt, n_ent, n_rows = h[CNT.POINTS], h[CNT.CLUSTERS], h[CNT.ENTRIES], h[CNT.ROWS]
         if m == 0 or n_clt == 0 or n_ent == 0:
             return "empty"
-        return ins_ind, res, ent.compact(n_ent), n_ent, n_rows, n_clt, m
+        return ins_ind, res, ent, n_ent, n_rows, n_clt, m
 
     def _class_thresholds(self):
         hit = getattr(self, "_thr_cache", None)
@@ -500,12 +501,17 @@
         proposals_offset = np.zeros(n_alive + 1, dtype=np.int64)
         np.cumsum(per_scene[alive], out=proposals_offset[1:])
         dense_of = (np.cumsum(alive) - 1).astype(np.int32)
-        up64 = torch.from_numpy(np.concatenate([proposals_offset, np.nonzero(alive)[0].astype(np.int64)])).to(dev)
-        dense_of = torch.from_numpy(dense_of).to(dev)
+        n_sc = int(dense_of.shape[0])
+        host = np.zeros(2 * n_alive + 1 + (n_sc + 1) // 2, dtype=np.int64)
+        host[:n_alive + 1] = proposals_offset
+        host[n_alive + 1:2 * n_alive + 1] = np.nonzero(alive)[0]
+        host[2 * n_alive + 1:].view(np.int32)[:n_sc] = dense_of
+        up64 = torch.from_numpy(host).to(dev)
+        dense_of = up64[2 * n_alive + 1:].view(torch.int32)[:n_sc]
         prop_idx, prop_ms, coords3, feat3 = stage_ops.proposal_rows(
             mask_score, mask_score_thd, row_scene, point_idx, dense_of, block_cnt, total, xyz_original,
             self.scale_size, self.voxel_size, point_feat_p)
-        return (prop_idx, up64[:n_alive + 1], up64[n_alive + 1:], prop_ms), coords3, feat3
+        return (prop_idx, up64[:n_alive + 1], up64[n_alive + 1:2 * n_alive + 1], prop_ms), coords3, feat3
 
     def get_proposal(self, row_scene, point_idx, mask_score, mask_score_thd=MASK_THD, n_scenes=None):
         assert row_scene.shape[0] == mask_score.shape[0]
diff --git a/pbnet_amd/pbnet_ops.py b/pbnet_amd/pbnet_ops.py
--- a/pbnet_amd/pbnet_ops.py
+++ b/pbnet_amd/pbnet_ops.py
@@ -17,7 +17,7 @@
 
 
 def cluster_device(off_xyz, org_xyz, sem, seg_len, radius, min_pts, para_f=PARA_F, nv_flag=NV_FLAG,
-                   general_sem=False, want_members=True, capacity=False, need_den=True):
+                   general_sem=False, want_members=True, capacity=False, need_den=True, n_clusters=None):
     N.require_cuda(off_xyz, org_xyz, sem, seg_len)
     off_xyz = off_xyz.to(torch.float32).contiguous()
     org_xyz = org_xyz.to(torch.float32).contiguous()
@@ -32,7 +32,9 @@
     den = torch.empty(n, **i32)
     centers = torch.empty(3 * max(n, 1), dtype=torch.float32, device=dev)
     clt_sem = torch.empty(max(n, 1), **i32)
-    n_clusters = torch.empty(1, **i32)
+    if n_clusters is None:
+        n_clusters = torch.empty(1, **i32)
+    assert n_clusters.dtype == torch.int32 and n_clusters.numel() == 1 and n_clusters.device == dev
     member_start = torch.empty(n + 1, **i32) if want_members else None
     member_idx = torch.empty(max(n, 1), **i32) if want_members else None
     lib = N.lib()
diff --git a/pbnet_amd/stage_ops.py b/pbnet_amd/stage_ops.py
--- a/pbnet_amd/stage_ops.py
+++ b/pbnet_amd/stage_ops.py
@@ -42,7 +42,7 @@
     dev = point_feat.device
     c = int(point_feat.shape[1])
     ld_out = c + 2 if ld_out is None else int(ld_out)
-    assert ent.n == n_ent and (n_ent_dev is None) == (n_rows_dev is None)
+    assert ent.n >= n_ent and (n_ent_dev is None) == (n_rows_dev is None) and (n_ent_dev is None or ent.n == n_ent)
     assert point_feat.stride(1) == 1 and sem_score.stride(1) == 1 and sem_score.dtype == point_feat.dtype
     assert xyz.dtype == torch.float32 and xyz.is_contiguous() and ins_ind.dtype == torch.int64
     assert member_idx.dtype == torch.int32 and (sem_pred is None or sem_pred.dtype == torch.int64)
@@ -80,6 +80,33 @@
         rc = N.lib().pbn_gather_pad_rows_dev(*(src + (N.ptr(idx2), int(n), N.ptr(n_dev)) + dst))
     N.check(rc, "pbn_gather_pad_rows")
     return out
+
+
+def point_rows(feats, row_index, v2p, coords):
+    N.require_cuda(feats, row_index, v2p, coords)
+    if v2p.dtype not in (torch.int32, torch.int64):
+        v2p = v2p.long()
+    if coords.dtype not in (torch.int32, torch.int64):
+        coords = coords.long()
+    v2p = v2p.contiguous()
+    if coords.stride(1) != 1:
+        coords = coords.contiguous()
+    es = feats.element_size()
+    n, c = int(v2p.shape[0]), int(feats.shape[1])
+    assert feats.stride(1) == 1 and v2p.dtype in (torch.int32, torch.int64) and coords.dtype in (torch.int32, torch.int64)
+    assert coords.dim() == 2 and coords.stride(1) == 1 and (row_index is None or row_index.dtype == torch.int64)
+    n_vox = int(coords.shape[0]) if row_index is None else min(int(coords.shape[0]), int(row_index.shape[0]))
+    dev = feats.device
+    idx = torch.empty(n, dtype=torch.int64, device=dev)
+    batch = torch.empty(n, dtype=torch.int32, device=dev)
+    out = torch.empty(n, c, dtype=feats.dtype, device=dev)
+    vp = N.c_vp
+    rc = N.lib().pbn_point_rows(N.ptr(v2p), int(v2p.dtype == torch.int64), N.ptr(row_index), vp(coords.data_ptr()),
+                                int(coords.dtype == torch.int64), coords.stride(0), n_vox, int(feats.shape[0]), n,
+                                vp(feats.data_ptr()), feats.stride(0) * es, c * es, N.ptr(idx), N.ptr(batch),
+                                vp(out.data_ptr()), N.current_stream())
+    N.check(rc, "pbn_point_rows")
+    return idx, batch, out
 
 
 class _HeadParams(object):
@@ -164,14 +191,15 @@
     return ins_ind, ins_orig, ins_off, ins_sem
 
 
-def class_gate(table, thr05, nb, m_cap, n_points, counts):
+def class_gate(table, thr05, nb, m_cap, n_points, counts, first=False):
     N.require_cuda(table, thr05, counts)
     s = int(table.shape[0])
     assert table.dtype == torch.int32 and thr05.dtype == torch.float32 and thr05.shape[0] == s and counts.numel() == CNT.WORDS
     class_base = torch.empty(s, dtype=torch.int32, device=table.device)
     seg_len = torch.empty((s - 2) * nb, dtype=torch.int32, device=table.device)
-    rc = N.lib().pbn_class_gate(N.ptr(table), N.ptr(thr05), s, int(nb), int(m_cap), int(n_points), N.ptr(class_base),
-                                N.ptr(seg_len), N.ptr(counts), N.current_stream())
+    gate = N.lib().pbn_class_gate_first if first else N.lib().pbn_class_gate
+    rc = gate(N.ptr(table), N.ptr(thr05), s, int(nb), int(m_cap), int(n_points), N.ptr(class_base), N.ptr(seg_len),
+              N.ptr(counts), N.current_stream())
     N.check(rc, "pbn_class_gate")
     return class_base, seg_len
 
```

Result: slower. 355.5 (-2.0%).
